# CIawevy/FreeFine

Measured on NVIDIA B200. Metric: edits/s @512^2 50-step SD1.5 (FreeFine 2-D geometric edit), higher is better.
Workload: dtype bf16

## Files before the change

### freefine_b200/_lib.py

```python
from __future__ import annotations

import ctypes as C
import os

_HERE = os.path.dirname(os.path.abspath(__file__))
LIB_PATH = os.environ.get("FREEFINE_B200_LIB", os.path.join(_HERE, "lib", "libfreefine_b200.so"))

FF_MAX_PASS = 4
FF_DT_F32, FF_DT_BF16, FF_DT_F16 = 0, 1, 2
FF_PASS_KEY_INVERT, FF_PASS_ROW_XOR, FF_PASS_ROW_WEIGHT, FF_PASS_KEY2_INVERT = 1, 2, 4, 8
FF_PASS_KEY_PREFIX, FF_PASS_KEY2_PREFIX = 16, 32


class FFAttnPass(C.Structure):
    _fields_ = [("kv_stream", C.c_int32), ("key_mask", C.c_int32), ("row_mask", C.c_int32), ("flags", C.c_uint32),
                ("weight", C.c_float), ("kv_stream2", C.c_int32), ("key_mask2", C.c_int32), ("reserved", C.c_int32)]


class FFAttnHeadPlan(C.Structure):
    _fields_ = [("n_pass", C.c_int32), ("reserved", C.c_int32 * 3), ("passes", FFAttnPass * FF_MAX_PASS)]


class FFAttnArgs(C.Structure):
    _fields_ = [("q", C.c_void_p), ("k", C.c_void_p), ("v", C.c_void_p), ("out", C.c_void_p), ("plan", C.c_void_p),
                ("bitmasks", C.c_void_p), ("mask_popcount", C.c_void_p),
                ("n_streams", C.c_int32), ("n_kv_streams", C.c_int32), ("heads", C.c_int32), ("head_dim", C.c_int32),
                ("s_q", C.c_int32), ("s_kv", C.c_int32), ("n_masks", C.c_int32), ("mask_words", C.c_int32),
                ("out_dtype", C.c_int32), ("scale", C.c_float), ("v_dtype", C.c_int32), ("v_head_stride", C.c_int32)]


PLAN_BYTES = C.sizeof(FFAttnHeadPlan)
PASS_BYTES = C.sizeof(FFAttnPass)

SIGNATURES = {
    "ff_version": (C.c_int, []),
    "ff_last_error": (C.c_char_p, []),
    "ff_attn_masked_kv": (C.c_int, [C.POINTER(FFAttnArgs), C.c_void_p]),
    "ff_attn_v_head_stride": (C.c_int, [C.c_int32]),
    "ff_attn_plain_smallkv": (C.c_int, [C.c_void_p] * 4 + [C.c_int32] * 5 + [C.c_float, C.c_int32, C.c_void_p]),
    "ff_debug_set_timeline": (C.c_int, [C.c_void_p]),
    "ff_kv_gather_cast": (C.c_int, [C.c_void_p, C.c_void_p, C.c_void_p, C.c_void_p, C.c_void_p, C.c_int32, C.c_int64,
                                    C.c_int32, C.c_int32, C.c_void_p]),
    "ff_mask_downsample_pack": (C.c_int, [C.c_void_p, C.c_int32, C.c_int32, C.c_int32, C.c_int32, C.c_int32,
                                          C.c_void_p, C.c_int32, C.c_void_p, C.c_void_p]),
    "ff_upsample2x_nhwc": (C.c_int, [C.c_void_p, C.c_void_p, C.c_int32, C.c_int32, C.c_int32, C.c_int32, C.c_void_p]),
    "ff_concat_nhwc": (C.c_int, [C.c_void_p, C.c_void_p, C.c_void_p, C.c_int64, C.c_int32, C.c_int32, C.c_void_p]),
    "ff_linear_bias_residual": (C.c_int, [C.c_void_p] * 5 + [C.c_int64, C.c_int32, C.c_int32, C.c_void_p, C.c_int64, C.c_void_p]),
    "ff_mask_prep": (C.c_int, [C.c_void_p] * 4 + [C.c_int32] * 7 + [C.c_void_p] * 6),
    "ff_dilate_mask": (C.c_int, [C.c_void_p, C.c_void_p, C.c_int32, C.c_int32, C.c_int32, C.c_int32, C.c_void_p]),
    "ff_warp_affine_blend": (C.c_int, [C.c_void_p, C.c_void_p, C.c_void_p, C.c_void_p, C.c_void_p, C.c_void_p,
                                       C.c_int32, C.c_int32, C.c_int32, C.c_int32, C.c_int32, C.c_int32, C.c_int32,
                                       C.c_int32, C.c_void_p]),
    "ff_ddim_cfg_step": (C.c_int, [C.c_void_p, C.c_void_p, C.c_void_p, C.c_void_p, C.c_void_p, C.c_float, C.c_float,
                                   C.c_float, C.c_float, C.c_float, C.c_float, C.c_float, C.c_void_p, C.c_void_p,
                                   C.c_int32, C.c_int32, C.c_int32, C.c_int32, C.c_void_p]),
    "ff_debug_set_trace": (C.c_int, [C.c_void_p]),
    "ff_ddim_step": (C.c_int, [C.c_void_p, C.c_void_p, C.c_void_p, C.c_void_p, C.c_float, C.c_float, C.c_float,
                               C.c_float, C.c_float, C.c_float, C.c_void_p, C.c_void_p, C.c_int32, C.c_int32,
                               C.c_int32, C.c_int32, C.c_void_p]),
    "ff_ddim_cfg_step_compose": (C.c_int, [C.c_void_p, C.c_int32, C.c_void_p, C.c_void_p, C.c_void_p, C.c_void_p,
                                           C.c_float, C.c_float, C.c_float, C.c_float, C.c_float, C.c_float, C.c_float,
                                           C.c_void_p, C.c_void_p, C.c_int32, C.c_int32, C.c_int32, C.c_int32, C.c_void_p]),
    "ff_ddim_inv_step": (C.c_int, [C.c_void_p, C.c_void_p, C.c_float, C.c_float, C.c_float, C.c_float, C.c_void_p,
                                   C.c_void_p, C.c_int64, C.c_void_p]),
    "ff_cross_region_blend": (C.c_int, [C.c_void_p, C.c_void_p, C.c_int32, C.c_void_p, C.c_int32, C.c_int32,
                                        C.c_int32, C.c_int32, C.c_void_p]),
    "ff_group_norm_ws_bytes": (C.c_int64, [C.c_int32, C.c_int32]),
    "ff_group_norm_nhwc": (C.c_int, [C.c_void_p, C.c_void_p, C.c_int64, C.c_void_p, C.c_void_p, C.c_void_p, C.c_void_p,
                                     C.c_int32, C.c_int32, C.c_int32, C.c_int32, C.c_float, C.c_int32, C.c_void_p]),
    "ff_bias_residual_nhwc": (C.c_int, [C.c_void_p, C.c_void_p, C.c_void_p, C.c_void_p, C.c_int64, C.c_int32,
                                        C.c_void_p]),
    "ff_geglu": (C.c_int, [C.c_void_p, C.c_void_p, C.c_int64, C.c_int32, C.c_void_p]),
    "ff_layer_norm": (C.c_int, [C.c_void_p, C.c_void_p, C.c_void_p, C.c_void_p, C.c_int64, C.c_int32, C.c_float,
                                C.c_void_p]),
}

_lib = None


def load() -> C.CDLL:
    global _lib
    if _lib is None:
        if not os.path.exists(LIB_PATH):
            raise RuntimeError(f"{LIB_PATH} is missing: build it with `python -m freefine_b200.csrc.build` "
                               "(freefine_b200 has no fallback path)")
        lib = C.CDLL(LIB_PATH)
        for name, (res, args) in SIGNATURES.items():
            fn = getattr(lib, name)
            fn.restype, fn.argtypes = res, args
        _lib = lib
    return _lib


def check(rc: int, what: str) -> None:
    if rc != 0:
        msg = load().ff_last_error()
        raise RuntimeError(f"{what} failed (code {rc}): {msg.decode() if msg else ''}")
```

### freefine_b200/attention.py

```python
from __future__ import annotations

import abc
import math

import os

import torch

from . import ops, plans


class AttentionControl(abc.ABC):
    def step_callback(self, x_t):
        return x_t

    def between_steps(self):
        return

    @property
    def num_uncond_att_layers(self):
        return self.num_att_layers if self.LOW_RESOURCE else 0

    @abc.abstractmethod
    def forward(self, attn, is_cross: bool, place_in_unet: str):
        raise NotImplementedError

    def _advance(self):
        self.cur_att_layer += 1
        if self.cur_att_layer == self.num_att_layers + self.num_uncond_att_layers:
            self.cur_att_layer = 0
            self.cur_step += 1
            self.between_steps()

    def __call__(self, attn, is_cross: bool, place_in_unet: str):
        self._advance()
        return attn

    def reset(self):
        self.cur_step = 0
        self.cur_att_layer = 0

    def __init__(self):
        self.cur_step = 0
        self.num_att_layers = -1
        self.cur_att_layer = 0
        self.LOW_RESOURCE = False


def _as_u8_stack(mask: torch.Tensor) -> torch.Tensor:
    m = mask if mask.dim() == 3 else mask[None]
    if m.dtype != torch.uint8:
        m = m.clamp(0, 255).to(torch.uint8)
    return m.contiguous()


class Attention_Modulator(AttentionControl):

    def __init__(self, start_layer=None):
        super().__init__()
        self.step_num = 0
        self.model_type = 'Inverse'
        self.use_cfg = False
        self.use_style_align = False
        self.use_tca = False
        self.local_edit = False
        self.fg_retain_mask = None
        self.fg_retain_mask_st2 = None
        self.fg_ref_mask = None
        self.obj_mask = None
        self.local_edit_region = None
        self.layer_idx = list(range(start_layer, 16)) if start_layer is not None else list(range(16))
        self.down_sampling_shape = dict()
        self.method = None
        self.context_guidance = None
        self.tca_scope = ['up']
        self.style_align_scope = ['down', 'mid', 'up']
        self.src_masks = None
        self.tgt_masks = None
        self.prompt_length = 1
        self.heads = None
        self.scale = None
        self.upcast_attention = False
        self.upcast_softmax = False
        self.log_mask = False
        self.sort_keys = True
        self.p_operand = "f16"
        self.small_kv_kernel = os.environ.get("FF_ATTN_SMALLKV", "1") != "0"
        self._tables = {}
        self._plans = {}

    def forward(self, attn, is_cross: bool, place_in_unet: str):
        return attn

    def reset(self):
        super().reset()
        self.step_num = 0
        self.model_type = 'Inverse'
        self.use_cfg = False
        self.use_tca = False
        self.use_style_align = False
        self.local_edit = False
        self.down_sampling_shape = dict()
        self.style_align = False
        self.method = None
        self.context_guidance = None
        self.tca_scope = ['up']
        self.style_align_scope = ['down', 'mid', 'up']
        self._tables.clear()
        self._plans.clear()

    def get_down_h_w(self, d_ratio, h, w, seq):
        if d_ratio in self.down_sampling_shape:
            nh, nw = self.down_sampling_shape[d_ratio]
            assert nh * nw == seq, f'{nh} * {nw} != {seq}'
            return nh, nw
        r = d_ratio // 8
        nh, nw = h // 8, w // 8
        while r != 1:
            r //= 2
            nh, nw = (nh + 1) // 2, (nw + 1) // 2
        assert nw * nh == seq
        self.down_sampling_shape[d_ratio] = [nh, nw]
        return nh, nw

    def _grid(self, H, W, seq):
        d_ratio = 2 ** int(math.log2((H * W // seq) ** 0.5) + 0.5)
        return self.get_down_h_w(d_ratio, H, W, seq)

    def _table(self, kind: str, seq: int, masks, min_tokens: int = 0):
        sig = tuple((m.data_ptr(), m._version, tuple(m.shape)) for m in masks)
        hit = self._tables.get((kind, seq))
        if hit is not None and hit[0] == sig:
            return hit[1], hit[2]
        stacks = [_as_u8_stack(m) for m in masks]
        E, H, W = stacks[0].shape
        for s in stacks:
            if s.shape != (E, H, W):
                raise ValueError(f"mask shapes differ: {[tuple(x.shape) for x in stacks]}")
            if not s.is_cuda:
                raise RuntimeError("controller masks must live on the CUDA device (no CPU path)")
        h, w = self._grid(H, W, seq)
        stacked = torch.stack(stacks, dim=1).reshape(E * len(stacks), H, W)
        words = ops.mask_words(max(seq, min_tokens))
        bits = torch.zeros((stacked.shape[0], words), dtype=torch.int32, device=stacked.device)
        bits, pop = ops.mask_downsample_pack(stacked, h, w, bits=bits)
        self._tables[(kind, seq)] = (sig, bits, pop, tuple(masks))
        return bits, pop

    def _plan(self, key, builder):
        p = self._plans.get(key)
        if p is None:
            if len(self._plans) > 256:
                self._plans.clear()
            host = builder()
            p = ops.to_device_bytes(host, self._device)
            self._plans[key] = p
            ops.PLAN_REGISTRY[p.data_ptr()] = host
        return p

    def _kv_index(self, kind: str, seq: int, bits, stream_masks):
        ck = (kind, "kvidx", seq)
        hit = self._tables.get(ck)
        if hit is not None and hit[0] is bits:
            return hit[1]
        shifts = torch.arange(32, device=bits.device, dtype=torch.int32)
        key_bits = ((bits[:, :, None] >> shifts) & 1).reshape(bits.shape[0], -1)[:, :seq]
        idx = plans.kv_sort_index(key_bits, stream_masks)
        self._tables[ck] = (bits, idx)
        return idx

    def _attend(self, query, key, value, plan, bits=None, pop=None, kv_index=None):
        self._device = query.device
        dt = query.dtype
        if dt not in (torch.float32, torch.bfloat16):
            query, key, value, dt = query.float(), key.float(), value.float(), torch.float32
        q = query.to(torch.bfloat16).contiguous()
        k = key.to(torch.bfloat16).contiguous()
        v = value.to(torch.bfloat16).contiguous()
        k, v = ops.kv_gather_cast(k, v, self.heads, kv_index, p_operand=self.p_operand)
        return ops.attn_masked_kv(q, k, v, plan, self.heads, self.scale, bits, pop, out_dtype=dt)

    def plain_attention(self, query, key, value):
        self._device = query.device
        B = query.shape[0]
        if key.shape[0] != B:
            raise ValueError("plain attention needs one K/V stream per query stream")
        d = query.shape[-1] // self.heads
        if (key.shape[1] <= (128 if d == 8 else ops.SMALLKV_MAX_KEYS) and d in ops.SMALLKV_HEAD_DIMS and self.p_operand == "f16"
                and self.small_kv_kernel):
            dt = query.dtype
            if dt not in (torch.float32, torch.bfloat16):
                query, key, value, dt = query.float(), key.float(), value.float(), torch.float32
            return ops.attn_plain_smallkv(query.to(torch.bfloat16).contiguous(), key.to(torch.bfloat16).contiguous(),
                                          value.to(torch.bfloat16).contiguous(), self.heads, self.scale, out_dtype=dt)
        plan = self._plan(("plain", B, self.heads), lambda: plans.plain_plan(B, self.heads))
        return self._attend(query, key, value, plan)

    def _tca_common(self, query, key, value, kind):
        B, S, _ = query.shape
        if self.cur_att_layer // 2 not in self.layer_idx:
            out = self.plain_attention(query, key, value)
            self._advance()
            return out
        if B % 4:
            raise ValueError(f"TCA expects 4 streams [u_e,u_r,c_e,c_r] per edit, got batch {B}")
        if self.method not in ('tca', 'mmsa'):
            raise ValueError(f"controller.method must be 'tca' or 'mmsa' here, got {self.method!r}")
        E = B // 4
        self._device = query.device
        if kind == "edit":
            bits, pop = self._table("edit", S, [self.fg_ref_mask, self.fg_retain_mask])
            src_id, tgt_id = (lambda e: 2 * e), (lambda e: 2 * e + 1)
        else:
            bits, pop = self._table("bg", S, [self.fg_retain_mask])
            src_id, tgt_id = (lambda e: e), (lambda e: e)
        if bits.shape[0] not in (2 * E if kind == "edit" else E,):
            raise ValueError(f"{E} edits in the stream batch but masks for {bits.shape[0]} rows")
        cg = None if self.method == 'mmsa' else float(self.context_guidance)
        pf = self.sort_keys
        plan = self._plan((kind, E, self.heads, self.method, cg, pf),
                          lambda: plans.tca_plan(E, self.heads, self.method, cg, src_id, tgt_id, kind=kind, prefix=pf))
        kv_index = None
        if pf:
            kv_index = self._kv_index(kind, S, bits, [src_id(s // 4) if s % 2 else -1 for s in range(B)])
        out = self._attend(query, key, value, plan, bits, pop, kv_index)
        self._advance()
        return out

    def Temporal_contextal_attention(self, query, key, value, is_cross, place_in_unet):
        return self._tca_common(query, key, value, "edit")

    def Temporal_contextal_attention_bg(self, query, key, value, is_cross, place_in_unet):
        return self._tca_common(query, key, value, "bg")

    def Temporal_contextal_attention_compose(self, query, key, value, is_cross, place_in_unet):
        B, S, _ = query.shape
        if self.cur_att_layer // 2 not in self.layer_idx:
            out = self.plain_attention(query, key, value)
            self._advance()
            return out
        N = B - 2
        self._device = query.device
        src = self.src_masks[:N] if torch.is_tensor(self.src_masks) else torch.stack(list(self.src_masks)[:N])
        tgt = self.tgt_masks[:N] if torch.is_tensor(self.tgt_masks) else torch.stack(list(self.tgt_masks)[:N])
        bits, pop = self._table("compose", S, [m for m in src] + [m for m in tgt])
        cg = None if self.method == 'mmsa' else float(self.context_guidance)
        pf = self.sort_keys
        plan = self._plan(("compose", N, self.heads, self.method, cg, pf),
                          lambda: plans.compose_plan(N, self.heads, self.method, cg, list(range(N)),
                                                     list(range(N, 2 * N)), prefix=pf))
        kv_index = self._kv_index("compose", S, bits, [-1] + list(range(N)) + [-1]) if pf else None
        out = self._attend(query, key, value, plan, bits, pop, kv_index)
        self._advance()
        return out

    def _style_align(self, query, key, value, mask, bg=False):
        B, S, _ = query.shape
        if B % 4:
            raise ValueError("style-align expects 4 streams per edit")
        E = B // 4
        self._device = query.device
        bits = pop = None
        src_id = None
        if self.method == 'sdsa':
            bits, pop = self._table("sdsa", S, [mask])
            src_id = lambda e: e
        pf = self.sort_keys and src_id is not None
        plan = self._plan(("style", E, self.heads, self.method, pf, bg),
                          lambda: plans.style_align_plan(E, self.heads, src_id, prefix=pf, bg=bg))
        kv_index = self._kv_index("sdsa", S, bits, [s // 4 if s % 2 else -1 for s in range(B)]) if pf else None
        out = self._attend(query, key, value, plan, bits, pop, kv_index)
        self._advance()
        return out

    def style_align_share_attention(self, query, key, value, is_cross, place_in_unet):
        return self._style_align(query, key, value, self.fg_ref_mask)

    def style_align_share_attention_bg(self, query, key, value, is_cross, place_in_unet):
        return self._style_align(query, key, value, self.fg_retain_mask, bg=True)

    def modulate_local_cross_attn(self, query, key, value, is_cross, place_in_unet):
        B, S, _ = query.shape
        if B % 4:
            raise ValueError("local cross-attention modulation expects 4 streams per edit")
        hs = self.plain_attention(query, key, value)
        bits, _ = self._table("region", S, [self.local_edit_region])
        ids = self._plans.get(("region_ids", B // 4))
        if ids is None:
            ids = torch.arange(B // 4, dtype=torch.int32, device=query.device)
            self._plans[("region_ids", B // 4)] = ids
        ops.cross_region_blend(hs, bits, ids)
        self._advance()
        return hs

    modulate_local_cross_attn_bg = modulate_local_cross_attn

    def modulate_local_cross_attn_compose(self, query, key, value, is_cross, place_in_unet):
        Bq, S, _ = query.shape
        self._device = query.device
        L = len(self.tgt_masks)
        nu = Bq - 1
        if key.shape[0] != nu + L:
            raise ValueError(f"expected {nu + L} prompt streams, got {key.shape[0]}")
        tg = self.tgt_masks if torch.is_tensor(self.tgt_masks) else torch.stack(list(self.tgt_masks))
        bits, pop = self._table("cross_compose", S, [m for m in tg], min_tokens=key.shape[1])

        def build():
            p = plans._empty(Bq, self.heads)
            for s in range(nu):
                for h in range(self.heads):
                    plans._add(p, s, h, s, 1.0)
            for h in range(self.heads):
                for i in range(L):
                    plans._add(p, nu, h, nu + i, 1.0, row_mask=i, flags=plans.FF_PASS_ROW_WEIGHT)
            return p

        plan = self._plan(("cross_compose", Bq, L, self.heads), build)
        out = self._attend(query, key, value, plan, bits, pop)
        self._advance()
        return out


def override_forward(unet):
    inner = unet.forward

    def forward(sample, timestep, encoder_hidden_states, *args, **kwargs):
        out = inner(sample, timestep, encoder_hidden_states, *args, **kwargs)
        if torch.is_tensor(out):
            return out
        return out.sample if hasattr(out, "sample") else out[0]

    return forward


class _DummyController:
    num_att_layers = 0
    use_tca = use_style_align = local_edit = False

    def __call__(self, *args):
        return args[0]


def _register(model, controller, flavour: str):
    if controller is None:
        controller = _DummyController()
    plain = Attention_Modulator()

    def ca_forward(self, place_in_unet):
        to_out = self.to_out[0] if isinstance(self.to_out, torch.nn.ModuleList) else self.to_out

        def forward(hidden_states, encoder_hidden_states=None, attention_mask=None, temb=None):
            is_cross = encoder_hidden_states is not None
            residual = hidden_states
            if self.spatial_norm is not None:
                hidden_states = self.spatial_norm(hidden_states, temb)
            input_ndim = hidden_states.ndim
            if input_ndim == 4:
                batch_size, channel, height, width = hidden_states.shape
                hidden_states = hidden_states.view(batch_size, channel, height * width).transpose(1, 2)
            if attention_mask is not None:
                raise NotImplementedError("explicit attention_mask is not part of the FreeFine hot path")
            if self.group_norm is not None:
                hidden_states = self.group_norm(hidden_states.transpose(1, 2)).transpose(1, 2)
            query = self.to_q(hidden_states)
            if encoder_hidden_states is None:
                encoder_hidden_states = hidden_states
            elif self.norm_cross:
                encoder_hidden_states = self.norm_encoder_hidden_states(encoder_hidden_states)
            key = self.to_k(encoder_hidden_states)
            value = self.to_v(encoder_hidden_states)

            c = controller if isinstance(controller, Attention_Modulator) else plain
            c.heads, c.scale = self.heads, self.scale
            c.upcast_attention, c.upcast_softmax = self.upcast_attention, self.upcast_softmax
            if flavour == "edit":
                if not is_cross and controller.use_style_align and place_in_unet in controller.style_align_scope:
                    hidden_states = controller.style_align_share_attention(query, key, value, is_cross, place_in_unet)
                elif not is_cross and controller.use_tca and place_in_unet in controller.tca_scope:
                    hidden_states = controller.Temporal_contextal_attention(query, key, value, is_cross, place_in_unet)
                elif controller.local_edit and is_cross:
                    hidden_states = controller.modulate_local_cross_attn(query, key, value, is_cross, place_in_unet)
                else:
                    hidden_states = c.plain_attention(query, key, value)
                    controller(None, is_cross, place_in_unet)
            elif flavour == "bggen":
                if place_in_unet in ['up'] and not is_cross and controller.use_tca:
                    hidden_states = controller.Temporal_contextal_attention_bg(query, key, value, is_cross, place_in_unet)
                elif controller.local_edit and is_cross:
                    hidden_states = controller.modulate_local_cross_attn_bg(query, key, value, is_cross, place_in_unet)
                else:
                    hidden_states = c.plain_attention(query, key, value)
                    controller(None, is_cross, place_in_unet)
            else:
                if not is_cross and controller.use_tca and place_in_unet in controller.tca_scope:
                    hidden_states = controller.Temporal_contextal_attention_compose(query, key, value, is_cross, place_in_unet)
                elif controller.local_edit and is_cross:
                    hidden_states = controller.modulate_local_cross_attn_compose(query, key, value, is_cross, place_in_unet)
                else:
                    hidden_states = c.plain_attention(query, key, value)
                    controller(None, is_cross, place_in_unet)

            block_res = getattr(self, "ff_block_residual", None)
            if (block_res is not None and input_ndim == 3 and hidden_states.is_cuda and hidden_states.dtype == torch.bfloat16
                    and isinstance(to_out, torch.nn.Linear) and not self.residual_connection
                    and self.rescale_output_factor == 1.0):
                self.ff_residual_fused = True
                return ops.linear_bias_residual(hidden_states.contiguous(), to_out.weight, to_out.bias, block_res)
            hidden_states = to_out(hidden_states)
            if input_ndim == 4:
                hidden_states = hidden_states.transpose(-1, -2).reshape(batch_size, channel, height, width)
            if self.residual_connection:
                hidden_states = hidden_states + residual
            if self.rescale_output_factor != 1.0:
                hidden_states = hidden_states / self.rescale_output_factor
            return hidden_states

        return forward

    def register_recr(net_, count, place_in_unet):
        if net_.__class__.__name__ == 'Attention':
            net_.forward = ca_forward(net_, place_in_unet)
            return count + 1
        if hasattr(net_, 'children'):
            for child in net_.children():
                count = register_recr(child, count, place_in_unet)
        return count

    n = 0
    for name, net in model.unet.named_children():
        if "down" in name:
            n += register_recr(net, 0, "down")
        elif "up" in name:
            n += register_recr(net, 0, "up")
        elif "mid" in name:
            n += register_recr(net, 0, "mid")
    controller.num_att_layers = n


def register_attention_control(model, controller):
    _register(model, controller, "edit")


def register_attention_control_4bggen(model, controller):
    _register(model, controller, "bggen")


def register_attention_control_compose(model, controller):
    _register(model, controller, "compose")
```

### freefine_b200/csrc/attn_ring.cuh

```cuda
#pragma once
#include <type_traits>

template <int DPAD_, int NWG_, int NBUF_> struct RCfg {
  static constexpr int DPAD = DPAD_, NWG = NWG_, NBUF = NBUF_;
  static_assert(NBUF > NWG || NWG == 1, "a warpgroup must find its next S ready: more S/P buffers than warpgroups");
  static constexpr int DPV = Cfg<DPAD, false>::DPV;
  static constexpr int NKT = (DPAD + BOX_COLS - 1) / BOX_COLS;
  static constexpr int TMEM_S = 0, TMEM_O = NBUF * BN;
  static constexpr int TMEM_USED = TMEM_O + NWG * DPV;
  static_assert(TMEM_USED <= 512, "TMEM budget");
  static constexpr int TMEM_COLS = TMEM_USED <= 256 ? 256 : 512;
  static constexpr int MIN_CTAS = TMEM_COLS == 256 ? 2 : 1;
  static constexpr int NUM_WARPS = 4 * NWG + 4;
  static constexpr int NUM_THREADS = 32 * NUM_WARPS;
  static constexpr bool REBALANCE = false;
  static constexpr int REG_AUX = 32, REG_SOFTMAX = 112;
  static constexpr int SMEM_Q = NKT * TILE_BYTES;
  static constexpr int SMEM_K = NKT * KV_BYTES;
  static constexpr int ACC_LD = DPAD + 4;
  static constexpr int SMEM_ACC = BM * ACC_LD * 4;
  static constexpr int SMEM_MX = NWG > 1 ? NWG * BM * 4 : 0;
  static constexpr int SMEM_FIXED = 2 * SMEM_Q + SMEM_ACC + SMEM_MX + 1024  + 512 ;
  static constexpr int SMEM_BUDGET = MIN_CTAS == 2 ? 113 * 1024 : 227 * 1024;
  static constexpr int NST_FIT = (SMEM_BUDGET - SMEM_FIXED) / (2 * SMEM_K);
  static constexpr int NST = (NST_FIT >= 2 * NBUF && 2 * NBUF <= 8) ? 2 * NBUF : NBUF;
  static_assert(NST <= NST_FIT, "shared memory budget: the K and V rings must hold NBUF tiles each");
  static constexpr int SMEM_BYTES = SMEM_FIXED + 2 * NST * SMEM_K;
};

#ifdef FF_TIMELINE
#define RT_TL(role_, tile_, site_)                                                                                       \
  do {                                                                                                                   \
    if (tl && (tile_) < FF_TL_TILES) tl[(((size_t)tl_cta * 4 + (role_)) * FF_TL_TILES + (tile_)) * 8 + (site_)] = clock64(); \
  } while (0)
#define RT_TLW(wg_, tile_, site_) do { if ((wg_) < 2) RT_TL(wg_, tile_, site_); } while (0)
#else
#define RT_TL(role_, tile_, site_) do { } while (0)
#define RT_TLW(wg_, tile_, site_) do { } while (0)
#endif

struct TileIter {
  const FFAttnHeadPlan* plan;
  int n_pass, q0, n_kv_tiles;
  int ip, seg, jn, j, j1;
  bool seg_live, valid;
  PassCtx cx;
  SegCtx sg;
  __device__ __forceinline__ void init(const FFAttnHeadPlan* pl, int np, int q0_, int nkt, const KParams& p) {
    plan = pl; n_pass = np; q0 = q0_; n_kv_tiles = nkt;
    ip = -1; seg = 1; jn = 0; j = 0; j1 = 0; seg_live = false; valid = true;
    seek(p);
  }
  __device__ __forceinline__ void seek(const KParams& p) {
#pragma unroll 1
    while (true) {
      if (seg_live && jn < n_kv_tiles) {
        const int cls = tile_class(sg, jn, p), e = run_end(sg, jn, cls, p), jb = jn;
        jn = e;
        if (tile_skip(cx, sg, cls, p.s_kv)) continue;
        j = jb; j1 = e;
        return;
      }
      if (ip >= 0 && seg == 0) {
        seg = 1; sg = cx.s1; seg_live = cx.active && sg.kv >= 0; jn = 0;
        continue;
      }
      if (++ip >= n_pass) { valid = false; return; }
      const FFAttnPass ps = plan->pass[ip];
      cx = make_ctx(ps, p, q0);
      seg = 0; sg = cx.s0; seg_live = cx.active && sg.kv >= 0; jn = 0;
    }
  }
  __device__ __forceinline__ void next(const KParams& p) { if (++j >= j1) seek(p); }
};

__device__ __forceinline__ int count_tiles(const FFAttnHeadPlan* plan, int n_pass, int q0, int n_kv_tiles, const KParams& p,
                                           int& pe0, int& pe1, int& pe2) {
  int n_total = 0;
  pe0 = pe1 = pe2 = 0;
#pragma unroll
  for (int ip = 0; ip < FF_MAX_PASS; ++ip) {
    if (ip < n_pass) {
      const FFAttnPass ps = plan->pass[ip];
      const PassCtx cx = make_ctx(ps, p, q0);
      if (cx.active) {
#pragma unroll 1
        for (int seg = 0; seg < 2; ++seg) {
          const SegCtx sg = seg ? cx.s1 : cx.s0;
          if (sg.kv < 0) continue;
#pragma unroll 1
          for (int j0 = 0; j0 < n_kv_tiles;) {
            const int cls = tile_class(sg, j0, p), j1 = run_end(sg, j0, cls, p), jb = j0;
            j0 = j1;
            if (!tile_skip(cx, sg, cls, p.s_kv)) n_total += j1 - jb;
          }
        }
      }
    }
    if (ip == 0) pe0 = n_total;
    if (ip == 1) pe1 = n_total;
    if (ip == 2) pe2 = n_total;
  }
  return n_total;
}

#ifndef FF_RING_POLY
#define FF_RING_POLY FF_POLY_PATTERN
#endif

template <bool MASKED, int PATTERN>
__device__ __forceinline__ void ring_chunk_f16(const float* s, uint32_t* pk, float sc, float nb, uint32_t bits) {
  const float2 sc2 = make_float2(sc, sc), nb2 = make_float2(nb, nb);
#pragma unroll
  for (int i = 0; i < 8; ++i) {
    float2 x = __ffma2_rn(make_float2(s[2 * i], s[2 * i + 1]), sc2, nb2);
    float2 e;
    if (MASKED) {
      x.x = (bits >> (2 * i)) & 1u ? x.x : -INFINITY;
      x.y = (bits >> (2 * i + 1)) & 1u ? x.y : -INFINITY;
      e = make_float2(fast_exp2(x.x), fast_exp2(x.y));
    } else if ((PATTERN >> i) & 1) {
      e = poly_exp2_x2(x);
    } else {
      e = make_float2(fast_exp2(x.x), fast_exp2(x.y));
    }
    pk[i] = pack_f16x2(e.x, e.y);
  }
}

__device__ __forceinline__ void mbar_wait_lean(uint32_t bar, uint32_t parity) {
  uint32_t done;
  asm volatile(
      "{\n\t.reg .pred p;\n\t"
      "mbarrier.try_wait.parity.shared::cta.b64 p, [%1], %2;\n\t"
      "selp.u32 %0, 1, 0, p;\n\t}"
      : "=r"(done)
      : "r"(bar), "r"(parity)
      : "memory");
  if (!done) mbar_wait_slow(bar, parity);
}

template <int DPAD>
__device__ __forceinline__ void issue_qk(uint32_t sbuf, uint64_t qdesc, uint64_t kdesc, uint32_t idesc, uint32_t bar_s_,
                                         uint32_t bar_ke_) {
  static_assert(DPAD == 48 || DPAD == 80, "issue_qk: 3 or 5 K-steps");
  if constexpr (DPAD == 48) {
    asm volatile(
        "{\n\t.reg .pred e, pf, pt;\n\t.reg .b64 q1, q2, k1, k2;\n\t"
        "elect.sync _|e, 0xffffffff;\n\t"
        "setp.ne.b32 pf, 0, 0;\n\tsetp.eq.b32 pt, 0, 0;\n\t"
        "add.u64 q1, %1, 2;\n\tadd.u64 q2, %1, 4;\n\tadd.u64 k1, %2, 2;\n\tadd.u64 k2, %2, 4;\n\t"
        "@e tcgen05.mma.cta_group::1.kind::f16 [%0], %1, %2, %3, pf;\n\t"
        "@e tcgen05.mma.cta_group::1.kind::f16 [%0], q1, k1, %3, pt;\n\t"
        "@e tcgen05.mma.cta_group::1.kind::f16 [%0], q2, k2, %3, pt;\n\t"
        "@e tcgen05.commit.cta_group::1.mbarrier::arrive::one.shared::cluster.b64 [%4];\n\t"
        "@e tcgen05.commit.cta_group::1.mbarrier::arrive::one.shared::cluster.b64 [%5];\n\t}"
        ::"r"(sbuf), "l"(qdesc), "l"(kdesc), "r"(idesc), "r"(bar_s_), "r"(bar_ke_)
        : "memory");
  } else {
    asm volatile(
        "{\n\t.reg .pred e, pf, pt;\n\t.reg .b64 q1, q2, q3, q4, k1, k2, k3, k4;\n\t"
        "elect.sync _|e, 0xffffffff;\n\t"
        "setp.ne.b32 pf, 0, 0;\n\tsetp.eq.b32 pt, 0, 0;\n\t"
        "add.u64 q1, %1, 2;\n\tadd.u64 q2, %1, 4;\n\tadd.u64 q3, %1, 6;\n\tadd.u64 q4, %1, %6;\n\t"
        "add.u64 k1, %2, 2;\n\tadd.u64 k2, %2, 4;\n\tadd.u64 k3, %2, 6;\n\tadd.u64 k4, %2, %7;\n\t"
        "@e tcgen05.mma.cta_group::1.kind::f16 [%0], %1, %2, %3, pf;\n\t"
        "@e tcgen05.mma.cta_group::1.kind::f16 [%0], q1, k1, %3, pt;\n\t"
        "@e tcgen05.mma.cta_group::1.kind::f16 [%0], q2, k2, %3, pt;\n\t"
        "@e tcgen05.mma.cta_group::1.kind::f16 [%0], q3, k3, %3, pt;\n\t"
        "@e tcgen05.mma.cta_group::1.kind::f16 [%0], q4, k4, %3, pt;\n\t"
        "@e tcgen05.commit.cta_group::1.mbarrier::arrive::one.shared::cluster.b64 [%4];\n\t"
        "@e tcgen05.commit.cta_group::1.mbarrier::arrive::one.shared::cluster.b64 [%5];\n\t}"
        ::"r"(sbuf), "l"(qdesc), "l"(kdesc), "r"(idesc), "r"(bar_s_), "r"(bar_ke_), "n"(TILE_BYTES >> 4), "n"(KV_BYTES >> 4)
        : "memory");
  }
}

__device__ __forceinline__ void issue_pv(uint32_t obuf, uint32_t pbase, uint64_t vdesc, uint32_t idesc, uint32_t acc0,
                                         uint32_t bar_ve_, uint32_t bar_d_) {
  asm volatile(
      "{\n\t.reg .pred e, p0, pt;\n\t.reg .b64 v1, v2, v3;\n\t.reg .b32 a1, a2, a3;\n\t"
      "elect.sync _|e, 0xffffffff;\n\t"
      "setp.ne.b32 p0, %4, 0;\n\tsetp.eq.b32 pt, 0, 0;\n\t"
      "add.u64 v1, %2, 128;\n\tadd.u64 v2, %2, 256;\n\tadd.u64 v3, %2, 384;\n\t"
      "add.u32 a1, %1, 8;\n\tadd.u32 a2, %1, 32;\n\tadd.u32 a3, %1, 40;\n\t"
      "@e tcgen05.mma.cta_group::1.kind::f16 [%0], [%1], %2, %3, p0;\n\t"
      "@e tcgen05.mma.cta_group::1.kind::f16 [%0], [a1], v1, %3, pt;\n\t"
      "@e tcgen05.mma.cta_group::1.kind::f16 [%0], [a2], v2, %3, pt;\n\t"
      "@e tcgen05.mma.cta_group::1.kind::f16 [%0], [a3], v3, %3, pt;\n\t"
      "@e tcgen05.commit.cta_group::1.mbarrier::arrive::one.shared::cluster.b64 [%5];\n\t"
      "@e tcgen05.commit.cta_group::1.mbarrier::arrive::one.shared::cluster.b64 [%6];\n\t}"
      ::"r"(obuf), "r"(pbase), "l"(vdesc), "r"(idesc), "r"(acc0), "r"(bar_ve_), "r"(bar_d_)
      : "memory");
}

__device__ __forceinline__ void token_wait(int g) {
  switch (g) {
    case 0: asm volatile("bar.sync 3, 256;" ::: "memory"); break;
    case 1: asm volatile("bar.sync 4, 256;" ::: "memory"); break;
    default: asm volatile("bar.sync 5, 256;" ::: "memory"); break;
  }
}
__device__ __forceinline__ void token_pass(int g) {
  switch (g) {
    case 0: asm volatile("bar.arrive 3, 256;" ::: "memory"); break;
    case 1: asm volatile("bar.arrive 4, 256;" ::: "memory"); break;
    default: asm volatile("bar.arrive 5, 256;" ::: "memory"); break;
  }
}

template <int DPAD, int NWG, int NBUF, bool TOKEN>
__global__ void __launch_bounds__(RCfg<DPAD, NWG, NBUF>::NUM_THREADS, RCfg<DPAD, NWG, NBUF>::MIN_CTAS)
attn_ring_kernel(const __grid_constant__ CUtensorMap tm_q, const __grid_constant__ CUtensorMap tm_k,
                 const __grid_constant__ CUtensorMap tm_v, const KParams p) {
  using C = RCfg<DPAD, NWG, NBUF>;
  constexpr int NST = C::NST, SW = 4 * NWG;
  extern __shared__ uint8_t smem_raw[];
  const uint32_t smem_base = (smem_u32(smem_raw) + 1023u) & ~1023u;
  const uint32_t sQ = smem_base;
  const uint32_t sK = sQ + 2 * C::SMEM_Q;
  const uint32_t sV = sK + NST * C::SMEM_K;
  const uint32_t sACC = sV + NST * C::SMEM_K;
  const uint32_t sMX = sACC + C::SMEM_ACC;
  const uint32_t bar_base = sMX + C::SMEM_MX;
  const uint32_t bar_qf = bar_base;
  const uint32_t bar_qe = bar_base + 16;
  const uint32_t bar_s = bar_base + 32;
  const uint32_t bar_p = bar_s + 8 * NBUF;
  const uint32_t bar_d = bar_p + 8 * NBUF;
  const uint32_t bar_kf = bar_d + 8 * NBUF, bar_ke = bar_kf + 8 * NST;
  const uint32_t bar_vf = bar_ke + 8 * NST, bar_ve = bar_vf + 8 * NST;
  const uint32_t tmem_slot = bar_ve + 8 * NST;
  static_assert(32 + 24 * NBUF + 32 * NST + 8 <= 512, "barrier block");
  uint8_t* gen_base = smem_raw + (smem_base - smem_u32(smem_raw));
  float* const acc_smem = reinterpret_cast<float*>(gen_base + (sACC - smem_base));
  float* const mx_smem = reinterpret_cast<float*>(gen_base + (sMX - smem_base));
  volatile uint32_t* tmem_slot_ptr = reinterpret_cast<volatile uint32_t*>(gen_base + (tmem_slot - smem_base));

  const int warp = threadIdx.x >> 5, lane = threadIdx.x & 31;
  const int n_kv_tiles = (p.s_kv + BN - 1) / BN;
  const int n_items = p.n_qtiles * p.heads * p.n_streams;

  if (threadIdx.x == 0) {
    for (int i = 0; i < 2; ++i) {
      mbar_init(bar_qf + 8 * i, 1);
      mbar_init(bar_qe + 8 * i, 1);
    }
    for (int i = 0; i < NBUF; ++i) {
      mbar_init(bar_s + 8 * i, 1);
      mbar_init(bar_p + 8 * i, 4);
      mbar_init(bar_d + 8 * i, 1);
    }
    for (int i = 0; i < NST; ++i) {
      mbar_init(bar_kf + 8 * i, 1);
      mbar_init(bar_ke + 8 * i, 1);
      mbar_init(bar_vf + 8 * i, 1);
      mbar_init(bar_ve + 8 * i, 1);
    }
    asm volatile("fence.mbarrier_init.release.cluster;" ::: "memory");
  }
  if (warp == SW) {
    asm volatile("tcgen05.alloc.cta_group::1.sync.aligned.shared::cta.b32 [%0], %1;" ::"r"(tmem_slot),
                 "r"((uint32_t)C::TMEM_COLS)
                 : "memory");
    asm volatile("tcgen05.relinquish_alloc_permit.cta_group::1.sync.aligned;" ::: "memory");
  }
  tc_fence_before();
  __syncthreads();
  tc_fence_after();
  const uint32_t tmem = __shfl_sync(0xffffffffu, *tmem_slot_ptr, 0);
#ifdef FF_TIMELINE
  const int tl_cta = blockIdx.x == 5 ? 0 : 1;
  const int tl_role = warp == 0 ? 0 : (warp == 4 && NWG > 1 ? 1 : (warp == SW + 1 ? 2 : (warp == SW + 2 ? 3 : -1)));
  unsigned long long* const tl = ((blockIdx.x == 5 || blockIdx.x == 77) && lane == 0 && tl_role >= 0) ? g_timeline : nullptr;
#endif
  auto item_coords = [&](int w, int& q0, int& head, int& stream) {
    const int qt = w % p.n_qtiles, hs = w / p.n_qtiles;
    q0 = qt * BM;
    head = hs % p.heads;
    stream = hs / p.heads;
  };
  auto item_plan = [&](int head, int stream, int& n_pass) {
    const FFAttnHeadPlan* plan = p.plan + (size_t)stream * p.heads + head;
    n_pass = __ldg(&plan->n_pass);
    n_pass = n_pass < 0 ? 0 : (n_pass > FF_MAX_PASS ? FF_MAX_PASS : n_pass);
    return plan;
  };

  if constexpr (C::REBALANCE) {
    if (warp >= SW) asm volatile("setmaxnreg.dec.sync.aligned.u32 %0;" ::"n"(C::REG_AUX));
    else asm volatile("setmaxnreg.inc.sync.aligned.u32 %0;" ::"n"(C::REG_SOFTMAX));
  }
  if (warp == SW || warp == SW + 3) {
    if (lane == 0) {
      const bool is_k = warp == SW;
      const CUtensorMap* tm = is_k ? &tm_k : &tm_v;
      const uint32_t ring = is_k ? sK : sV, bfull = is_k ? bar_kf : bar_vf, bempty = is_k ? bar_ke : bar_ve;
      int stage = 0, use = 0, li = 0;
#pragma unroll 1
      for (int w = blockIdx.x; w < n_items; w += gridDim.x, ++li) {
        int q0, head, stream, n_pass;
        item_coords(w, q0, head, stream);
        const FFAttnHeadPlan* plan = item_plan(head, stream, n_pass);
        if (is_k) {
          const int qb = li & 1;
          if (li >= 2) mbar_wait(bar_qe + 8 * qb, ((li >> 1) - 1) & 1);
          mbar_expect_tx(bar_qf + 8 * qb, C::NKT * TILE_BYTES);
          for (int kt = 0; kt < C::NKT; ++kt)
            tma_load_4d(sQ + qb * C::SMEM_Q + kt * TILE_BYTES, &tm_q, kt * BOX_COLS, head, q0, stream, bar_qf + 8 * qb);
        }
        TileIter ti;
        ti.init(plan, n_pass, q0, n_kv_tiles, p);
#pragma unroll 1
        while (ti.valid) {
          if (use > 0) mbar_wait(bempty + 8 * stage, (use - 1) & 1);
          const uint32_t full = bfull + 8 * stage, dst = ring + stage * C::SMEM_K;
          mbar_expect_tx(full, C::NKT * KV_BYTES);
          for (int kt = 0; kt < C::NKT; ++kt)
            tma_load_4d(dst + kt * KV_BYTES, tm, kt * BOX_COLS, head, ti.j * BN, ti.sg.kv, full);
          if (++stage == NST) { stage = 0; ++use; }
          ti.next(p);
        }
      }
    }
  } else if (warp == SW + 1) {
    constexpr uint32_t idesc_qk = make_idesc(BN, 0);
    const uint64_t qdesc00 = smem_desc_sw128(sQ, 16);
    const uint64_t kdesc0 = smem_desc_sw128(sK, 16);
    uint32_t kph = 0, bph0 = 0;
    int u = 0, tg = 0, li = 0;
#pragma unroll 1
    for (int w = blockIdx.x; w < n_items; w += gridDim.x, ++li) {
      int q0, head, stream, n_pass, pe0, pe1, pe2;
      item_coords(w, q0, head, stream);
      const FFAttnHeadPlan* plan = item_plan(head, stream, n_pass);
      int left = __shfl_sync(0xffffffffu, count_tiles(plan, n_pass, q0, n_kv_tiles, p, pe0, pe1, pe2), 0);
      const int qb = li & 1;
      const uint64_t qdesc0 = qdesc00 + (uint64_t)((qb * C::SMEM_Q) >> 4);
      mbar_wait(bar_qf + 8 * qb, (li >> 1) & 1);
#pragma unroll 1
      while (left > 0) {
#pragma unroll
        for (int uu = 0; uu < NST; ++uu) {
          if (uu < u) continue;
          if (left == 0) break;
          const int b = uu % NBUF;
          const uint32_t bph = bph0 ^ (uint32_t)((uu / NBUF) & 1);
          RT_TL(2, tg, 0);
          mbar_wait_lean(bar_kf + 8 * uu, kph);
          RT_TL(2, tg, 1);
          if (tg >= NBUF) mbar_wait_lean(bar_d + 8 * b, bph ^ 1u);
          RT_TL(2, tg, 2);
          tc_fence_after();
          issue_qk<DPAD>(tmem + C::TMEM_S + BN * b, qdesc0, kdesc0 + (uint64_t)((uu * C::SMEM_K) >> 4), idesc_qk,
                         bar_s + 8 * b, bar_ke + 8 * uu);
          __syncwarp();
          RT_TL(2, tg, 3);
          --left;
          ++tg;
          u = uu + 1;
        }
        if (u == NST) {
          u = 0;
          kph ^= 1u;
          bph0 ^= (uint32_t)((NST / NBUF) & 1);
        }
      }
      if (elect_one()) tc_commit(bar_qe + 8 * qb);
      __syncwarp();
    }
  } else if (warp == SW + 2) {
    constexpr uint32_t idesc_pv = make_idesc(C::DPV, 1, true);
    const uint64_t vdesc0 = smem_desc_sw128(sV, KV_BYTES);
    uint32_t vph = 0, bph0 = 0, g = 0;
    int u = 0, tg = 0;
#pragma unroll 1
    for (int w = blockIdx.x; w < n_items; w += gridDim.x) {
      int q0, head, stream, n_pass, pe0, pe1, pe2;
      item_coords(w, q0, head, stream);
      const FFAttnHeadPlan* plan = item_plan(head, stream, n_pass);
      const int n_total = __shfl_sync(0xffffffffu, count_tiles(plan, n_pass, q0, n_kv_tiles, p, pe0, pe1, pe2), 0);
      pe0 = __shfl_sync(0xffffffffu, pe0, 0);
      pe1 = __shfl_sync(0xffffffffu, pe1, 0);
      pe2 = __shfl_sync(0xffffffffu, pe2, 0);
      int t = 0, pi = 0, pend = pe0, pstart = 0;
      g = 0;
#pragma unroll 1
      while (t < n_total) {
#pragma unroll
        for (int uu = 0; uu < NST; ++uu) {
          if (uu < u) continue;
          if (t >= n_total) break;
          const int b = uu % NBUF;
          const uint32_t bph = bph0 ^ (uint32_t)((uu / NBUF) & 1);
          while (t >= pend && pi < 3) {
            pstart = pend;
            ++pi;
            pend = pi == 1 ? pe1 : (pi == 2 ? pe2 : n_total);
          }
          const uint32_t acc0 = (t - pstart < NWG) ? 0u : 1u;
          RT_TL(3, tg, 0);
          mbar_wait_lean(bar_vf + 8 * uu, vph);
          RT_TL(3, tg, 1);
          mbar_wait_lean(bar_p + 8 * b, bph);
          RT_TL(3, tg, 2);
          tc_fence_after();
          issue_pv(tmem + C::TMEM_O + C::DPV * g, tmem + C::TMEM_S + BN * b, vdesc0 + (uint64_t)((uu * C::SMEM_K) >> 4),
                   idesc_pv, acc0, bar_ve + 8 * uu, bar_d + 8 * b);
          __syncwarp();
          RT_TL(3, tg, 3);
          if (++g == (uint32_t)NWG) g = 0;
          ++t;
          ++tg;
          u = uu + 1;
        }
        if (u == NST) {
          u = 0;
          vph ^= 1u;
          bph0 ^= (uint32_t)((NST / NBUF) & 1);
        }
      }
    }
  } else if (warp < SW) {
    const int wq = warp & 3;
    const int wg = warp >> 2;
    const int rloc = 32 * wq + lane;
    const uint32_t tlane = tmem + ((uint32_t)(wq * 32) << 16);
    const uint32_t tO = tlane + C::TMEM_O + C::DPV * wg;
    float* const acc_row = acc_smem + (size_t)rloc * C::ACC_LD;
    int base = 0;
    int my_b = 0, prev_b = -1;
    uint32_t my_ph = 0, prev_ph = 0;
    bool s_ready = false;
    if (TOKEN && NWG > 1 && wg == NWG - 1) token_pass(0);
#pragma unroll 1
    for (int w = blockIdx.x; w < n_items; w += gridDim.x) {
      int q0, head, stream, n_pass;
      item_coords(w, q0, head, stream);
      const FFAttnHeadPlan* plan = item_plan(head, stream, n_pass);
      const int row = q0 + rloc;
      bool acc_started = false;
      int it = 0;
      int my_next = wg;
      my_b = (base + wg) % NBUF;
      my_ph = (uint32_t)(((base + wg) / NBUF) & 1);
      s_ready = false;
#pragma unroll 1
      for (int ip = 0; ip < n_pass; ++ip) {
        const FFAttnPass ps = plan->pass[ip];
        const PassCtx cx = make_ctx(ps, p, q0);
        if (!cx.active) continue;
        uint32_t rb = 0;
        if (ps.row_mask >= 0 && row < p.s_q)
          rb = (__ldg(p.bitmasks + (size_t)ps.row_mask * p.mask_words + (row >> 5)) >> (row & 31)) & 1u;
        const bool rowflip = cx.rowxor && rb;
        float m_used = -INFINITY;
        int n_mine = 0;
        const int it_pass0 = it;
#pragma unroll 1
        for (int seg = 0; seg < 2; ++seg) {
          const SegCtx sg = seg ? cx.s1 : cx.s0;
          if (sg.kv < 0) continue;
          const bool flip = sg.kinv != rowflip;
          const bool uniform = uniform_for(cx, sg, flip, p.s_kv);
          const float sc = uniform ? 0.f : p.scale_log2;
#pragma unroll 1
          for (int j0 = 0; j0 < n_kv_tiles;) {
            const int cls = tile_class(sg, j0, p), j1 = run_end(sg, j0, cls, p), jb = j0;
            j0 = j1;
            if (tile_skip(cx, sg, cls, p.s_kv)) continue;
            const bool row_ok_cls = row_allowed(cls, flip, uniform);
            const int it_run = it;
            it += j1 - jb;
            auto tile = [&](auto mixed_tag, int j) {
              constexpr bool MIXED = decltype(mixed_tag)::value;
              const uint32_t tS = tlane + C::TMEM_S + BN * my_b;
              RT_TLW(wg, my_next, 0);
              if (!s_ready) mbar_wait_lean(bar_s + 8 * my_b, my_ph);
              RT_TLW(wg, my_next, 1);
              tc_fence_after();
              float s0[32], s1[32];
              tmem_ld32(tS, s0);
              tmem_ld32(tS + 32, s1);
              uint32_t kb_lo = 0xffffffffu, kb_hi = 0xffffffffu;
              if constexpr (MIXED) {
#pragma unroll
                for (int h = 0; h < 2; ++h) {
                  const int kbase = j * BN + 32 * h;
                  const int rem = p.s_kv - kbase;
                  const uint32_t valid = rem >= 32 ? 0xffffffffu : (rem <= 0 ? 0u : ((1u << rem) - 1u));
                  uint32_t kb = 0xffffffffu;
                  if (sg.kmask >= 0 && !uniform && rem > 0) {
                    if (sg.prefix) {
                      const int tt = sg.T - kbase;
                      kb = tt >= 32 ? 0xffffffffu : (tt <= 0 ? 0u : ((1u << tt) - 1u));
                    } else {
                      kb = __ldg(p.bitmasks + (size_t)sg.kmask * p.mask_words + (kbase >> 5));
                    }
                    if (flip) kb = ~kb;
                  }
                  if (h == 0) kb_lo = kb & valid; else kb_hi = kb & valid;
                }
              }
              tmem_wait_ld32(s0);
              tmem_wait_ld32(s1);
              RT_TLW(wg, my_next, 2);
              float mt;
              {
                float m0, m1, m2, m3;
                if constexpr (!MIXED) {
                  m0 = fmaxf(s0[0], s0[1]);
                  m1 = fmaxf(s0[2], s0[3]);
                  m2 = fmaxf(s1[0], s1[1]);
                  m3 = fmaxf(s1[2], s1[3]);
#pragma unroll
                  for (int i = 4; i < 32; i += 4) {
                    m0 = fmaxf(m0, fmaxf(s0[i], s0[i + 1]));
                    m1 = fmaxf(m1, fmaxf(s0[i + 2], s0[i + 3]));
                    m2 = fmaxf(m2, fmaxf(s1[i], s1[i + 1]));
                    m3 = fmaxf(m3, fmaxf(s1[i + 2], s1[i + 3]));
                  }
                } else {
                  m0 = m1 = m2 = m3 = -INFINITY;
#pragma unroll
                  for (int i = 0; i < 32; i += 2) {
                    m0 = fmaxf(m0, (kb_lo >> i) & 1u ? s0[i] : -INFINITY);
                    m1 = fmaxf(m1, (kb_lo >> (i + 1)) & 1u ? s0[i + 1] : -INFINITY);
                    m2 = fmaxf(m2, (kb_hi >> i) & 1u ? s1[i] : -INFINITY);
                    m3 = fmaxf(m3, (kb_hi >> (i + 1)) & 1u ? s1[i + 1] : -INFINITY);
                  }
                }
                mt = fmaxf(fmaxf(m0, m1), fmaxf(m2, m3));
              }
              const float mts = (!MIXED && !row_ok_cls) ? -INFINITY : (uniform ? 0.f : mt * p.scale_log2);
              float alpha = 1.f;
              bool grow = false;
              if (n_mine == 0) {
                m_used = mts;
              } else if (mts > m_used + rescale_threshold<false>()) {
                alpha = fast_exp2(m_used - mts);
                m_used = mts;
                grow = true;
              }
              RT_TLW(wg, my_next, 3);
              int nb_ = my_b + NWG;
              uint32_t nph = my_ph;
              if (nb_ >= NBUF) { nb_ -= NBUF; nph ^= 1u; }
              s_ready = mbar_test(bar_s + 8 * nb_, nph);
              const float nb = (MIXED || row_ok_cls) ? -m_used : -60000.f;
              if (TOKEN && NWG > 1) token_wait(wg);
#pragma unroll
              for (int hb = 0; hb < 2; ++hb) {
                const float* sv = hb ? s1 : s0;
                uint32_t pk[16];
                if constexpr (!MIXED) {
#pragma unroll
                  for (int jj = 0; jj < 2; ++jj) ring_chunk_f16<false, FF_RING_POLY>(sv + 16 * jj, pk + 8 * jj, sc, nb, 0u);
                } else {
                  const uint32_t kbits = hb ? kb_hi : kb_lo;
#pragma unroll
                  for (int jj = 0; jj < 2; ++jj)
                    ring_chunk_f16<true, 0>(sv + 16 * jj, pk + 8 * jj, sc, nb, (kbits >> (16 * jj)) & 0xffffu);
                }
                tmem_st16(tS + 32 * hb, pk);
              }
              if (TOKEN && NWG > 1) token_pass((wg + 1) % NWG);
              RT_TLW(wg, my_next, 4);
              if (__any_sync(0xffffffffu, grow)) {
                if (prev_b >= 0) mbar_wait(bar_d + 8 * prev_b, prev_ph);
                tc_fence_after();
#pragma unroll
                for (int c = 0; c < C::DPV / 16; ++c) {
                  float o[16];
                  uint32_t ob[16];
                  tmem_ld16(tO + 16 * c, o);
                  tmem_wait_ld16(o);
#pragma unroll
                  for (int i = 0; i < 16; ++i) ob[i] = __float_as_uint(o[i] * alpha);
                  tmem_st16(tO + 16 * c, ob);
                }
              }
              tmem_wait_st();
              tc_fence_before();
              __syncwarp();
              if (lane == 0) mbar_arrive(bar_p + 8 * my_b);
              RT_TLW(wg, my_next, 5);
              ++n_mine;
              prev_b = my_b;
              prev_ph = my_ph;
              my_next += NWG;
              my_b = nb_;
              my_ph = nph;
            };
            if (cls == TILE_MIX) {
#pragma unroll 1
              while (my_next < it) tile(std::true_type{}, jb + (my_next - it_run));
            } else {
#pragma unroll 1
              while (my_next < it) tile(std::false_type{}, 0);
            }
          }
        }
        if (it == it_pass0) continue;
        if (n_mine > 0) mbar_wait(bar_d + 8 * prev_b, prev_ph);
        tc_fence_after();
        float cg_[NWG];
        bool wrote[NWG];
        if constexpr (NWG > 1) {
          mx_smem[wg * BM + rloc] = n_mine > 0 ? m_used : -INFINITY;
          tc_fence_before();
          named_bar_sync(1, 32 * SW);
          tc_fence_after();
          float mg[NWG], m_all = -INFINITY;
#pragma unroll
          for (int g = 0; g < NWG; ++g) {
            const int first = it_pass0 + ((g - it_pass0) % NWG + NWG) % NWG;
            wrote[g] = first < it;
            mg[g] = mx_smem[g * BM + rloc];
            m_all = fmaxf(m_all, mg[g]);
          }
          float l = 0.f;
#pragma unroll
          for (int g = 0; g < NWG; ++g) {
            const float a = (wrote[g] && mg[g] > -INFINITY) ? fast_exp2(mg[g] - m_all) : 0.f;
            cg_[g] = a;
            if (wrote[g]) l = fmaf(a, tmem_ld1_wait(tlane + C::TMEM_O + C::DPV * g + p.head_dim), l);
          }
          float coef = ps.weight;
          if (ps.flags & FF_PASS_ROW_WEIGHT) coef = rb ? coef : 0.f;
          coef = l > 0.f ? coef / l : 0.f;
#pragma unroll
          for (int g = 0; g < NWG; ++g) cg_[g] *= coef;
        } else {
          wrote[0] = n_mine > 0;
          const float l = (wrote[0] && m_used > -INFINITY) ? tmem_ld1_wait(tO + p.head_dim) : 0.f;
          float coef = ps.weight;
          if (ps.flags & FF_PASS_ROW_WEIGHT) coef = rb ? coef : 0.f;
          cg_[0] = l > 0.f ? coef / l : 0.f;
        }
#pragma unroll
        for (int c = 0; c < DPAD / 16; ++c) {
          if (c % NWG != wg) continue;
          float r[16];
#pragma unroll
          for (int i = 0; i < 16; ++i) r[i] = acc_started ? acc_row[16 * c + i] : 0.f;
#pragma unroll
          for (int g = 0; g < NWG; ++g) {
            if (!wrote[g]) continue;
            float o[16];
            tmem_ld16(tlane + C::TMEM_O + C::DPV * g + 16 * c, o);
            tmem_wait_ld16(o);
#pragma unroll
            for (int i = 0; i < 16; ++i) r[i] = fmaf(cg_[g], o[i], r[i]);
          }
#pragma unroll
          for (int i = 0; i < 16; i += 4)
            *reinterpret_cast<float4*>(acc_row + 16 * c + i) = make_float4(r[i], r[i + 1], r[i + 2], r[i + 3]);
        }
        acc_started = true;
        tc_fence_before();
        if constexpr (NWG > 1) named_bar_sync(2, 32 * SW);
        else __syncwarp();
        tc_fence_after();
      }
      base += it;
      {
        const bool row_ok = row < p.s_q;
        const size_t o_off = ((size_t)stream * p.s_q + (row_ok ? row : 0)) * ((size_t)p.heads * p.head_dim) +
                             (size_t)head * p.head_dim;
#pragma unroll
        for (int c = 0; c < DPAD / 16; ++c) {
          if (c % NWG != wg) continue;
          float o[16];
#pragma unroll
          for (int i = 0; i < 16; ++i) o[i] = acc_started ? acc_row[16 * c + i] : 0.f;
#pragma unroll
          for (int g = 0; g < 2; ++g) {
            if (row_ok && 16 * c + 8 * g < p.head_dim) {
              if (p.out_dtype == FF_DT_BF16) {
                uint4 v;
                v.x = pack_bf16x2(o[8 * g + 0], o[8 * g + 1]);
                v.y = pack_bf16x2(o[8 * g + 2], o[8 * g + 3]);
                v.z = pack_bf16x2(o[8 * g + 4], o[8 * g + 5]);
                v.w = pack_bf16x2(o[8 * g + 6], o[8 * g + 7]);
                *reinterpret_cast<uint4*>(static_cast<__nv_bfloat16*>(p.out) + o_off + 16 * c + 8 * g) = v;
              } else {
                float4* dst = reinterpret_cast<float4*>(static_cast<float*>(p.out) + o_off + 16 * c + 8 * g);
                dst[0] = make_float4(o[8 * g + 0], o[8 * g + 1], o[8 * g + 2], o[8 * g + 3]);
                dst[1] = make_float4(o[8 * g + 4], o[8 * g + 5], o[8 * g + 6], o[8 * g + 7]);
              }
            }
          }
        }
      }
    }
  }
  tc_fence_before();
  __syncthreads();
  if (warp == SW) {
    tc_fence_after();
    asm volatile("tcgen05.dealloc.cta_group::1.sync.aligned.b32 %0, %1;" ::"r"(tmem), "r"((uint32_t)C::TMEM_COLS)
                 : "memory");
  }
}
```

### freefine_b200/csrc/attn_t32.cuh

```cuda
#pragma once

constexpr int TBN = 32;

struct T32 {
  static constexpr int DPAD = 48, DPV = 48, NST = 8;
  static constexpr int KVB = TBN * 128;
  static constexpr int TMEM_S = 0, TMEM_P = 4 * TBN, TMEM_O = 4 * TBN + 2 * (TBN / 2), TMEM_COLS = 256;
  static_assert(TMEM_O + 2 * DPV == 256, "TMEM budget: 4 S buffers, 2 P regions, 2 accumulators");
  static constexpr int SMEM_Q = TILE_BYTES, SMEM_STAGE = 2 * KVB;
  static constexpr int ACC_LD = DPAD + 4, SMEM_ACC = BM * ACC_LD * 4, SMEM_MX = 2 * BM * 4;
  static constexpr int SMEM_BYTES = SMEM_Q + NST * SMEM_STAGE + SMEM_ACC + SMEM_MX + 1024 + 512;
  static_assert(SMEM_BYTES <= 113 * 1024, "two CTAs per SM");
};

__device__ __forceinline__ int t32_class(const SegCtx& g, int j, const KParams& p) {
  const int lo = j * TBN;
  if (lo + TBN > p.s_kv) return TILE_MIX;
  if (g.kmask < 0) return TILE_ALL;
  if (g.prefix) return lo + TBN <= g.T ? TILE_IN : (lo >= g.T ? TILE_OUT : TILE_MIX);
  const uint32_t bits = __ldg(p.bitmasks + (size_t)g.kmask * p.mask_words + (lo >> 5));
  return bits == 0xffffffffu ? TILE_IN : (bits == 0 ? TILE_OUT : TILE_MIX);
}
__device__ __forceinline__ int t32_run_end(const SegCtx& g, int j, int cls, const KParams& p) {
  if (cls == TILE_MIX || (g.kmask >= 0 && !g.prefix)) return j + 1;
  const int n_full = p.s_kv / TBN;
  if (cls == TILE_IN) { const int t = g.T / TBN; return t < n_full ? t : n_full; }
  return n_full;
}

__device__ __forceinline__ void t32_pv(uint32_t obuf, uint32_t pbase, uint64_t vdesc, uint32_t idesc_pv, uint32_t acc0,
                                       uint32_t bar_kve, uint32_t bar_o_) {
  asm volatile(
      "{\n\t.reg .pred e, p0, pt;\n\t.reg .b64 v1;\n\t.reg .b32 a1;\n\t"
      "elect.sync _|e, 0xffffffff;\n\t"
      "setp.ne.b32 p0, %4, 0;\n\tsetp.eq.b32 pt, 0, 0;\n\t"
      "add.u64 v1, %2, 128;\n\tadd.u32 a1, %1, 8;\n\t"
      "@e tcgen05.mma.cta_group::1.kind::f16 [%0], [%1], %2, %3, p0;\n\t"
      "@e tcgen05.mma.cta_group::1.kind::f16 [%0], [a1], v1, %3, pt;\n\t"
      "@e tcgen05.commit.cta_group::1.mbarrier::arrive::one.shared::cluster.b64 [%5];\n\t"
      "@e tcgen05.commit.cta_group::1.mbarrier::arrive::one.shared::cluster.b64 [%6];\n\t}"
      ::"r"(obuf), "r"(pbase), "l"(vdesc), "r"(idesc_pv), "r"(acc0), "r"(bar_kve), "r"(bar_o_)
      : "memory");
}

__global__ void __launch_bounds__(NUM_THREADS, 2)
attn_t32_kernel(const __grid_constant__ CUtensorMap tm_q, const __grid_constant__ CUtensorMap tm_k,
                const __grid_constant__ CUtensorMap tm_v, const KParams p) {
  using C = T32;
  extern __shared__ uint8_t smem_raw[];
  const uint32_t smem_base = (smem_u32(smem_raw) + 1023u) & ~1023u;
  const uint32_t sQ = smem_base;
  const uint32_t sKV = smem_base + C::SMEM_Q;
  const uint32_t sACC = sKV + C::NST * C::SMEM_STAGE;
  const uint32_t sMX = sACC + C::SMEM_ACC;
  const uint32_t bar_base = sMX + C::SMEM_MX;
  const uint32_t bar_q = bar_base;
  const uint32_t bar_s = bar_base + 16;
  const uint32_t bar_p = bar_base + 48;
  const uint32_t bar_o = bar_base + 64;
  const uint32_t bar_kv_full = bar_base + 80, bar_kv_empty = bar_base + 80 + 8 * C::NST;
  const uint32_t tmem_slot = bar_base + 80 + 16 * C::NST;
  static_assert(80 + 16 * C::NST + 8 <= 512, "barrier block");
  uint8_t* gen_base = smem_raw + (smem_base - smem_u32(smem_raw));
  float* const acc_smem = reinterpret_cast<float*>(gen_base + (sACC - smem_base));
  float* const mx_smem = reinterpret_cast<float*>(gen_base + (sMX - smem_base));
  volatile uint32_t* tmem_slot_ptr = reinterpret_cast<volatile uint32_t*>(gen_base + (tmem_slot - smem_base));

  const int warp = threadIdx.x >> 5, lane = threadIdx.x & 31;
  const int q0 = blockIdx.x * BM, head = blockIdx.y, stream = blockIdx.z;
  const FFAttnHeadPlan* plan = p.plan + (size_t)stream * p.heads + head;
  int n_pass = __ldg(&plan->n_pass);
  n_pass = n_pass < 0 ? 0 : (n_pass > FF_MAX_PASS ? FF_MAX_PASS : n_pass);
  const int n_kv_tiles = (p.s_kv + TBN - 1) / TBN;

  if (threadIdx.x == 0) {
    mbar_init(bar_q, 1);
    for (int i = 0; i < 4; ++i) mbar_init(bar_s + 8 * i, 1);
    for (int i = 0; i < 2; ++i) {
      mbar_init(bar_p + 8 * i, NUM_SOFTMAX_WARPS / 2);
      mbar_init(bar_o + 8 * i, 1);
    }
    for (int i = 0; i < C::NST; ++i) {
      mbar_init(bar_kv_full + 8 * i, 1);
      mbar_init(bar_kv_empty + 8 * i, 1);
    }
    asm volatile("fence.mbarrier_init.release.cluster;" ::: "memory");
  }
  if (warp == NUM_SOFTMAX_WARPS) {
    asm volatile("tcgen05.alloc.cta_group::1.sync.aligned.shared::cta.b32 [%0], %1;" ::"r"(tmem_slot),
                 "r"((uint32_t)C::TMEM_COLS)
                 : "memory");
    asm volatile("tcgen05.relinquish_alloc_permit.cta_group::1.sync.aligned;" ::: "memory");
  }
  tc_fence_before();
  __syncthreads();
  tc_fence_after();
  const uint32_t tmem = *tmem_slot_ptr;

  if (warp == NUM_SOFTMAX_WARPS) {
    if (lane == 0) {
      mbar_expect_tx(bar_q, TILE_BYTES);
      tma_load_4d(sQ, &tm_q, 0, head, q0, stream, bar_q);
      int it = 0;
#pragma unroll 1
      for (int ip = 0; ip < n_pass; ++ip) {
        const FFAttnPass ps = plan->pass[ip];
        const PassCtx cx = make_ctx(ps, p, q0);
        if (!cx.active) continue;
#pragma unroll 1
        for (int seg = 0; seg < 2; ++seg) {
          const SegCtx sg = seg ? cx.s1 : cx.s0;
          if (sg.kv < 0) continue;
#pragma unroll 1
          for (int j0 = 0; j0 < n_kv_tiles;) {
            const int cls = t32_class(sg, j0, p), j1 = t32_run_end(sg, j0, cls, p), jb = j0;
            j0 = j1;
            if (tile_skip(cx, sg, cls, p.s_kv)) continue;
#pragma unroll 1
            for (int j = jb; j < j1; ++j, ++it) {
              const int stage = it % C::NST, use = it / C::NST;
              if (use > 0) mbar_wait(bar_kv_empty + 8 * stage, (use - 1) & 1);
              const uint32_t full = bar_kv_full + 8 * stage;
              const uint32_t sK = sKV + stage * C::SMEM_STAGE, sV = sK + C::KVB;
              mbar_expect_tx(full, 2 * C::KVB);
              tma_load_4d(sK, &tm_k, 0, head, j * TBN, sg.kv, full);
              tma_load_4d(sV, &tm_v, 0, head, j * TBN, sg.kv, full);
            }
          }
        }
      }
    }
  } else if (warp == NUM_SOFTMAX_WARPS + 1) {
    constexpr uint32_t idesc_qk = make_idesc(TBN, 0);
    constexpr uint32_t idesc_pv = make_idesc(C::DPV, 1, true);
    const uint64_t qdesc0 = smem_desc_sw128(sQ, 16);
    const uint64_t kdesc0 = smem_desc_sw128(sKV, 16);
    const uint64_t vdesc0 = smem_desc_sw128(sKV + C::KVB, C::KVB);
    int pe0 = 0, pe1 = 0, pe2 = 0, n_total = 0;
#pragma unroll
    for (int ip = 0; ip < FF_MAX_PASS; ++ip) {
      if (ip < n_pass) {
        const FFAttnPass ps = plan->pass[ip];
        const PassCtx cx = make_ctx(ps, p, q0);
        if (cx.active) {
#pragma unroll 1
          for (int seg = 0; seg < 2; ++seg) {
            const SegCtx sg = seg ? cx.s1 : cx.s0;
            if (sg.kv < 0) continue;
#pragma unroll 1
            for (int j0 = 0; j0 < n_kv_tiles;) {
              const int cls = t32_class(sg, j0, p), j1 = t32_run_end(sg, j0, cls, p), jb = j0;
              j0 = j1;
              if (!tile_skip(cx, sg, cls, p.s_kv)) n_total += j1 - jb;
            }
          }
        }
      }
      if (ip == 0) pe0 = n_total;
      if (ip == 1) pe1 = n_total;
      if (ip == 2) pe2 = n_total;
    }
    mbar_wait(bar_q, 0);
    tc_fence_after();
#pragma unroll
    for (int t0 = 0; t0 < 4; ++t0) {
      if (t0 < n_total) {
        lean_wait(bar_kv_full + 8 * t0, 0);
        tc_fence_after();
        lean_qk48(tmem + C::TMEM_S + TBN * (2 * (t0 & 1) + ((t0 >> 1) & 1)), qdesc0, kdesc0 + (uint64_t)((t0 * C::SMEM_STAGE) >> 4),
                  idesc_qk, bar_s + 8 * (2 * (t0 & 1) + ((t0 >> 1) & 1)));
      }
    }
    uint32_t gph = 0;
    int t = 0;
#pragma unroll 1
    while (t < n_total) {
#pragma unroll
      for (int u = 0; u < 8; ++u) {
        if (t < n_total) {
          const int pstart = t >= pe2 ? pe2 : (t >= pe1 ? pe1 : (t >= pe0 ? pe0 : 0));
          const uint32_t acc0 = (t - pstart < 2) ? 0u : 1u;
          const int wgi = u & 1, kb = (u >> 1) & 1;
          lean_wait(bar_p + 8 * wgi, (uint32_t)kb);
          tc_fence_after();
          t32_pv(tmem + C::TMEM_O + C::DPV * wgi, tmem + C::TMEM_P + (TBN / 2) * wgi, vdesc0 + (uint64_t)((u * C::SMEM_STAGE) >> 4),
                 idesc_pv, acc0, bar_kv_empty + 8 * u, bar_o + 8 * wgi);
          if (t + 4 < n_total) {
            lean_wait(bar_kv_full + 8 * ((u + 4) & 7), u < 4 ? gph : gph ^ 1u);
            tc_fence_after();
            lean_qk48(tmem + C::TMEM_S + TBN * (2 * wgi + kb), qdesc0, kdesc0 + (uint64_t)((((u + 4) & 7) * C::SMEM_STAGE) >> 4),
                      idesc_qk, bar_s + 8 * (2 * wgi + kb));
          }
          ++t;
        }
      }
      gph ^= 1u;
    }
    __syncwarp();
  } else {
    const int wq = warp & 3, wg = warp >> 2;
    const int rloc = 32 * wq + lane;
    const int row = q0 + rloc;
    const uint32_t tlane = tmem + ((uint32_t)(wq * 32) << 16);
    const uint32_t tP = tlane + C::TMEM_P + (TBN / 2) * wg;
    const uint32_t tO = tlane + C::TMEM_O + C::DPV * wg;
    const uint32_t tOx = tlane + C::TMEM_O + C::DPV * (wg ^ 1);
    float* const acc_row = acc_smem + (size_t)rloc * C::ACC_LD;
    bool acc_started = false;
    int it = 0;
#pragma unroll 1
    for (int ip = 0; ip < n_pass; ++ip) {
      const FFAttnPass ps = plan->pass[ip];
      const PassCtx cx = make_ctx(ps, p, q0);
      if (!cx.active) continue;
      uint32_t rb = 0;
      if (ps.row_mask >= 0 && row < p.s_q)
        rb = (__ldg(p.bitmasks + (size_t)ps.row_mask * p.mask_words + (row >> 5)) >> (row & 31)) & 1u;
      const bool rowflip = cx.rowxor && rb;
      float m_used = -INFINITY;
      int n_mine = 0, last_mine = 0;
      const int it_pass0 = it;
#pragma unroll 1
      for (int seg = 0; seg < 2; ++seg) {
        const SegCtx sg = seg ? cx.s1 : cx.s0;
        if (sg.kv < 0) continue;
        const bool flip = sg.kinv != rowflip;
        const bool uniform = uniform_for(cx, sg, flip, p.s_kv);
        const float sc = uniform ? 0.f : p.scale_log2;
#pragma unroll 1
        for (int j0 = 0; j0 < n_kv_tiles;) {
          const int cls = t32_class(sg, j0, p), j1 = t32_run_end(sg, j0, cls, p), jb = j0;
          j0 = j1;
          if (tile_skip(cx, sg, cls, p.s_kv)) continue;
          const bool row_ok_cls = row_allowed(cls, flip, uniform);
          int j = jb + (((it ^ wg) & 1) ? 1 : 0);
          int itj = it + (j - jb);
          it += j1 - jb;
#pragma unroll 1
          for (; j < j1; j += 2, itj += 2) {
            const int kbuf = (itj >> 1) & 1;
            const uint32_t tS = tlane + C::TMEM_S + TBN * (2 * wg + kbuf);
            mbar_wait(bar_s + 8 * (2 * wg + kbuf), (uint32_t)((itj >> 2) & 1));
            tc_fence_after();
            float s[32];
            tmem_ld32(tS, s);
            uint32_t kbits = 0xffffffffu;
            if (cls == TILE_MIX) {
              const int kbase = j * TBN;
              const int rem = p.s_kv - kbase;
              const uint32_t valid = rem >= 32 ? 0xffffffffu : (rem <= 0 ? 0u : ((1u << rem) - 1u));
              uint32_t kb = 0xffffffffu;
              if (sg.kmask >= 0 && !uniform && rem > 0) {
                if (sg.prefix) {
                  const int tt = sg.T - kbase;
                  kb = tt >= 32 ? 0xffffffffu : (tt <= 0 ? 0u : ((1u << tt) - 1u));
                } else {
                  kb = __ldg(p.bitmasks + (size_t)sg.kmask * p.mask_words + (kbase >> 5));
                }
                if (flip) kb = ~kb;
              }
              kbits = kb & valid;
            }
            tmem_wait_ld32(s);
            float mt;
            {
              float m0, m1;
              if (cls != TILE_MIX) {
                m0 = fmaxf(s[0], s[1]);
                m1 = fmaxf(s[2], s[3]);
#pragma unroll
                for (int i = 4; i < 32; i += 4) {
                  m0 = fmaxf(m0, fmaxf(s[i], s[i + 1]));
                  m1 = fmaxf(m1, fmaxf(s[i + 2], s[i + 3]));
                }
              } else {
                m0 = m1 = -INFINITY;
#pragma unroll
                for (int i = 0; i < 32; i += 2) {
                  m0 = fmaxf(m0, (kbits >> i) & 1u ? s[i] : -INFINITY);
                  m1 = fmaxf(m1, (kbits >> (i + 1)) & 1u ? s[i + 1] : -INFINITY);
                }
              }
              mt = fmaxf(m0, m1);
              if (cls != TILE_MIX && !row_ok_cls) mt = -INFINITY;
            }
            const float mts = uniform ? 0.f : mt * p.scale_log2;
            float alpha = 1.f;
            bool grow = false;
            if (n_mine == 0) {
              m_used = mts;
            } else if (mts > m_used + rescale_threshold<false>()) {
              alpha = fast_exp2(m_used - mts);
              m_used = mts;
              grow = true;
            }
            const bool any_grow = __any_sync(0xffffffffu, grow);
            const float nb = (cls == TILE_MIX || row_ok_cls) ? -m_used : -INFINITY;
            uint32_t pk[16];
            if (cls != TILE_MIX) {
#pragma unroll
              for (int jj = 0; jj < 2; ++jj) softmax_chunk_f16<false>(s + 16 * jj, pk + 8 * jj, sc, nb, 0u);
            } else {
#pragma unroll
              for (int jj = 0; jj < 2; ++jj) softmax_chunk_f16<true>(s + 16 * jj, pk + 8 * jj, sc, nb, (kbits >> (16 * jj)) & 0xffffu);
            }
            if (itj >= 2) {
              const uint32_t po = (uint32_t)(((itj - 2) >> 1) & 1);
              if (!mbar_test(bar_o + 8 * wg, po)) mbar_wait(bar_o + 8 * wg, po);
            }
            tc_fence_after();
            if (any_grow) {
#pragma unroll
              for (int c = 0; c < C::DPV / 16; ++c) {
                float o[16];
                uint32_t ob[16];
                tmem_ld16(tO + 16 * c, o);
                tmem_wait_ld16(o);
#pragma unroll
                for (int i = 0; i < 16; ++i) ob[i] = __float_as_uint(o[i] * alpha);
                tmem_st16(tO + 16 * c, ob);
              }
            }
            tmem_st16(tP, pk);
            tmem_wait_st();
            tc_fence_before();
            __syncwarp();
            if (lane == 0) mbar_arrive(bar_p + 8 * wg);
            ++n_mine;
            last_mine = itj;
          }
        }
      }
      if (it == it_pass0) continue;
      if (n_mine > 0) mbar_wait(bar_o + 8 * wg, (uint32_t)((last_mine >> 1) & 1));
      tc_fence_after();
      mx_smem[wg * BM + rloc] = n_mine > 0 ? m_used : -INFINITY;
      tc_fence_before();
      named_bar_sync(1, 32 * NUM_SOFTMAX_WARPS);
      tc_fence_after();
      const float m_other = mx_smem[(wg ^ 1) * BM + rloc];
      const float m_all = fmaxf(m_used, m_other);
      const bool wrote_mine = n_mine > 0, wrote_other = (it - it_pass0) - n_mine > 0;
      const float a_mine = (wrote_mine && m_used > -INFINITY) ? fast_exp2(m_used - m_all) : 0.f;
      const float a_other = (wrote_other && m_other > -INFINITY) ? fast_exp2(m_other - m_all) : 0.f;
      float l = 0.f;
      if (wrote_mine) l = a_mine * tmem_ld1_wait(tO + p.head_dim);
      if (wrote_other) l = fmaf(a_other, tmem_ld1_wait(tOx + p.head_dim), l);
      float coef = ps.weight;
      if (ps.flags & FF_PASS_ROW_WEIGHT) coef = rb ? coef : 0.f;
      coef = l > 0.f ? coef / l : 0.f;
      const float c_mine = coef * a_mine, c_other = coef * a_other;
#pragma unroll
      for (int c = 0; c < C::DPAD / 16; ++c) {
        if ((c & 1) != wg) continue;
        float r[16];
#pragma unroll
        for (int i = 0; i < 16; ++i) r[i] = acc_started ? acc_row[16 * c + i] : 0.f;
        if (wrote_mine) {
          float o[16];
          tmem_ld16(tO + 16 * c, o);
          tmem_wait_ld16(o);
#pragma unroll
          for (int i = 0; i < 16; ++i) r[i] = fmaf(c_mine, o[i], r[i]);
        }
        if (wrote_other) {
          float o[16];
          tmem_ld16(tOx + 16 * c, o);
          tmem_wait_ld16(o);
#pragma unroll
          for (int i = 0; i < 16; ++i) r[i] = fmaf(c_other, o[i], r[i]);
        }
#pragma unroll
        for (int i = 0; i < 16; i += 4)
          *reinterpret_cast<float4*>(acc_row + 16 * c + i) = make_float4(r[i], r[i + 1], r[i + 2], r[i + 3]);
      }
      acc_started = true;
      tc_fence_before();
      named_bar_sync(2, 32 * NUM_SOFTMAX_WARPS);
      tc_fence_after();
    }
    {
      const bool row_ok = row < p.s_q;
      const size_t o_off = ((size_t)stream * p.s_q + (row_ok ? row : 0)) * ((size_t)p.heads * p.head_dim) +
                           (size_t)head * p.head_dim;
#pragma unroll
      for (int c = 0; c < C::DPAD / 16; ++c) {
        if ((c & 1) != wg) continue;
        float o[16];
#pragma unroll
        for (int i = 0; i < 16; ++i) o[i] = acc_started ? acc_row[16 * c + i] : 0.f;
#pragma unroll
        for (int g = 0; g < 2; ++g) {
          if (row_ok && 16 * c + 8 * g < p.head_dim) {
            if (p.out_dtype == FF_DT_BF16) {
              uint4 v;
              v.x = pack_bf16x2(o[8 * g + 0], o[8 * g + 1]);
              v.y = pack_bf16x2(o[8 * g + 2], o[8 * g + 3]);
              v.z = pack_bf16x2(o[8 * g + 4], o[8 * g + 5]);
              v.w = pack_bf16x2(o[8 * g + 6], o[8 * g + 7]);
              *reinterpret_cast<uint4*>(static_cast<__nv_bfloat16*>(p.out) + o_off + 16 * c + 8 * g) = v;
            } else {
              float4* dst = reinterpret_cast<float4*>(static_cast<float*>(p.out) + o_off + 16 * c + 8 * g);
              dst[0] = make_float4(o[8 * g + 0], o[8 * g + 1], o[8 * g + 2], o[8 * g + 3]);
              dst[1] = make_float4(o[8 * g + 4], o[8 * g + 5], o[8 * g + 6], o[8 * g + 7]);
            }
          }
        }
      }
    }
  }
  tc_fence_before();
  __syncthreads();
  if (warp == NUM_SOFTMAX_WARPS) {
    tc_fence_after();
    asm volatile("tcgen05.dealloc.cta_group::1.sync.aligned.b32 %0, %1;" ::"r"(tmem), "r"((uint32_t)C::TMEM_COLS)
                 : "memory");
  }
}
```

### freefine_b200/csrc/attn_tcgen05.cu

```cuda
#include <cuda.h>
#include <cuda_bf16.h>

#include <atomic>
#include <cstdlib>
#include <type_traits>

#include "ff_common.cuh"

namespace {

constexpr int BM = 128;
constexpr int BN = 64;
constexpr int BOX_COLS = 64;
constexpr int TILE_BYTES = BM * 128;
constexpr int KV_BYTES = BN * 128;
constexpr int NUM_SOFTMAX_WARPS = 8;
constexpr int NUM_THREADS = 32 * (NUM_SOFTMAX_WARPS + 2);
template <bool HILO> constexpr float rescale_threshold() { return HILO ? 24.f : 8.f; }
#ifndef FF_RING_DEFAULT
#define FF_RING_DEFAULT 6
#endif
#ifndef FF_POLY_PATTERN
#define FF_POLY_PATTERN 0x92
#endif
#ifndef FF_T32_DEFAULT
#define FF_T32_DEFAULT 0
#endif
#ifndef FF_SEP_P
#define FF_SEP_P 0
#endif
#ifndef FF_SELF_ISSUE
#define FF_SELF_ISSUE 0
#endif

template <int DPAD, bool HILO> struct Cfg {
  static constexpr int DPV = DPAD == 16 ? 16 : (DPAD == 48 ? 48 : DPAD + 16);
  static constexpr int NKT = (DPAD + BOX_COLS - 1) / BOX_COLS;
  static_assert((DPV + BOX_COLS - 1) / BOX_COLS == NKT, "V tile must span as many boxes as the K tile");
  static constexpr int NSTAGE = DPAD <= 48 ? 4 : (DPAD <= 80 ? 3 : 2);
  static_assert(NSTAGE >= 2, "QK(t+1) is issued before PV(t): tile t+1 must fit beside tile t");
  static constexpr bool SEP = FF_SEP_P && DPAD == 48 && !HILO && NSTAGE == 4;
  static constexpr int TMEM_S = 0, TMEM_P = 2 * BN, TMEM_O = 2 * BN + (SEP ? BN / 2 : 0);
  static constexpr int TMEM_USED = TMEM_O + 2 * DPV;
  static constexpr int TMEM_COLS = TMEM_USED <= 256 ? 256 : 512;
  static constexpr int SMEM_Q = NKT * TILE_BYTES;
  static constexpr int SMEM_STAGE = 2 * NKT * KV_BYTES;
  static constexpr int ACC_LD = DPAD <= 80 ? DPAD + 4 : DPAD;
  static constexpr int SMEM_ACC = BM * ACC_LD * 4;
  static constexpr int SMEM_MX = 2 * BM * 4;
  static constexpr int SMEM_BYTES = SMEM_Q + NSTAGE * SMEM_STAGE + SMEM_ACC + SMEM_MX + 1024  + 256 ;
  static_assert(SMEM_BYTES <= 227 * 1024, "shared memory budget");
  static constexpr int MIN_CTAS = (SMEM_BYTES <= 113 * 1024 && TMEM_COLS == 256) ? 2 : 1;
  static constexpr bool SELF = FF_SELF_ISSUE && !SEP && DPAD == 48 && !HILO && NSTAGE == 4;
  static constexpr int THREADS = SELF ? 32 * (NUM_SOFTMAX_WARPS + 1) : NUM_THREADS;
};

__device__ __forceinline__ uint32_t smem_u32(const void* p) { return (uint32_t)__cvta_generic_to_shared(p); }

__device__ __forceinline__ void mbar_init(uint32_t bar, uint32_t count) {
  asm volatile("mbarrier.init.shared::cta.b64 [%0], %1;" ::"r"(bar), "r"(count));
}
__device__ __forceinline__ void mbar_expect_tx(uint32_t bar, uint32_t bytes) {
  asm volatile("mbarrier.arrive.expect_tx.shared::cta.b64 _, [%0], %1;" ::"r"(bar), "r"(bytes) : "memory");
}
__device__ __forceinline__ void mbar_arrive(uint32_t bar) {
  asm volatile("mbarrier.arrive.shared::cta.b64 _, [%0];" ::"r"(bar) : "memory");
}
__device__ __forceinline__ uint32_t mbar_try(uint32_t bar, uint32_t parity) {
  uint32_t done;
#ifdef FF_TRYWAIT_NOHINT
  asm volatile(
      "{\n\t.reg .pred p;\n\t"
      "mbarrier.try_wait.parity.shared::cta.b64 p, [%1], %2;\n\t"
      "selp.u32 %0, 1, 0, p;\n\t}"
      : "=r"(done)
      : "r"(bar), "r"(parity)
      : "memory");
#else
  asm volatile(
      "{\n\t.reg .pred p;\n\t"
      "mbarrier.try_wait.parity.shared::cta.b64 p, [%1], %2, %3;\n\t"
      "selp.u32 %0, 1, 0, p;\n\t}"
      : "=r"(done)
      : "r"(bar), "r"(parity), "r"(0x989680u)
      : "memory");
#endif
  return done;
}
__device__ __forceinline__ bool mbar_test(uint32_t bar, uint32_t parity) {
  uint32_t done;
  asm volatile(
      "{\n\t.reg .pred p;\n\t"
      "mbarrier.test_wait.parity.shared::cta.b64 p, [%1], %2;\n\t"
      "selp.u32 %0, 1, 0, p;\n\t}"
      : "=r"(done)
      : "r"(bar), "r"(parity)
      : "memory");
  return done != 0;
}
#ifndef FF_WAIT_FORM
#define FF_WAIT_FORM 1
#endif
__device__ __noinline__ void mbar_wait_slow(uint32_t bar, uint32_t parity) {
#if FF_WAIT_FORM == 0
  const long long t0 = clock64();
  while (!mbar_try(bar, parity)) {
    if (clock64() - t0 > 4000000000LL) {
      printf("ff_attn: mbarrier wait timed out (block %d,%d,%d thread %d bar %u parity %u)\n", blockIdx.x,
             blockIdx.y, blockIdx.z, threadIdx.x, bar, parity);
      __trap();
    }
  }
#else
  const long long t0 = clock64();
#pragma unroll 1
  for (uint32_t n = 1;; ++n) {
    if ((n & 15u) == 0 && clock64() - t0 > 4000000000LL) break;
#if FF_WAIT_FORM == 1
    if (mbar_try(bar, parity)) return;
#else
    uint32_t done;
    asm volatile(
        "{\n\t.reg .pred p;\n\t"
        "mbarrier.try_wait.parity.shared::cta.b64 p, [%1], %2;\n\t"
        "selp.u32 %0, 1, 0, p;\n\t}"
        : "=r"(done)
        : "r"(bar), "r"(parity)
        : "memory");
    if (done) return;
#endif
  }
  printf("ff_attn: mbarrier wait timed out (block %d,%d,%d thread %d bar %u parity %u)\n", blockIdx.x, blockIdx.y,
         blockIdx.z, threadIdx.x, bar, parity);
  __trap();
#endif
}
__device__ __forceinline__ void mbar_wait(uint32_t bar, uint32_t parity) {
  if (!mbar_try(bar, parity)) mbar_wait_slow(bar, parity);
}
#ifndef FF_SPIN_MASK
#define FF_SPIN_MASK 0
#endif
template <int ROLE_BIT>
__device__ __forceinline__ void mbar_wait_hot(uint32_t bar, uint32_t parity) {
  if constexpr ((FF_SPIN_MASK >> ROLE_BIT) & 1) {
    for (uint32_t n = 0; !mbar_test(bar, parity); ++n) {
#ifdef FF_SPIN_SLEEP
      __nanosleep(FF_SPIN_SLEEP);
#endif
      if (n > (1u << 24)) { mbar_wait_slow(bar, parity); return; }
    }
  } else {
    mbar_wait(bar, parity);
  }
}
__device__ __forceinline__ void tma_load_4d(uint32_t dst, const CUtensorMap* map, int c0, int c1, int c2, int c3,
                                            uint32_t bar) {
  asm volatile(
      "cp.async.bulk.tensor.4d.shared::cluster.global.tile.mbarrier::complete_tx::bytes [%0], [%1, {%2, %3, %4, %5}], [%6];"
      ::"r"(dst), "l"(map), "r"(c0), "r"(c1), "r"(c2), "r"(c3), "r"(bar)
      : "memory");
}
__device__ __forceinline__ void named_bar_sync(int id, int count) {
  switch (id) {
    case 1: asm volatile("bar.sync 1, %0;" ::"r"(count) : "memory"); break;
    case 2: asm volatile("bar.sync 2, %0;" ::"r"(count) : "memory"); break;
    case 3: asm volatile("bar.sync 3, %0;" ::"r"(count) : "memory"); break;
    default: asm volatile("bar.sync 4, %0;" ::"r"(count) : "memory"); break;
  }
}
__device__ __forceinline__ bool elect_one() {
  uint32_t pred;
  asm volatile("{\n\t.reg .pred p;\n\telect.sync _|p, 0xffffffff;\n\tselp.u32 %0, 1, 0, p;\n\t}" : "=r"(pred));
  return pred != 0;
}
__device__ __forceinline__ void tc_fence_before() { asm volatile("tcgen05.fence::before_thread_sync;" ::: "memory"); }
__device__ __forceinline__ void tc_fence_after() { asm volatile("tcgen05.fence::after_thread_sync;" ::: "memory"); }
__device__ __forceinline__ void tc_commit(uint32_t bar) {
  asm volatile("tcgen05.commit.cta_group::1.mbarrier::arrive::one.shared::cluster.b64 [%0];" ::"r"(bar) : "memory");
}
__device__ __forceinline__ void mma_ss(uint32_t d_tmem, uint64_t a_desc, uint64_t b_desc, uint32_t idesc,
                                       uint32_t accumulate) {
  asm volatile(
      "{\n\t.reg .pred p;\n\tsetp.ne.b32 p, %4, 0;\n\t"
      "tcgen05.mma.cta_group::1.kind::f16 [%0], %1, %2, %3, p;\n\t}"
      ::"r"(d_tmem), "l"(a_desc), "l"(b_desc), "r"(idesc), "r"(accumulate)
      : "memory");
}
__device__ __forceinline__ void mma_ts(uint32_t d_tmem, uint32_t a_tmem, uint64_t b_desc, uint32_t idesc,
                                       uint32_t accumulate) {
  asm volatile(
      "{\n\t.reg .pred p;\n\tsetp.ne.b32 p, %4, 0;\n\t"
      "tcgen05.mma.cta_group::1.kind::f16 [%0], [%1], %2, %3, p;\n\t}"
      ::"r"(d_tmem), "r"(a_tmem), "l"(b_desc), "r"(idesc), "r"(accumulate)
      : "memory");
}
__device__ __forceinline__ void tmem_ld32(uint32_t taddr, float (&v)[32]) {
  uint32_t* r = reinterpret_cast<uint32_t*>(v);
  asm volatile(
      "tcgen05.ld.sync.aligned.32x32b.x32.b32 "
      "{%0, %1, %2, %3, %4, %5, %6, %7, %8, %9, %10, %11, %12, %13, %14, %15, "
      "%16, %17, %18, %19, %20, %21, %22, %23, %24, %25, %26, %27, %28, %29, %30, %31}, [%32];"
      : "=r"(r[0]), "=r"(r[1]), "=r"(r[2]), "=r"(r[3]), "=r"(r[4]), "=r"(r[5]), "=r"(r[6]), "=r"(r[7]),
        "=r"(r[8]), "=r"(r[9]), "=r"(r[10]), "=r"(r[11]), "=r"(r[12]), "=r"(r[13]), "=r"(r[14]), "=r"(r[15]),
        "=r"(r[16]), "=r"(r[17]), "=r"(r[18]), "=r"(r[19]), "=r"(r[20]), "=r"(r[21]), "=r"(r[22]), "=r"(r[23]),
        "=r"(r[24]), "=r"(r[25]), "=r"(r[26]), "=r"(r[27]), "=r"(r[28]), "=r"(r[29]), "=r"(r[30]), "=r"(r[31])
      : "r"(taddr)
      : "memory");
}
__device__ __forceinline__ void tmem_ld16(uint32_t taddr, float (&v)[16]) {
  uint32_t* r = reinterpret_cast<uint32_t*>(v);
  asm volatile(
      "tcgen05.ld.sync.aligned.32x32b.x16.b32 "
      "{%0, %1, %2, %3, %4, %5, %6, %7, %8, %9, %10, %11, %12, %13, %14, %15}, [%16];"
      : "=r"(r[0]), "=r"(r[1]), "=r"(r[2]), "=r"(r[3]), "=r"(r[4]), "=r"(r[5]), "=r"(r[6]), "=r"(r[7]),
        "=r"(r[8]), "=r"(r[9]), "=r"(r[10]), "=r"(r[11]), "=r"(r[12]), "=r"(r[13]), "=r"(r[14]), "=r"(r[15])
      : "r"(taddr)
      : "memory");
}
__device__ __forceinline__ float tmem_ld1_wait(uint32_t taddr) {
  uint32_t r;
  asm volatile("tcgen05.ld.sync.aligned.32x32b.x1.b32 {%0}, [%1];\n\ttcgen05.wait::ld.sync.aligned;"
               : "=r"(r) : "r"(taddr) : "memory");
  return __uint_as_float(r);
}
__device__ __forceinline__ void tmem_st16(uint32_t taddr, const uint32_t (&r)[16]) {
  asm volatile(
      "tcgen05.st.sync.aligned.32x32b.x16.b32 [%0], "
      "{%1, %2, %3, %4, %5, %6, %7, %8, %9, %10, %11, %12, %13, %14, %15, %16};"
      ::"r"(taddr), "r"(r[0]), "r"(r[1]), "r"(r[2]), "r"(r[3]), "r"(r[4]), "r"(r[5]), "r"(r[6]), "r"(r[7]),
        "r"(r[8]), "r"(r[9]), "r"(r[10]), "r"(r[11]), "r"(r[12]), "r"(r[13]), "r"(r[14]), "r"(r[15])
      : "memory");
}
__device__ __forceinline__ void tmem_wait_ld() { asm volatile("tcgen05.wait::ld.sync.aligned;" ::: "memory"); }
__device__ __forceinline__ void tmem_wait_ld16(float (&v)[16]) {
#ifdef FF_PLAIN_WAIT
  tmem_wait_ld();
  return;
#endif
  uint32_t* r = reinterpret_cast<uint32_t*>(v);
  asm volatile("tcgen05.wait::ld.sync.aligned;"
               : "+r"(r[0]), "+r"(r[1]), "+r"(r[2]), "+r"(r[3]), "+r"(r[4]), "+r"(r[5]), "+r"(r[6]), "+r"(r[7]),
                 "+r"(r[8]), "+r"(r[9]), "+r"(r[10]), "+r"(r[11]), "+r"(r[12]), "+r"(r[13]), "+r"(r[14]), "+r"(r[15])
               :
               : "memory");
}
__device__ __forceinline__ void tmem_wait_ld32(float (&v)[32]) {
#ifdef FF_PLAIN_WAIT
  tmem_wait_ld();
  return;
#endif
  uint32_t* r = reinterpret_cast<uint32_t*>(v);
  asm volatile("tcgen05.wait::ld.sync.aligned;"
               : "+r"(r[0]), "+r"(r[1]), "+r"(r[2]), "+r"(r[3]), "+r"(r[4]), "+r"(r[5]), "+r"(r[6]), "+r"(r[7]),
                 "+r"(r[8]), "+r"(r[9]), "+r"(r[10]), "+r"(r[11]), "+r"(r[12]), "+r"(r[13]), "+r"(r[14]), "+r"(r[15]),
                 "+r"(r[16]), "+r"(r[17]), "+r"(r[18]), "+r"(r[19]), "+r"(r[20]), "+r"(r[21]), "+r"(r[22]), "+r"(r[23]),
                 "+r"(r[24]), "+r"(r[25]), "+r"(r[26]), "+r"(r[27]), "+r"(r[28]), "+r"(r[29]), "+r"(r[30]), "+r"(r[31])
               :
               : "memory");
}
__device__ __forceinline__ void tmem_wait_st() { asm volatile("tcgen05.wait::st.sync.aligned;" ::: "memory"); }
__device__ __forceinline__ float fast_exp2(float x) {
#ifdef FF_KO_MUFU
  return x;
#else
  float y;
  asm("ex2.approx.ftz.f32 %0, %1;" : "=f"(y) : "f"(x));
  return y;
#endif
}

__device__ __forceinline__ uint64_t smem_desc_sw128(uint32_t saddr, uint32_t lbo_bytes) {
  return (uint64_t)((saddr & 0x3FFFFu) >> 4) | ((uint64_t)(lbo_bytes >> 4) << 16) | ((uint64_t)(1024u >> 4) << 32) |
         (1ull << 46) | (2ull << 61);
}
__host__ __device__ constexpr uint32_t make_idesc(int n, int b_mn, bool f16 = false) {
  return (1u << 4) | (f16 ? 0u : ((1u << 7) | (1u << 10))) | ((uint32_t)b_mn << 16) | ((uint32_t)(n >> 3) << 17) |
         ((uint32_t)(BM >> 4) << 24);
}

__device__ uint32_t* g_trace = nullptr;
__device__ __forceinline__ void trace(uint32_t* tr, int role, uint32_t it, uint32_t site) {
  if (tr) {
    const uint32_t cta = blockIdx.x + gridDim.x * (blockIdx.y + gridDim.y * blockIdx.z);
    volatile uint32_t* t = tr + (size_t)cta * 8 + role * 2;
    t[0] = it;
    t[1] = site;
    __threadfence_system();
  }
}

#ifdef FF_TIMELINE
__device__ unsigned long long* g_timeline = nullptr;
#define FF_TL_TILES 64
#define FF_TL(role_, tile_, site_)                                                                      \
  do {                                                                                                  \
    if (tl && (tile_) < FF_TL_TILES) tl[(((size_t)tl_cta * 2 + (role_)) * FF_TL_TILES + (tile_)) * 8 + (site_)] = clock64(); \
  } while (0)
#else
#define FF_TL(role_, tile_, site_) do { } while (0)
#endif

struct KParams {
  const FFAttnHeadPlan* plan;
  const uint32_t* bitmasks;
  const int32_t* popc;
  void* out;
  int heads, head_dim, s_q, s_kv, mask_words, out_dtype, n_kv_streams;
  int n_streams, n_qtiles;
  float scale_log2;
};

enum { TILE_ALL = 0, TILE_IN = 1, TILE_OUT = 2, TILE_MIX = 3 };

struct SegCtx {
  int kv;
  int kmask;
  int T;
  bool kinv, prefix;
};
struct PassCtx {
  SegCtx s0, s1;
  bool rowxor, active, two_seg;
  bool has_rf0, has_rf1;
};

__device__ __forceinline__ PassCtx make_ctx(const FFAttnPass& ps, const KParams& p, int q0) {
  PassCtx c;
  c.s0.kv = ps.kv_stream;
  c.s1.kv = ps.kv_stream2;
  c.two_seg = ps.kv_stream2 >= 0;
  c.s0.kmask = ps.key_mask;
  c.s1.kmask = ps.key_mask2;
  c.s0.kinv = (ps.flags & FF_PASS_KEY_INVERT) != 0;
  c.s1.kinv = (ps.flags & FF_PASS_KEY2_INVERT) != 0;
  c.s0.prefix = (ps.flags & FF_PASS_KEY_PREFIX) != 0;
  c.s1.prefix = (ps.flags & FF_PASS_KEY2_PREFIX) != 0;
  c.s0.T = ps.key_mask >= 0 ? __ldg(p.popc + ps.key_mask) : 0;
  c.s1.T = ps.key_mask2 >= 0 ? __ldg(p.popc + ps.key_mask2) : 0;
  c.rowxor = (ps.flags & FF_PASS_ROW_XOR) != 0 && ps.row_mask >= 0;
  c.active = true;
  c.has_rf0 = true;
  c.has_rf1 = false;
  if (ps.row_mask >= 0 && (c.rowxor || (ps.flags & FF_PASS_ROW_WEIGHT))) {
    uint32_t any1 = 0, any0 = 0;
    for (int w = 0; w < BM / 32; ++w) {
      const int base = q0 + 32 * w;
      if (base >= p.s_q) break;
      const uint32_t bits = __ldg(p.bitmasks + (size_t)ps.row_mask * p.mask_words + (base >> 5));
      const int rem = p.s_q - base;
      const uint32_t valid = rem >= 32 ? 0xffffffffu : ((1u << rem) - 1u);
      any1 |= bits & valid;
      any0 |= ~bits & valid;
    }
    if (ps.flags & FF_PASS_ROW_WEIGHT) c.active = any1 != 0;
    if (c.rowxor) {
      c.has_rf0 = any0 != 0;
      c.has_rf1 = any1 != 0;
    }
  }
  return c;
}

__device__ __forceinline__ bool uniform_for(const PassCtx& c, const SegCtx& g, bool f, int s_kv) {
  if (c.two_seg || g.kmask < 0) return false;
  return (f ? s_kv - g.T : g.T) == 0;
}

__device__ __forceinline__ int tile_class(const SegCtx& g, int j, const KParams& p) {
  const int lo = j * BN;
  if (lo + BN > p.s_kv) return TILE_MIX;
  if (g.kmask < 0) return TILE_ALL;
  if (g.prefix) return lo + BN <= g.T ? TILE_IN : (lo >= g.T ? TILE_OUT : TILE_MIX);
  uint32_t a = 0xffffffffu, o = 0;
  for (int w = 0; w < BN / 32; ++w) {
    const uint32_t bits = __ldg(p.bitmasks + (size_t)g.kmask * p.mask_words + (lo >> 5) + w);
    a &= bits;
    o |= bits;
  }
  return a == 0xffffffffu ? TILE_IN : (o == 0 ? TILE_OUT : TILE_MIX);
}

__device__ __forceinline__ int run_end(const SegCtx& g, int j, int cls, const KParams& p) {
  if (cls == TILE_MIX || (g.kmask >= 0 && !g.prefix)) return j + 1;
  const int n_full = p.s_kv / BN;
  if (cls == TILE_IN) { const int t = g.T / BN; return t < n_full ? t : n_full; }
  return n_full;
}

__device__ __forceinline__ bool row_allowed(int cls, bool flip, bool uniform) {
  return uniform || cls == TILE_ALL || ((cls == TILE_IN) != flip);
}

__device__ __forceinline__ bool tile_skip(const PassCtx& c, const SegCtx& g, int cls, int s_kv) {
  if (cls == TILE_MIX || cls == TILE_ALL) return false;
  bool need = false;
  if (c.has_rf0) need = need || row_allowed(cls, g.kinv, uniform_for(c, g, g.kinv, s_kv));
  if (c.has_rf1) need = need || row_allowed(cls, !g.kinv, uniform_for(c, g, !g.kinv, s_kv));
  return !need;
}

__device__ __forceinline__ uint32_t pack_bf16x2(float lo, float hi) {
  const __nv_bfloat162 b = __floats2bfloat162_rn(lo, hi);
  return *reinterpret_cast<const uint32_t*>(&b);
}

template <bool MASKED>
__device__ __forceinline__ void softmax_chunk_hilo(const float* s, uint32_t* hl, float sc, float nb, uint32_t bits) {
  const float2 sc2 = make_float2(sc, sc), nb2 = make_float2(nb, nb);
#pragma unroll
  for (int i = 0; i < 8; ++i) {
    float2 x = __ffma2_rn(make_float2(s[2 * i], s[2 * i + 1]), sc2, nb2);
    if (MASKED) {
      x.x = (bits >> (2 * i)) & 1u ? x.x : -INFINITY;
      x.y = (bits >> (2 * i + 1)) & 1u ? x.y : -INFINITY;
    }
    const float2 e = make_float2(fast_exp2(x.x), fast_exp2(x.y));
    const uint32_t b0 = __float_as_uint(e.x), b1 = __float_as_uint(e.y);
    hl[i] = __byte_perm(b0, b1, 0x7632);
    const float2 r = __fadd2_rn(e, make_float2(-__uint_as_float(b0 & 0xffff0000u), -__uint_as_float(b1 & 0xffff0000u)));
    hl[8 + i] = pack_bf16x2(r.x, r.y);
  }
}

__device__ __forceinline__ float2 poly_exp2_x2(float2 x) {
  const float MAGIC = 12582912.f;
  x.x = fmaxf(x.x, -125.f);
  x.y = fmaxf(x.y, -125.f);
  const float2 t = __fadd2_rn(x, make_float2(MAGIC, MAGIC));
  const float2 n = __fadd2_rn(t, make_float2(-MAGIC, -MAGIC));
  const float2 f = __fadd2_rn(x, make_float2(-n.x, -n.y));
  float2 r = __ffma2_rn(make_float2(0.055205512791872025f, 0.055205512791872025f), f,
                        make_float2(0.24261389672756195f, 0.24261389672756195f));
  r = __ffma2_rn(r, f, make_float2(0.6932547688484192f, 0.6932547688484192f));
  r = __ffma2_rn(r, f, make_float2(0.9999276995658875f, 0.9999276995658875f));
  r.x = __int_as_float(__float_as_int(r.x) + (__float_as_int(t.x) << 23));
  r.y = __int_as_float(__float_as_int(r.y) + (__float_as_int(t.y) << 23));
  return r;
}

__device__ __forceinline__ uint32_t pack_f16x2(float lo, float hi) {
  uint32_t r;
  asm("cvt.rn.f16x2.f32 %0, %1, %2;" : "=r"(r) : "f"(hi), "f"(lo));
  return r;
}

template <bool MASKED>
__device__ __forceinline__ void softmax_chunk_f16(const float* s, uint32_t* pk, float sc, float nb, uint32_t bits) {
  const float2 sc2 = make_float2(sc, sc), nb2 = make_float2(nb, nb);
#pragma unroll
  for (int i = 0; i < 8; ++i) {
    float2 x = __ffma2_rn(make_float2(s[2 * i], s[2 * i + 1]), sc2, nb2);
    float2 e;
    if (MASKED) {
      x.x = (bits >> (2 * i)) & 1u ? x.x : -INFINITY;
      x.y = (bits >> (2 * i + 1)) & 1u ? x.y : -INFINITY;
      e = make_float2(fast_exp2(x.x), fast_exp2(x.y));
#ifdef FF_KO_EXP
    } else if (true) {
      e = x;
#endif
    } else if ((FF_POLY_PATTERN >> i) & 1) {
      e = poly_exp2_x2(x);
    } else {
      e = make_float2(fast_exp2(x.x), fast_exp2(x.y));
    }
    pk[i] = pack_f16x2(e.x, e.y);
  }
}


#ifndef FF_LEAN_ISSUER
#define FF_LEAN_ISSUER 1
#endif
__device__ __forceinline__ void lean_wait(uint32_t bar, uint32_t parity) {
  uint32_t done;
  asm volatile(
      "{\n\t.reg .pred p;\n\t"
      "mbarrier.try_wait.parity.shared::cta.b64 p, [%1], %2;\n\t"
      "selp.u32 %0, 1, 0, p;\n\t}"
      : "=r"(done)
      : "r"(bar), "r"(parity)
      : "memory");
#ifdef FF_LEAN_SPIN
  for (int n = 0; !done && n < FF_LEAN_SPIN; ++n) done = mbar_test(bar, parity);
#endif
  if (!done) mbar_wait_slow(bar, parity);
}
__device__ __forceinline__ void lean_qk48(uint32_t sbuf, uint64_t qdesc, uint64_t kdesc, uint32_t idesc, uint32_t bar_s_) {
  asm volatile(
      "{\n\t.reg .pred e, pf, pt;\n\t.reg .b64 q1, q2, k1, k2;\n\t"
      "elect.sync _|e, 0xffffffff;\n\t"
      "setp.ne.b32 pf, 0, 0;\n\tsetp.eq.b32 pt, 0, 0;\n\t"
      "add.u64 q1, %1, 2;\n\tadd.u64 q2, %1, 4;\n\tadd.u64 k1, %2, 2;\n\tadd.u64 k2, %2, 4;\n\t"
      "@e tcgen05.mma.cta_group::1.kind::f16 [%0], %1, %2, %3, pf;\n\t"
      "@e tcgen05.mma.cta_group::1.kind::f16 [%0], q1, k1, %3, pt;\n\t"
      "@e tcgen05.mma.cta_group::1.kind::f16 [%0], q2, k2, %3, pt;\n\t"
      "@e tcgen05.commit.cta_group::1.mbarrier::arrive::one.shared::cluster.b64 [%4];\n\t}"
      ::"r"(sbuf), "l"(qdesc), "l"(kdesc), "r"(idesc), "r"(bar_s_)
      : "memory");
}
#ifdef FF_KO_PV1
#define FF_KO_PVSTEPS(x)
#else
#define FF_KO_PVSTEPS(x) x
#endif
#ifdef FF_KO_QK1
#define FF_KO_QKSTEPS(x)
#else
#define FF_KO_QKSTEPS(x) x
#endif
template <bool WITH_QK>
__device__ __forceinline__ void lean_pv_qk48(uint32_t obuf, uint32_t sp, uint64_t vdesc, uint32_t idesc_pv, uint32_t acc0,
                                             uint32_t bar_kve, uint64_t qdesc, uint64_t kdesc, uint32_t idesc_qk,
                                             uint32_t bar_s_) {
  if constexpr (WITH_QK) {
    asm volatile(
        "{\n\t.reg .pred e, p0, pf, pt;\n\t.reg .b64 v1, v2, v3, q1, q2, k1, k2;\n\t.reg .b32 a1, a2, a3;\n\t"
        "elect.sync _|e, 0xffffffff;\n\t"
        "setp.ne.b32 p0, %4, 0;\n\tsetp.ne.b32 pf, 0, 0;\n\tsetp.eq.b32 pt, 0, 0;\n\t"
        "add.u64 v1, %2, 128;\n\tadd.u64 v2, %2, 256;\n\tadd.u64 v3, %2, 384;\n\t"
        "add.u32 a1, %1, 8;\n\tadd.u32 a2, %1, 32;\n\tadd.u32 a3, %1, 40;\n\t"
        "add.u64 q1, %6, 2;\n\tadd.u64 q2, %6, 4;\n\tadd.u64 k1, %7, 2;\n\tadd.u64 k2, %7, 4;\n\t"
        "@e tcgen05.mma.cta_group::1.kind::f16 [%0], [%1], %2, %3, p0;\n\t"
        FF_KO_PVSTEPS("@e tcgen05.mma.cta_group::1.kind::f16 [%0], [a1], v1, %3, pt;\n\t")
        FF_KO_PVSTEPS("@e tcgen05.mma.cta_group::1.kind::f16 [%0], [a2], v2, %3, pt;\n\t")
        FF_KO_PVSTEPS("@e tcgen05.mma.cta_group::1.kind::f16 [%0], [a3], v3, %3, pt;\n\t")
        "@e tcgen05.commit.cta_group::1.mbarrier::arrive::one.shared::cluster.b64 [%5];\n\t"
        "@e tcgen05.mma.cta_group::1.kind::f16 [%1], %6, %7, %8, pf;\n\t"
        FF_KO_QKSTEPS("@e tcgen05.mma.cta_group::1.kind::f16 [%1], q1, k1, %8, pt;\n\t")
        FF_KO_QKSTEPS("@e tcgen05.mma.cta_group::1.kind::f16 [%1], q2, k2, %8, pt;\n\t")
        "@e tcgen05.commit.cta_group::1.mbarrier::arrive::one.shared::cluster.b64 [%9];\n\t}"
        ::"r"(obuf), "r"(sp), "l"(vdesc), "r"(idesc_pv), "r"(acc0), "r"(bar_kve), "l"(qdesc), "l"(kdesc), "r"(idesc_qk),
          "r"(bar_s_)
        : "memory");
  } else {
    asm volatile(
        "{\n\t.reg .pred e, p0, pt;\n\t.reg .b64 v1, v2, v3;\n\t.reg .b32 a1, a2, a3;\n\t"
        "elect.sync _|e, 0xffffffff;\n\t"
        "setp.ne.b32 p0, %4, 0;\n\tsetp.eq.b32 pt, 0, 0;\n\t"
        "add.u64 v1, %2, 128;\n\tadd.u64 v2, %2, 256;\n\tadd.u64 v3, %2, 384;\n\t"
        "add.u32 a1, %1, 8;\n\tadd.u32 a2, %1, 32;\n\tadd.u32 a3, %1, 40;\n\t"
        "@e tcgen05.mma.cta_group::1.kind::f16 [%0], [%1], %2, %3, p0;\n\t"
        "@e tcgen05.mma.cta_group::1.kind::f16 [%0], [a1], v1, %3, pt;\n\t"
        "@e tcgen05.mma.cta_group::1.kind::f16 [%0], [a2], v2, %3, pt;\n\t"
        "@e tcgen05.mma.cta_group::1.kind::f16 [%0], [a3], v3, %3, pt;\n\t"
        "@e tcgen05.commit.cta_group::1.mbarrier::arrive::one.shared::cluster.b64 [%5];\n\t"
        "@e tcgen05.commit.cta_group::1.mbarrier::arrive::one.shared::cluster.b64 [%6];\n\t}"
        ::"r"(obuf), "r"(sp), "l"(vdesc), "r"(idesc_pv), "r"(acc0), "r"(bar_kve), "r"(bar_s_)
        : "memory");
  }
}

__device__ __forceinline__ void lean_pv48_sep(uint32_t obuf, uint32_t pbase, uint64_t vdesc, uint32_t idesc_pv, uint32_t acc0,
                                              uint32_t bar_kve, uint32_t bar_o_) {
  asm volatile(
      "{\n\t.reg .pred e, p0, pt;\n\t.reg .b64 v1, v2, v3;\n\t.reg .b32 a1, a2, a3;\n\t"
      "elect.sync _|e, 0xffffffff;\n\t"
      "setp.ne.b32 p0, %4, 0;\n\tsetp.eq.b32 pt, 0, 0;\n\t"
      "add.u64 v1, %2, 128;\n\tadd.u64 v2, %2, 256;\n\tadd.u64 v3, %2, 384;\n\t"
      "add.u32 a1, %1, 8;\n\tadd.u32 a2, %1, 16;\n\tadd.u32 a3, %1, 24;\n\t"
      "@e tcgen05.mma.cta_group::1.kind::f16 [%0], [%1], %2, %3, p0;\n\t"
      "@e tcgen05.mma.cta_group::1.kind::f16 [%0], [a1], v1, %3, pt;\n\t"
      "@e tcgen05.mma.cta_group::1.kind::f16 [%0], [a2], v2, %3, pt;\n\t"
      "@e tcgen05.mma.cta_group::1.kind::f16 [%0], [a3], v3, %3, pt;\n\t"
      "@e tcgen05.commit.cta_group::1.mbarrier::arrive::one.shared::cluster.b64 [%5];\n\t"
      "@e tcgen05.commit.cta_group::1.mbarrier::arrive::one.shared::cluster.b64 [%6];\n\t}"
      ::"r"(obuf), "r"(pbase), "l"(vdesc), "r"(idesc_pv), "r"(acc0), "r"(bar_kve), "r"(bar_o_)
      : "memory");
}

template <int DPAD, bool P_HILO>
__global__ void __launch_bounds__(Cfg<DPAD, P_HILO>::THREADS, Cfg<DPAD, P_HILO>::MIN_CTAS)
attn_masked_kv_kernel(const __grid_constant__ CUtensorMap tm_q, const __grid_constant__ CUtensorMap tm_k,
                      const __grid_constant__ CUtensorMap tm_v, const KParams p) {
  using C = Cfg<DPAD, P_HILO>;
  extern __shared__ uint8_t smem_raw[];
  const uint32_t smem_base = (smem_u32(smem_raw) + 1023u) & ~1023u;
  const uint32_t sQ = smem_base;
  const uint32_t sKV = smem_base + C::SMEM_Q;
  const uint32_t sACC = sKV + C::NSTAGE * C::SMEM_STAGE;
  const uint32_t sMX = sACC + C::SMEM_ACC;
  const uint32_t bar_base = sMX + C::SMEM_MX;
  const uint32_t bar_q = bar_base;
  const uint32_t bar_s = bar_base + 16, bar_p = bar_base + 32;
  const uint32_t bar_kv_full = bar_base + 48, bar_kv_empty = bar_base + 48 + 8 * C::NSTAGE;
  const uint32_t tmem_slot = bar_base + 48 + 16 * C::NSTAGE;
  const uint32_t bar_f = bar_base + 192, bar_o = bar_base + 208;
  static_assert(48 + 16 * C::NSTAGE + 8 <= 192, "barrier block layout");
  uint8_t* gen_base = smem_raw + (smem_base - smem_u32(smem_raw));
  float* const acc_smem = reinterpret_cast<float*>(gen_base + (sACC - smem_base));
  float* const mx_smem = reinterpret_cast<float*>(gen_base + (sMX - smem_base));
  volatile uint32_t* tmem_slot_ptr =
      reinterpret_cast<volatile uint32_t*>(gen_base + (tmem_slot - smem_base));

  const int warp = threadIdx.x >> 5, lane = threadIdx.x & 31;
  const int q0 = blockIdx.x * BM, head = blockIdx.y, stream = blockIdx.z;
  const FFAttnHeadPlan* plan = p.plan + (size_t)stream * p.heads + head;
  int n_pass = __ldg(&plan->n_pass);
  n_pass = n_pass < 0 ? 0 : (n_pass > FF_MAX_PASS ? FF_MAX_PASS : n_pass);
  const int n_kv_tiles = (p.s_kv + BN - 1) / BN;

  if (threadIdx.x == 0) {
    mbar_init(bar_q, 1);
    mbar_init(bar_s, 1);
    mbar_init(bar_s + 8, 1);
    mbar_init(bar_p, NUM_SOFTMAX_WARPS / 2);
    mbar_init(bar_p + 8, NUM_SOFTMAX_WARPS / 2);
    mbar_init(bar_f, NUM_SOFTMAX_WARPS / 2);
    mbar_init(bar_f + 8, NUM_SOFTMAX_WARPS / 2);
    mbar_init(bar_o, 1);
    mbar_init(bar_o + 8, 1);
    for (int i = 0; i < C::NSTAGE; ++i) {
      mbar_init(bar_kv_full + 8 * i, 1);
      mbar_init(bar_kv_empty + 8 * i, 1);
    }
    asm volatile("fence.mbarrier_init.release.cluster;" ::: "memory");
  }
  if (warp == NUM_SOFTMAX_WARPS) {
    asm volatile("tcgen05.alloc.cta_group::1.sync.aligned.shared::cta.b32 [%0], %1;" ::"r"(tmem_slot),
                 "r"((uint32_t)C::TMEM_COLS)
                 : "memory");
    asm volatile("tcgen05.relinquish_alloc_permit.cta_group::1.sync.aligned;" ::: "memory");
  }
  tc_fence_before();
  __syncthreads();
  tc_fence_after();
  const uint32_t tmem = *tmem_slot_ptr;
#ifdef FF_ENABLE_TRACE
  uint32_t* const tr = g_trace;
  const int trole = warp == NUM_SOFTMAX_WARPS ? 0 : (warp == NUM_SOFTMAX_WARPS + 1 ? 1 : (threadIdx.x == 0 ? 2 : (threadIdx.x == 32 * NUM_SOFTMAX_WARPS - 32 ? 3 : -1)));
#define FF_TRACE(it_, site_) do { if (tr && trole >= 0 && (warp < NUM_SOFTMAX_WARPS || lane == 0)) trace(tr, trole, (uint32_t)(it_), (site_)); } while (0)
#else
#define FF_TRACE(it_, site_) do { } while (0)
#endif
  FF_TRACE(0, 1);
#ifdef FF_TIMELINE
  const int tl_lin = blockIdx.x + gridDim.x * (blockIdx.y + gridDim.y * blockIdx.z);
  const int tl_cta = tl_lin == 4000 ? 0 : 1;
  unsigned long long* const tl = ((tl_lin == 4000 || tl_lin == 4101) && lane == 0 &&
                                  (warp == 0 || warp == NUM_SOFTMAX_WARPS + 1)) ? g_timeline : nullptr;
#endif

  if (warp == NUM_SOFTMAX_WARPS) {
    if (lane == 0) {
      mbar_expect_tx(bar_q, C::NKT * TILE_BYTES);
      for (int kt = 0; kt < C::NKT; ++kt)
        tma_load_4d(sQ + kt * TILE_BYTES, &tm_q, kt * BOX_COLS, head, q0, stream, bar_q);
      int it = 0;
#pragma unroll 1
      for (int ip = 0; ip < n_pass; ++ip) {
        const FFAttnPass ps = plan->pass[ip];
        const PassCtx cx = make_ctx(ps, p, q0);
        if (!cx.active) continue;
#pragma unroll 1
        for (int seg = 0; seg < 2; ++seg) {
          const SegCtx sg = seg ? cx.s1 : cx.s0;
          if (sg.kv < 0) continue;
#pragma unroll 1
          for (int j0 = 0; j0 < n_kv_tiles;) {
            const int cls = tile_class(sg, j0, p), j1 = run_end(sg, j0, cls, p), jb = j0;
            j0 = j1;
            if (tile_skip(cx, sg, cls, p.s_kv)) continue;
#pragma unroll 1
            for (int j = jb; j < j1; ++j) {
            const int stage = it % C::NSTAGE, use = it / C::NSTAGE;
            FF_TRACE(it, 10);
            if (use > 0) mbar_wait_hot<2>(bar_kv_empty + 8 * stage, (use - 1) & 1);
            FF_TRACE(it, 11);
            const uint32_t full = bar_kv_full + 8 * stage;
            const uint32_t sK = sKV + stage * C::SMEM_STAGE, sV = sK + C::NKT * KV_BYTES;
#ifdef FF_KO_TMA
            if (it >= C::NSTAGE) { mbar_arrive(full); ++it; continue; }
#endif
            mbar_expect_tx(full, 2 * C::NKT * KV_BYTES);
            for (int kt = 0; kt < C::NKT; ++kt) {
              tma_load_4d(sK + kt * KV_BYTES, &tm_k, kt * BOX_COLS, head, j * BN, sg.kv, full);
              tma_load_4d(sV + kt * KV_BYTES, &tm_v, kt * BOX_COLS, head, j * BN, sg.kv, full);
            }
            ++it;
            }
          }
        }
      }
    }
  } else if (!C::SELF && warp == NUM_SOFTMAX_WARPS + 1) {
    {
      const bool leader = elect_one();
      constexpr uint32_t idesc_qk = make_idesc(BN, 0);
      constexpr uint32_t idesc_pv = make_idesc(C::DPV, 1, !P_HILO);
      const uint64_t qdesc0 = smem_desc_sw128(sQ, 16);
      const uint64_t kdesc0 = smem_desc_sw128(sKV, 16);
      const uint64_t vdesc0 = smem_desc_sw128(sKV + C::NKT * KV_BYTES, KV_BYTES);
      int pe0 = 0, pe1 = 0, pe2 = 0, n_total = 0;
#pragma unroll
      for (int ip = 0; ip < FF_MAX_PASS; ++ip) {
        if (ip < n_pass) {
          const FFAttnPass ps = plan->pass[ip];
          const PassCtx cx = make_ctx(ps, p, q0);
          if (cx.active) {
#pragma unroll 1
            for (int seg = 0; seg < 2; ++seg) {
              const SegCtx sg = seg ? cx.s1 : cx.s0;
              if (sg.kv < 0) continue;
#pragma unroll 1
              for (int j0 = 0; j0 < n_kv_tiles;) {
                const int cls = tile_class(sg, j0, p), j1 = run_end(sg, j0, cls, p), jb = j0;
                j0 = j1;
                if (!tile_skip(cx, sg, cls, p.s_kv)) n_total += j1 - jb;
              }
            }
          }
        }
        if (ip == 0) pe0 = n_total;
        if (ip == 1) pe1 = n_total;
        if (ip == 2) pe2 = n_total;
      }
      FF_TRACE(0, 20);
      mbar_wait(bar_q, 0);
      if constexpr (C::SEP) {
        tc_fence_after();
        if (n_total > 0) { lean_wait(bar_kv_full, 0); tc_fence_after(); lean_qk48(tmem + C::TMEM_S, qdesc0, kdesc0, idesc_qk, bar_s); }
        if (n_total > 1) {
          lean_wait(bar_kv_full + 8, 0);
          tc_fence_after();
          lean_qk48(tmem + C::TMEM_S + BN, qdesc0, kdesc0 + (uint64_t)(C::SMEM_STAGE >> 4), idesc_qk, bar_s + 8);
        }
        uint32_t gph = 0;
        int t = 0;
#pragma unroll 1
        while (t < n_total) {
#pragma unroll
          for (int u = 0; u < 4; ++u) {
            if (t < n_total) {
              const int pstart = t >= pe2 ? pe2 : (t >= pe1 ? pe1 : (t >= pe0 ? pe0 : 0));
              const uint32_t acc0 = (t - pstart < 2) ? 0u : 1u;
              FF_TL(1, t, 0);
              if (t + 2 < n_total) {
                lean_wait(bar_kv_full + 8 * ((u + 2) & 3), u < 2 ? gph : gph ^ 1u);
                lean_wait(bar_f + 8 * (u & 1), (uint32_t)((u >> 1) & 1));
                FF_TL(1, t, 1);
                tc_fence_after();
                lean_qk48(tmem + C::TMEM_S + BN * (u & 1), qdesc0, kdesc0 + (uint64_t)((((u + 2) & 3) * C::SMEM_STAGE) >> 4),
                          idesc_qk, bar_s + 8 * (u & 1));
              }
              FF_TL(1, t, 2);
              lean_wait(bar_p, (uint32_t)(u & 1));
              FF_TL(1, t, 3);
              tc_fence_after();
              lean_pv48_sep(tmem + C::TMEM_O + C::DPV * (u & 1), tmem + C::TMEM_P, vdesc0 + (uint64_t)((u * C::SMEM_STAGE) >> 4),
                            idesc_pv, acc0, bar_kv_empty + 8 * u, bar_o + 8 * (u & 1));
              FF_TL(1, t, 4);
              ++t;
            }
          }
          gph ^= 1u;
        }
        __syncwarp();
      } else if constexpr (FF_LEAN_ISSUER && DPAD == 48 && !P_HILO && C::NSTAGE == 4) {
        tc_fence_after();
        if (n_total > 0) { lean_wait(bar_kv_full, 0); tc_fence_after(); lean_qk48(tmem + C::TMEM_S, qdesc0, kdesc0, idesc_qk, bar_s); }
        if (n_total > 1) {
          lean_wait(bar_kv_full + 8, 0);
          tc_fence_after();
          lean_qk48(tmem + C::TMEM_S + BN, qdesc0, kdesc0 + (uint64_t)(C::SMEM_STAGE >> 4), idesc_qk, bar_s + 8);
        }
        uint32_t gph = 0;
        int t = 0;
#pragma unroll 1
        while (t < n_total) {
#pragma unroll
          for (int u = 0; u < 4; ++u) {
            if (t < n_total) {
              const bool more = t + 2 < n_total;
              const int pstart = t >= pe2 ? pe2 : (t >= pe1 ? pe1 : (t >= pe0 ? pe0 : 0));
              const uint32_t acc0 = (t - pstart < 2) ? 0u : 1u;
              const uint32_t sp = tmem + C::TMEM_S + BN * (u & 1);
              const uint32_t obuf = tmem + C::TMEM_O + C::DPV * (u & 1);
              const uint64_t vd = vdesc0 + (uint64_t)((u * C::SMEM_STAGE) >> 4);
              const uint64_t kd = kdesc0 + (uint64_t)((((u + 2) & 3) * C::SMEM_STAGE) >> 4);
              if (more) lean_wait(bar_kv_full + 8 * ((u + 2) & 3), u < 2 ? gph : gph ^ 1u);
              lean_wait(bar_p + 8 * (u & 1), (uint32_t)((u >> 1) & 1));
              tc_fence_after();
              if (more) lean_pv_qk48<true>(obuf, sp, vd, idesc_pv, acc0, bar_kv_empty + 8 * u, qdesc0, kd, idesc_qk, bar_s + 8 * (u & 1));
              else lean_pv_qk48<false>(obuf, sp, vd, idesc_pv, acc0, bar_kv_empty + 8 * u, 0, 0, 0, bar_s + 8 * (u & 1));
              ++t;
            }
          }
          gph ^= 1u;
        }
        __syncwarp();
      } else {
      int qk_t = 0;
      uint32_t q_stage = 0, q_phase = 0, p_stage = 0;
      auto wait_kv = [&]() { mbar_wait_hot<1>(bar_kv_full + 8 * q_stage, q_phase); };
      auto issue_qk = [&]() {
        const uint64_t kd = kdesc0 + ((q_stage * (uint32_t)C::SMEM_STAGE) >> 4);
        const uint32_t sbuf = tmem + C::TMEM_S + BN * (qk_t & 1);
#pragma unroll
        for (int ks = 0; ks < DPAD / 16; ++ks) {
          const uint32_t qoff = (ks >> 2) * TILE_BYTES + (ks & 3) * 32;
          const uint32_t koff = (ks >> 2) * KV_BYTES + (ks & 3) * 32;
          mma_ss(sbuf, qdesc0 + (qoff >> 4), kd + (koff >> 4), idesc_qk, ks > 0);
        }
        tc_commit(bar_s + 8 * (qk_t & 1));
      };
      auto advance_qk = [&]() {
        ++qk_t;
        if (++q_stage == (uint32_t)C::NSTAGE) { q_stage = 0; q_phase ^= 1u; }
      };
#pragma unroll 1
      for (int k = 0; k < 2 && qk_t < n_total; ++k) {
        wait_kv();
        tc_fence_after();
        if (leader) issue_qk();
        __syncwarp();
        advance_qk();
      }
#pragma unroll 1
      for (int t = 0; t < n_total; ++t) {
        const bool more = qk_t < n_total;
        const int pstart = t >= pe2 ? pe2 : (t >= pe1 ? pe1 : (t >= pe0 ? pe0 : 0));
        const bool first_of_parity = t - pstart < 2;
        const uint64_t vd = vdesc0 + ((p_stage * (uint32_t)C::SMEM_STAGE) >> 4);
        const uint32_t pbase = tmem + C::TMEM_S + BN * (t & 1);
        const uint32_t obuf = tmem + C::TMEM_O + C::DPV * (t & 1);
        bool kv_ready = more && __all_sync(0xffffffffu, mbar_test(bar_kv_full + 8 * q_stage, q_phase));
        FF_TL(1, t, 0);
        mbar_wait_hot<1>(bar_p + 8 * (t & 1), (t >> 1) & 1);
        FF_TL(1, t, 3);
        if (more && !kv_ready) kv_ready = __all_sync(0xffffffffu, mbar_test(bar_kv_full + 8 * q_stage, q_phase));
        tc_fence_after();
        if (leader) {
#pragma unroll
          for (int ks = 0; ks < BN / 16; ++ks) {
            const uint64_t vdesc = vd + ((ks * 2048) >> 4);
            if constexpr (P_HILO) {
              mma_ts(obuf, pbase + 16 * ks, vdesc, idesc_pv, (!first_of_parity || ks > 0) ? 1u : 0u);
              mma_ts(obuf, pbase + 16 * ks + 8, vdesc, idesc_pv, 1u);
            } else {
              mma_ts(obuf, pbase + 32 * (ks >> 1) + 8 * (ks & 1), vdesc, idesc_pv,
                     (!first_of_parity || ks > 0) ? 1u : 0u);
            }
          }
          tc_commit(bar_kv_empty + 8 * p_stage);
          if (kv_ready) issue_qk();
          else if (!more) tc_commit(bar_s + 8 * (t & 1));
        }
        __syncwarp();
        if (more && !kv_ready) {
          wait_kv();
          tc_fence_after();
          if (leader) issue_qk();
          __syncwarp();
        }
        if (more) advance_qk();
        FF_TL(1, t, 4);
        if (++p_stage == (uint32_t)C::NSTAGE) p_stage = 0;
      }
      __syncwarp();
      }
    }
  } else {
    const int wq = warp & 3;
    const int wg = warp >> 2;
    const int rloc = 32 * wq + lane;
    const int row = q0 + rloc;
    const uint32_t tlane = tmem + ((uint32_t)(wq * 32) << 16);
    const uint32_t tS = tlane + C::TMEM_S + BN * wg;
    const uint32_t tO = tlane + C::TMEM_O + C::DPV * wg;
    const uint32_t tOx = tlane + C::TMEM_O + C::DPV * (wg ^ 1);
    float* const acc_row = acc_smem + (size_t)rloc * C::ACC_LD;
    bool acc_started = false;
    int it = 0;
    int n_total = 0;
    [[maybe_unused]] constexpr uint32_t s_idesc_qk = make_idesc(BN, 0);
    [[maybe_unused]] constexpr uint32_t s_idesc_pv = make_idesc(C::DPV, 1, !P_HILO);
    [[maybe_unused]] const uint64_t s_qdesc0 = smem_desc_sw128(sQ, 16);
    [[maybe_unused]] const uint64_t s_kdesc0 = smem_desc_sw128(sKV, 16);
    [[maybe_unused]] const uint64_t s_vdesc0 = smem_desc_sw128(sKV + C::NKT * KV_BYTES, KV_BYTES);
    if constexpr (C::SELF) {
      if (wq == 0) {
#pragma unroll 1
        for (int ip = 0; ip < n_pass; ++ip) {
          const FFAttnPass ps = plan->pass[ip];
          const PassCtx cx = make_ctx(ps, p, q0);
          if (!cx.active) continue;
#pragma unroll 1
          for (int seg = 0; seg < 2; ++seg) {
            const SegCtx sg = seg ? cx.s1 : cx.s0;
            if (sg.kv < 0) continue;
#pragma unroll 1
            for (int j0 = 0; j0 < n_kv_tiles;) {
              const int cls = tile_class(sg, j0, p), j1 = run_end(sg, j0, cls, p), jb = j0;
              j0 = j1;
              if (!tile_skip(cx, sg, cls, p.s_kv)) n_total += j1 - jb;
            }
          }
        }
        n_total = __shfl_sync(0xffffffffu, n_total, 0);
        if (wg < n_total) {
          mbar_wait(bar_q, 0);
          lean_wait(bar_kv_full + 8 * wg, 0);
          tc_fence_after();
          lean_qk48(tmem + C::TMEM_S + BN * wg, s_qdesc0, s_kdesc0 + (uint64_t)((wg * C::SMEM_STAGE) >> 4), s_idesc_qk,
                    bar_s + 8 * wg);
        }
      }
    }
#pragma unroll 1
    for (int ip = 0; ip < n_pass; ++ip) {
      const FFAttnPass ps = plan->pass[ip];
      const PassCtx cx = make_ctx(ps, p, q0);
      if (!cx.active) continue;
      uint32_t rb = 0;
      if (ps.row_mask >= 0 && row < p.s_q)
        rb = (__ldg(p.bitmasks + (size_t)ps.row_mask * p.mask_words + (row >> 5)) >> (row & 31)) & 1u;
      const bool rowflip = cx.rowxor && rb;
      float m_used = -INFINITY;
      int n_mine = 0, last_mine = 0;
      const int it_pass0 = it;
#pragma unroll 1
      for (int seg = 0; seg < 2; ++seg) {
        const SegCtx sg = seg ? cx.s1 : cx.s0;
        if (sg.kv < 0) continue;
        const bool flip = sg.kinv != rowflip;
        const bool uniform = uniform_for(cx, sg, flip, p.s_kv);
        const float sc = uniform ? 0.f : p.scale_log2;
#pragma unroll 1
        for (int j0 = 0; j0 < n_kv_tiles;) {
          const int cls = tile_class(sg, j0, p), j1 = run_end(sg, j0, cls, p), jb = j0;
          j0 = j1;
          if (tile_skip(cx, sg, cls, p.s_kv)) continue;
          const bool row_ok_cls = row_allowed(cls, flip, uniform);
          int j = jb + (((it ^ wg) & 1) ? 1 : 0);
          int itj = it + (j - jb);
          it += j1 - jb;
#pragma unroll 1
          for (; j < j1; j += 2, itj += 2) {
            FF_TRACE(itj, 30);
            FF_TL(0, itj, 0);
            mbar_wait_hot<0>(bar_s + 8 * wg, (itj >> 1) & 1);
            FF_TL(0, itj, 1);
            FF_TRACE(itj, 31);
            tc_fence_after();
            uint32_t kb_lo = 0xffffffffu, kb_hi = 0xffffffffu;
            if (cls == TILE_MIX) {
#pragma unroll
              for (int w = 0; w < 2; ++w) {
                const int kbase = j * BN + 32 * w;
                const int rem = p.s_kv - kbase;
                const uint32_t valid = rem >= 32 ? 0xffffffffu : (rem <= 0 ? 0u : ((1u << rem) - 1u));
                uint32_t kb = 0xffffffffu;
                if (sg.kmask >= 0 && !uniform && rem > 0) {
                  if (sg.prefix) {
                    const int t = sg.T - kbase;
                    kb = t >= 32 ? 0xffffffffu : (t <= 0 ? 0u : ((1u << t) - 1u));
                  } else {
                    kb = __ldg(p.bitmasks + (size_t)sg.kmask * p.mask_words + (kbase >> 5));
                  }
                  if (flip) kb = ~kb;
                }
                if (w == 0) kb_lo = kb & valid; else kb_hi = kb & valid;
              }
            }
            float mt, sb[32];
            {
              float sa[32];
              tmem_ld32(tS, sa);
#ifdef FF_LD_BOTH
              tmem_ld32(tS + 32, sb);
#endif
              tmem_wait_ld32(sa);
              float m0, m1;
              if (cls != TILE_MIX) {
                m0 = fmaxf(sa[0], sa[1]);
                m1 = fmaxf(sa[2], sa[3]);
#pragma unroll
                for (int i = 4; i < 32; i += 4) {
                  m0 = fmaxf(m0, fmaxf(sa[i], sa[i + 1]));
                  m1 = fmaxf(m1, fmaxf(sa[i + 2], sa[i + 3]));
                }
              } else {
                m0 = m1 = -INFINITY;
#pragma unroll
                for (int i = 0; i < 32; i += 2) {
                  m0 = fmaxf(m0, (kb_lo >> i) & 1u ? sa[i] : -INFINITY);
                  m1 = fmaxf(m1, (kb_lo >> (i + 1)) & 1u ? sa[i + 1] : -INFINITY);
                }
              }
              mt = fmaxf(m0, m1);
            }
            {
#ifdef FF_KO_LD2
#pragma unroll
              for (int i = 0; i < 32; ++i) sb[i] = mt + (float)i;
#else
#ifndef FF_LD_BOTH
              tmem_ld32(tS + 32, sb);
#endif
              tmem_wait_ld32(sb);
#endif
              float m0, m1;
              if (cls != TILE_MIX) {
                m0 = fmaxf(sb[0], sb[1]);
                m1 = fmaxf(sb[2], sb[3]);
#pragma unroll
                for (int i = 4; i < 32; i += 4) {
                  m0 = fmaxf(m0, fmaxf(sb[i], sb[i + 1]));
                  m1 = fmaxf(m1, fmaxf(sb[i + 2], sb[i + 3]));
                }
              } else {
                m0 = m1 = -INFINITY;
#pragma unroll
                for (int i = 0; i < 32; i += 2) {
                  m0 = fmaxf(m0, (kb_hi >> i) & 1u ? sb[i] : -INFINITY);
                  m1 = fmaxf(m1, (kb_hi >> (i + 1)) & 1u ? sb[i + 1] : -INFINITY);
                }
              }
              mt = fmaxf(mt, fmaxf(m0, m1));
              if (cls != TILE_MIX && !row_ok_cls) mt = -INFINITY;
#ifdef FF_KO_MAX
              mt = 0.f;
#endif
            }
            FF_TL(0, itj, 2);
            const float mts = uniform ? 0.f : mt * p.scale_log2;
            float alpha = 1.f;
            bool grow = false;
            if (n_mine == 0) {
              m_used = mts;
            } else if (mts > m_used + rescale_threshold<P_HILO>()) {
              alpha = fast_exp2(m_used - mts);
              m_used = mts;
              grow = true;
            }
            const bool any_grow = __any_sync(0xffffffffu, grow);
            auto rescale_o = [&]() {
#pragma unroll
              for (int c = 0; c < C::DPV / 16; ++c) {
                float o[16];
                uint32_t ob[16];
                tmem_ld16(tO + 16 * c, o);
                tmem_wait_ld16(o);
#pragma unroll
                for (int i = 0; i < 16; ++i) ob[i] = __float_as_uint(o[i] * alpha);
                tmem_st16(tO + 16 * c, ob);
              }
            };
            if (!C::SEP && any_grow) rescale_o();
            FF_TL(0, itj, 3);
            const float nb = (cls == TILE_MIX || row_ok_cls) ? -m_used : -INFINITY;
            uint32_t pk[(P_HILO || C::SEP) ? 32 : 16];
#pragma unroll
            for (int hb = 1; hb >= 0; --hb) {
              float sa[32];
#ifdef FF_KO_REREAD
              const float* sv = sb;
#else
              if (hb == 0) {
                tmem_ld32(tS, sa);
                tmem_wait_ld32(sa);
                if constexpr (C::SEP) {
                  tc_fence_before();
                  __syncwarp();
                  if (lane == 0) mbar_arrive(bar_f + 8 * wg);
                }
              }
              const float* sv = hb ? sb : sa;
#endif
              const uint32_t kbits = hb ? kb_hi : kb_lo;
              if (cls != TILE_MIX) {
#pragma unroll
                for (int jj = 0; jj < 2; ++jj) {
                  if constexpr (P_HILO) softmax_chunk_hilo<false>(sv + 16 * jj, pk + 16 * jj, sc, nb, 0u);
                  else softmax_chunk_f16<false>(sv + 16 * jj, pk + (C::SEP ? 16 * hb : 0) + 8 * jj, sc, nb, 0u);
                }
              } else {
#pragma unroll
                for (int jj = 0; jj < 2; ++jj) {
                  const uint32_t bits = (kbits >> (16 * jj)) & 0xffffu;
                  if constexpr (P_HILO) softmax_chunk_hilo<true>(sv + 16 * jj, pk + 16 * jj, sc, nb, bits);
                  else softmax_chunk_f16<true>(sv + 16 * jj, pk + (C::SEP ? 16 * hb : 0) + 8 * jj, sc, nb, bits);
                }
              }
              if constexpr (P_HILO) {
                tmem_st16(tS + 32 * hb, *reinterpret_cast<const uint32_t(*)[16]>(pk));
                tmem_st16(tS + 32 * hb + 16, *reinterpret_cast<const uint32_t(*)[16]>(pk + 16));
              } else if constexpr (!C::SEP) {
                tmem_st16(tS + 32 * hb, *reinterpret_cast<const uint32_t(*)[16]>(pk));
              }
            }
            if constexpr (C::SEP) {
              if (itj >= 1) {
                const uint32_t bo = bar_o + 8 * (wg ^ 1), po = (uint32_t)(((itj - 1) >> 1) & 1);
                if (!mbar_test(bo, po)) mbar_wait(bo, po);
              }
              tc_fence_after();
              if (any_grow) rescale_o();
              tmem_st16(tlane + C::TMEM_P, *reinterpret_cast<const uint32_t(*)[16]>(pk));
              tmem_st16(tlane + C::TMEM_P + 16, *reinterpret_cast<const uint32_t(*)[16]>(pk + 16));
            }
            FF_TL(0, itj, 4);
            tmem_wait_st();
            FF_TL(0, itj, 5);
            tc_fence_before();
            if constexpr (C::SELF) {
              named_bar_sync(3 + wg, 128);
              if (wq == 0) {
                const int stg = itj & 3, nxt = (itj + 2) & 3;
                const bool more = itj + 2 < n_total;
                if (more) lean_wait(bar_kv_full + 8 * nxt, (uint32_t)(((itj + 2) >> 2) & 1));
                tc_fence_after();
                const uint32_t sp = tmem + C::TMEM_S + BN * wg;
                const uint32_t obuf = tmem + C::TMEM_O + C::DPV * wg;
                const uint64_t vd = s_vdesc0 + (uint64_t)((stg * C::SMEM_STAGE) >> 4);
                const uint64_t kd = s_kdesc0 + (uint64_t)((nxt * C::SMEM_STAGE) >> 4);
                const uint32_t acc0 = n_mine == 0 ? 0u : 1u;
                if (more) lean_pv_qk48<true>(obuf, sp, vd, s_idesc_pv, acc0, bar_kv_empty + 8 * stg, s_qdesc0, kd, s_idesc_qk, bar_s + 8 * wg);
                else lean_pv_qk48<false>(obuf, sp, vd, s_idesc_pv, acc0, bar_kv_empty + 8 * stg, 0, 0, 0, bar_s + 8 * wg);
              }
            } else {
              __syncwarp();
              if (lane == 0) mbar_arrive(C::SEP ? bar_p : bar_p + 8 * wg);
            }
            FF_TL(0, itj, 6);
            FF_TRACE(itj, 34);
            ++n_mine;
            last_mine = itj;
          }
        }
      }
      if (it == it_pass0) continue;
      FF_TRACE(it, 35);
      if constexpr (C::SEP) {
        const int L = it - 1;
        mbar_wait(bar_o + 8 * (L & 1), (uint32_t)((L >> 1) & 1));
        tc_fence_after();
      } else if (n_mine > 0) mbar_wait_hot<0>(bar_s + 8 * wg, ((last_mine + 2) >> 1) & 1);
      FF_TRACE(it, 36);
      mx_smem[wg * BM + rloc] = n_mine > 0 ? m_used : -INFINITY;
      tc_fence_before();
      named_bar_sync(1, 32 * NUM_SOFTMAX_WARPS);
      tc_fence_after();
      const float m_other = mx_smem[(wg ^ 1) * BM + rloc];
      const float m_all = fmaxf(m_used, m_other);
      const bool wrote_mine = n_mine > 0, wrote_other = (it - it_pass0) - n_mine > 0;
      const float a_mine = (wrote_mine && m_used > -INFINITY) ? fast_exp2(m_used - m_all) : 0.f;
      const float a_other = (wrote_other && m_other > -INFINITY) ? fast_exp2(m_other - m_all) : 0.f;
      float l = 0.f;
      if (wrote_mine) l = a_mine * tmem_ld1_wait(tO + p.head_dim);
      if (wrote_other) l = fmaf(a_other, tmem_ld1_wait(tOx + p.head_dim), l);
      float coef = ps.weight;
      if (ps.flags & FF_PASS_ROW_WEIGHT) coef = rb ? coef : 0.f;
      coef = l > 0.f ? coef / l : 0.f;
      const float c_mine = coef * a_mine, c_other = coef * a_other;
#pragma unroll
      for (int c = 0; c < DPAD / 16; ++c) {
        if ((c & 1) != wg) continue;
        float r[16];
#pragma unroll
        for (int i = 0; i < 16; ++i) r[i] = acc_started ? acc_row[16 * c + i] : 0.f;
        if (wrote_mine) {
          float o[16];
          tmem_ld16(tO + 16 * c, o);
          tmem_wait_ld16(o);
#pragma unroll
          for (int i = 0; i < 16; ++i) r[i] = fmaf(c_mine, o[i], r[i]);
        }
        if (wrote_other) {
          float o[16];
          tmem_ld16(tOx + 16 * c, o);
          tmem_wait_ld16(o);
#pragma unroll
          for (int i = 0; i < 16; ++i) r[i] = fmaf(c_other, o[i], r[i]);
        }
#pragma unroll
        for (int i = 0; i < 16; i += 4)
          *reinterpret_cast<float4*>(acc_row + 16 * c + i) = make_float4(r[i], r[i + 1], r[i + 2], r[i + 3]);
      }
      acc_started = true;
      tc_fence_before();
      named_bar_sync(2, 32 * NUM_SOFTMAX_WARPS);
      tc_fence_after();
    }
    {
      const bool row_ok = row < p.s_q;
      const size_t o_off = ((size_t)stream * p.s_q + (row_ok ? row : 0)) * ((size_t)p.heads * p.head_dim) +
                           (size_t)head * p.head_dim;
#pragma unroll
      for (int c = 0; c < DPAD / 16; ++c) {
        if ((c & 1) != wg) continue;
        float o[16];
#pragma unroll
        for (int i = 0; i < 16; ++i) o[i] = acc_started ? acc_row[16 * c + i] : 0.f;
#pragma unroll
        for (int g = 0; g < 2; ++g) {
          if (row_ok && 16 * c + 8 * g < p.head_dim) {
            if (p.out_dtype == FF_DT_BF16) {
              uint4 v;
              v.x = pack_bf16x2(o[8 * g + 0], o[8 * g + 1]);
              v.y = pack_bf16x2(o[8 * g + 2], o[8 * g + 3]);
              v.z = pack_bf16x2(o[8 * g + 4], o[8 * g + 5]);
              v.w = pack_bf16x2(o[8 * g + 6], o[8 * g + 7]);
              *reinterpret_cast<uint4*>(static_cast<__nv_bfloat16*>(p.out) + o_off + 16 * c + 8 * g) = v;
            } else {
              float4* dst = reinterpret_cast<float4*>(static_cast<float*>(p.out) + o_off + 16 * c + 8 * g);
              dst[0] = make_float4(o[8 * g + 0], o[8 * g + 1], o[8 * g + 2], o[8 * g + 3]);
              dst[1] = make_float4(o[8 * g + 4], o[8 * g + 5], o[8 * g + 6], o[8 * g + 7]);
            }
          }
        }
      }
    }
  }
  FF_TRACE(0, 90);
  tc_fence_before();
  __syncthreads();
  if (warp == NUM_SOFTMAX_WARPS) {
    tc_fence_after();
    asm volatile("tcgen05.dealloc.cta_group::1.sync.aligned.b32 %0, %1;" ::"r"(tmem), "r"((uint32_t)C::TMEM_COLS)
                 : "memory");
  }
}

#include "attn_ring.cuh"
#include "attn_t32.cuh"

typedef CUresult (*EncodeTiledFn)(CUtensorMap*, CUtensorMapDataType, cuuint32_t, void*, const cuuint64_t*,
                                  const cuuint64_t*, const cuuint32_t*, const cuuint32_t*, CUtensorMapInterleave,
                                  CUtensorMapSwizzle, CUtensorMapL2promotion, CUtensorMapFloatOOBfill);

EncodeTiledFn get_encode_fn() {
  static EncodeTiledFn fn = nullptr;
  if (!fn) {
    void* ptr = nullptr;
    cudaDriverEntryPointQueryResult qres;
    if (cudaGetDriverEntryPoint("cuTensorMapEncodeTiled", &ptr, cudaEnableDefault, &qres) == cudaSuccess &&
        qres == cudaDriverEntryPointSuccess)
      fn = reinterpret_cast<EncodeTiledFn>(ptr);
  }
  return fn;
}

int make_map(CUtensorMap* map, const void* base, int streams, int S, int heads, int d, int box_rows,
             bool f16 = false) {
  EncodeTiledFn enc = get_encode_fn();
  if (!enc) return ff::fail(FF_E_CUDA, "cuTensorMapEncodeTiled entry point not found");
  const cuuint64_t C = (cuuint64_t)heads * d;
  cuuint64_t dims[4] = {(cuuint64_t)d, (cuuint64_t)heads, (cuuint64_t)S, (cuuint64_t)streams};
  cuuint64_t strides[3] = {(cuuint64_t)d * 2, C * 2, (cuuint64_t)S * C * 2};
  cuuint32_t box[4] = {BOX_COLS, 1, (cuuint32_t)box_rows, 1};
  cuuint32_t estr[4] = {1, 1, 1, 1};
  CUresult r = enc(map, f16 ? CU_TENSOR_MAP_DATA_TYPE_FLOAT16 : CU_TENSOR_MAP_DATA_TYPE_BFLOAT16, 4, const_cast<void*>(base), dims, strides, box, estr,
                   CU_TENSOR_MAP_INTERLEAVE_NONE, CU_TENSOR_MAP_SWIZZLE_128B, CU_TENSOR_MAP_L2_PROMOTION_L2_128B,
                   CU_TENSOR_MAP_FLOAT_OOB_FILL_NONE);
  if (r != CUDA_SUCCESS)
    return ff::fail(FF_E_CUDA, "cuTensorMapEncodeTiled failed (CUresult %d) dims=[%d,%d,%d,%d]", (int)r, d, heads, S,
                    streams);
  return FF_OK;
}

template <typename K>
int ensure_smem(K kernel, int bytes, std::atomic<uint64_t>& done) {
  int dev = 0;
  cudaGetDevice(&dev);
  const uint64_t bit = 1ull << (dev & 63);
  if (done.load(std::memory_order_acquire) & bit) return FF_OK;
  cudaError_t e = cudaFuncSetAttribute(kernel, cudaFuncAttributeMaxDynamicSharedMemorySize, bytes);
  if (e != cudaSuccess) return ff::fail(FF_E_CUDA, "cudaFuncSetAttribute(smem=%d): %s", bytes, cudaGetErrorString(e));
  done.fetch_or(bit, std::memory_order_release);
  return FF_OK;
}

template <int DPAD, bool HILO>
int launch(const CUtensorMap& mq, const CUtensorMap& mk, const CUtensorMap& mv, const KParams& kp, int n_streams,
           cudaStream_t st) {
  using C = Cfg<DPAD, HILO>;
  static std::atomic<uint64_t> configured{0};
  int rc = ensure_smem(attn_masked_kv_kernel<DPAD, HILO>, C::SMEM_BYTES, configured);
  if (rc != FF_OK) return rc;
  dim3 grid((kp.s_q + BM - 1) / BM, kp.heads, n_streams);
  attn_masked_kv_kernel<DPAD, HILO><<<grid, C::THREADS, C::SMEM_BYTES, st>>>(mq, mk, mv, kp);
  return ff::check_launch("ff_attn_masked_kv");
}

int sm_count() {
  static std::atomic<int> cached[64];
  int dev = 0;
  cudaGetDevice(&dev);
  int n = cached[dev & 63].load(std::memory_order_relaxed);
  if (n == 0) {
    cudaDeviceGetAttribute(&n, cudaDevAttrMultiProcessorCount, dev);
    if (n <= 0) n = 148;
    cached[dev & 63].store(n, std::memory_order_relaxed);
  }
  return n;
}

template <int DPAD, int NWG, int NBUF, bool TOKEN>
int launch_ring(const CUtensorMap& mq, const CUtensorMap& mk, const CUtensorMap& mv, const KParams& kp, int n_streams,
                cudaStream_t st) {
  using C = RCfg<DPAD, NWG, NBUF>;
  static std::atomic<uint64_t> configured{0};
  int rc = ensure_smem(attn_ring_kernel<DPAD, NWG, NBUF, TOKEN>, C::SMEM_BYTES, configured);
  if (rc != FF_OK) return rc;
  const int n_items = kp.n_qtiles * kp.heads * n_streams;
  int ctas = sm_count() * C::MIN_CTAS;
  if (ctas > n_items) ctas = n_items;
  attn_ring_kernel<DPAD, NWG, NBUF, TOKEN><<<ctas, C::NUM_THREADS, C::SMEM_BYTES, st>>>(mq, mk, mv, kp);
  return ff::check_launch("ff_attn_masked_kv (ring kernel)");
}

int launch_t32(const CUtensorMap& mq, const CUtensorMap& mk, const CUtensorMap& mv, const KParams& kp, int n_streams, cudaStream_t st) {
  static std::atomic<uint64_t> configured{0};
  int rc = ensure_smem(attn_t32_kernel, T32::SMEM_BYTES, configured);
  if (rc != FF_OK) return rc;
  dim3 grid((kp.s_q + BM - 1) / BM, kp.heads, n_streams);
  attn_t32_kernel<<<grid, NUM_THREADS, T32::SMEM_BYTES, st>>>(mq, mk, mv, kp);
  return ff::check_launch("ff_attn_masked_kv (32-key tiles)");
}

int t32_mode() {
  static int mode = -1;
  if (mode < 0) {
    const char* e = getenv("FF_ATTN_T32");
    mode = e ? (atoi(e) != 0) : FF_T32_DEFAULT;
  }
  return mode;
}

int ring_mode() {
  static int mode = -1;
  if (mode < 0) {
    const char* e = getenv("FF_ATTN_RING");
    mode = e ? atoi(e) : FF_RING_DEFAULT;
    if (mode < 0 || mode > 7) mode = FF_RING_DEFAULT;
  }
  return mode;
}

}

extern "C" int ff_debug_set_timeline(void* device_ptr) {
#ifdef FF_TIMELINE
  cudaError_t e = cudaMemcpyToSymbol(g_timeline, &device_ptr, sizeof(void*));
  if (e != cudaSuccess) return ff::fail(FF_E_CUDA, "ff_debug_set_timeline: %s", cudaGetErrorString(e));
  return FF_OK;
#else
  (void)device_ptr;
  return ff::fail(FF_E_UNSUPPORTED, "ff_debug_set_timeline: library built without -DFF_TIMELINE");
#endif
}

extern "C" int ff_debug_set_trace(void* device_visible_ptr) {
#ifndef FF_ENABLE_TRACE
  if (device_visible_ptr) return ff::fail(FF_E_UNSUPPORTED, "ff_debug_set_trace: library built without FF_TRACE=1");
#endif
  cudaError_t e = cudaMemcpyToSymbol(g_trace, &device_visible_ptr, sizeof(void*));
  if (e != cudaSuccess) return ff::fail(FF_E_CUDA, "ff_debug_set_trace: %s", cudaGetErrorString(e));
  return FF_OK;
}

extern "C" int ff_attn_v_head_stride(int32_t head_dim) {
  if (head_dim <= 8) return Cfg<16, false>::DPV;
  if (head_dim <= 40) return Cfg<48, false>::DPV;
  if (head_dim <= 80) return Cfg<80, false>::DPV;
  return Cfg<160, false>::DPV;
}

extern "C" int ff_attn_masked_kv(const FFAttnArgs* a, void* stream) {
  FF_REQUIRE(a != nullptr, "ff_attn_masked_kv: null args");
  FF_REQUIRE(a->q && a->k && a->v && a->out && a->plan, "ff_attn_masked_kv: null pointer");
  FF_REQUIRE(a->n_streams > 0 && a->n_kv_streams > 0 && a->heads > 0 && a->s_q > 0 && a->s_kv > 0,
             "ff_attn_masked_kv: bad shape");
  FF_REQUIRE(a->head_dim >= 8 && a->head_dim % 8 == 0, "ff_attn_masked_kv: head_dim=%d must be a multiple of 8",
             a->head_dim);
  if (a->head_dim > 160) return ff::fail(FF_E_UNSUPPORTED, "ff_attn_masked_kv: head_dim=%d > 160", a->head_dim);
  FF_REQUIRE(a->heads <= 65535 && a->n_streams <= 65535, "ff_attn_masked_kv: heads / streams exceed grid limits");
  FF_REQUIRE(ff::aligned16(a->q) && ff::aligned16(a->k) && ff::aligned16(a->v) && ff::aligned16(a->out),
             "ff_attn_masked_kv: q/k/v/out must be 16-byte aligned");
  FF_REQUIRE(a->out_dtype == FF_DT_BF16 || a->out_dtype == FF_DT_F32, "ff_attn_masked_kv: bad out_dtype");
  FF_REQUIRE(a->v_dtype == FF_DT_BF16 || a->v_dtype == FF_DT_F16, "ff_attn_masked_kv: v_dtype must be bf16 or f16");
  FF_REQUIRE(a->scale > 0.f, "ff_attn_masked_kv: scale must be positive");
  if (a->n_masks > 0) {
    FF_REQUIRE(a->bitmasks && a->mask_popcount, "ff_attn_masked_kv: n_masks>0 but no bitmasks / popcounts");
    const int need = ((a->s_q > a->s_kv ? a->s_q : a->s_kv) + 31) / 32;
    FF_REQUIRE(a->mask_words >= need, "ff_attn_masked_kv: mask_words=%d < %d", a->mask_words, need);
  }
  int dev = 0, major = 0;
  cudaGetDevice(&dev);
  {
    static std::atomic<int> cached_major[64];
    major = cached_major[dev & 63].load(std::memory_order_relaxed);
    if (major == 0) {
      cudaDeviceGetAttribute(&major, cudaDevAttrComputeCapabilityMajor, dev);
      cached_major[dev & 63].store(major, std::memory_order_relaxed);
    }
  }
  if (major != 10) return ff::fail(FF_E_ARCH, "ff_attn_masked_kv: needs an sm_100 device (got sm_%d*)", major);

  alignas(64) CUtensorMap mq, mk, mv;
  int rc;
  if ((rc = make_map(&mq, a->q, a->n_streams, a->s_q, a->heads, a->head_dim, BM)) != FF_OK) return rc;
  const bool v_f16 = a->v_dtype == FF_DT_F16;
  const bool use_t32 = v_f16 && a->head_dim > 8 && a->head_dim <= 40 && t32_mode() != 0;
  const int kv_rows = use_t32 ? TBN : BN;
  if ((rc = make_map(&mk, a->k, a->n_kv_streams, a->s_kv, a->heads, a->head_dim, kv_rows)) != FF_OK) return rc;
  FF_REQUIRE(a->v_head_stride == ff_attn_v_head_stride(a->head_dim),
             "ff_attn_masked_kv: V must be staged by ff_kv_gather_cast (v_head_stride=%d, expected %d)",
             a->v_head_stride, ff_attn_v_head_stride(a->head_dim));
  if ((rc = make_map(&mv, a->v, a->n_kv_streams, a->s_kv, a->heads, a->v_head_stride, kv_rows, v_f16)) != FF_OK) return rc;

  KParams kp;
  kp.plan = a->plan;
  kp.bitmasks = a->bitmasks;
  kp.popc = a->mask_popcount;
  kp.out = a->out;
  kp.heads = a->heads;
  kp.head_dim = a->head_dim;
  kp.s_q = a->s_q;
  kp.s_kv = a->s_kv;
  kp.mask_words = a->mask_words;
  kp.out_dtype = a->out_dtype;
  kp.n_kv_streams = a->n_kv_streams;
  kp.n_streams = a->n_streams;
  kp.n_qtiles = (a->s_q + BM - 1) / BM;
  kp.scale_log2 = a->scale * 1.4426950408889634f;
  cudaStream_t st = static_cast<cudaStream_t>(stream);
  const int d = a->head_dim;
  if (v_f16) {
    if (d <= 8) return launch<16, false>(mq, mk, mv, kp, a->n_streams, st);
    if (use_t32) return launch_t32(mq, mk, mv, kp, a->n_streams, st);
    const int rm = ring_mode();
    if (rm == 1 && d <= 40) return launch_ring<48, 1, 3, false>(mq, mk, mv, kp, a->n_streams, st);
    if (rm == 2 && d <= 40) return launch_ring<48, 2, 4, false>(mq, mk, mv, kp, a->n_streams, st);
    if (rm == 3 && d <= 40) return launch_ring<48, 3, 5, false>(mq, mk, mv, kp, a->n_streams, st);
    if (rm == 7 && d <= 40) return launch_ring<48, 4, 5, false>(mq, mk, mv, kp, a->n_streams, st);
    if (rm == 4 && d <= 40) return launch_ring<48, 3, 5, true>(mq, mk, mv, kp, a->n_streams, st);
    if (rm == 5 && d <= 40) return launch_ring<48, 2, 4, true>(mq, mk, mv, kp, a->n_streams, st);
    if (d > 40 && d <= 80 && (rm == 4 || rm == 5)) return launch_ring<80, 2, 3, true>(mq, mk, mv, kp, a->n_streams, st);
    if (d > 40 && d <= 80 && rm != 0) return launch_ring<80, 2, 3, false>(mq, mk, mv, kp, a->n_streams, st);
    if (d <= 40) return launch<48, false>(mq, mk, mv, kp, a->n_streams, st);
    if (d <= 80) return launch<80, false>(mq, mk, mv, kp, a->n_streams, st);
    return launch<160, false>(mq, mk, mv, kp, a->n_streams, st);
  }
  if (d <= 8) return launch<16, true>(mq, mk, mv, kp, a->n_streams, st);
  if (d <= 40) return launch<48, true>(mq, mk, mv, kp, a->n_streams, st);
  if (d <= 80) return launch<80, true>(mq, mk, mv, kp, a->n_streams, st);
  return launch<160, true>(mq, mk, mv, kp, a->n_streams, st);
}
```

### freefine_b200/plans.py

```python
from __future__ import annotations

import numpy as np

from ._lib import (FF_MAX_PASS, FF_PASS_KEY2_INVERT, FF_PASS_KEY2_PREFIX, FF_PASS_KEY_INVERT, FF_PASS_KEY_PREFIX,
                   FF_PASS_ROW_WEIGHT, FF_PASS_ROW_XOR, PLAN_BYTES)

PASS_DTYPE = np.dtype([("kv_stream", "<i4"), ("key_mask", "<i4"), ("row_mask", "<i4"), ("flags", "<u4"),
                       ("weight", "<f4"), ("kv_stream2", "<i4"), ("key_mask2", "<i4"), ("reserved", "<i4")])
PLAN_DTYPE = np.dtype([("n_pass", "<i4"), ("reserved", "<i4", (3,)), ("passes", PASS_DTYPE, (FF_MAX_PASS,))])
assert PLAN_DTYPE.itemsize == PLAN_BYTES


def q0_masked(heads: int, stream_in_edit: int, head: int) -> bool:
    return ((heads * stream_in_edit + head) % 4) in (0, 2)


def _empty(n_streams: int, heads: int) -> np.ndarray:
    p = np.zeros((n_streams, heads), PLAN_DTYPE)
    p["passes"]["kv_stream"] = -1
    p["passes"]["kv_stream2"] = -1
    p["passes"]["key_mask"] = -1
    p["passes"]["key_mask2"] = -1
    p["passes"]["row_mask"] = -1
    return p


def _add(plan, s, h, kv, weight, key_mask=-1, row_mask=-1, flags=0, kv2=-1, key_mask2=-1):
    e = plan[s, h]
    i = int(e["n_pass"])
    if i >= FF_MAX_PASS:
        raise ValueError(f"more than {FF_MAX_PASS} passes for stream {s} head {h}")
    ps = e["passes"][i]
    ps["kv_stream"], ps["key_mask"], ps["row_mask"], ps["flags"] = kv, key_mask, row_mask, flags
    ps["weight"], ps["kv_stream2"], ps["key_mask2"] = weight, kv2, key_mask2
    plan[s, h]["n_pass"] = i + 1


def plain_plan(n_streams: int, heads: int, kv_of=None) -> np.ndarray:
    p = _empty(n_streams, heads)
    for s in range(n_streams):
        for h in range(heads):
            _add(p, s, h, s if kv_of is None else kv_of(s), 1.0)
    return p


def tca_plan(n_edits: int, heads: int, method: str, cg, src_id, tgt_id, kind: str = "edit",
             prefix: bool = False) -> np.ndarray:
    pf = FF_PASS_KEY_PREFIX if prefix else 0
    if method not in ("tca", "mmsa"):
        raise ValueError(f"method must be 'tca' or 'mmsa', got {method!r}")
    if kind not in ("edit", "bg"):
        raise ValueError(kind)
    p = _empty(4 * n_edits, heads)
    w_ref = 1.0 if method == "mmsa" else float(cg)
    w_self = 0.0 if method == "mmsa" else 1.0 - float(cg)
    for e in range(n_edits):
        for sl in range(4):
            s = 4 * e + sl
            r = 4 * e + (1 if sl < 2 else 3)
            for h in range(heads):
                masked = q0_masked(heads, sl, h)
                if not masked and r == s:
                    _add(p, s, h, s, 1.0 if method == "mmsa" else w_ref + w_self)
                    continue
                if masked and kind == "edit":
                    _add(p, s, h, r, w_ref, key_mask=src_id(e), row_mask=tgt_id(e),
                         flags=FF_PASS_KEY_INVERT | FF_PASS_ROW_XOR | pf)
                elif masked:
                    _add(p, s, h, r, w_ref, key_mask=src_id(e), flags=FF_PASS_KEY_INVERT | pf)
                else:
                    _add(p, s, h, r, w_ref)
                if method == "tca":
                    _add(p, s, h, s, w_self)
    return p


def compose_plan(n_src: int, heads: int, method: str, cg, src_ids, tgt_ids, prefix: bool = False) -> np.ndarray:
    if method not in ("tca", "mmsa"):
        raise ValueError(method)
    B = n_src + 2
    p = _empty(B, heads)
    for s in range(B):
        for h in range(heads):
            if s in (0, B - 1):
                w_new = 1.0 if method == "mmsa" else float(cg)
                for i in range(n_src):
                    _add(p, s, h, 1 + i, w_new, key_mask=src_ids[i], row_mask=tgt_ids[i],
                         flags=FF_PASS_ROW_WEIGHT | (FF_PASS_KEY_PREFIX if prefix else 0))
                if method == "tca":
                    _add(p, s, h, s, 1.0 - float(cg))
            else:
                _add(p, s, h, s, 1.0)
    return p


def style_align_plan(n_edits: int, heads: int, src_id=None, prefix: bool = False, bg: bool = False) -> np.ndarray:
    p = _empty(4 * n_edits, heads)
    for e in range(n_edits):
        for sl in range(4):
            s = 4 * e + sl
            r = 4 * e + (1 if sl < 2 else 3)
            for h in range(heads):
                masked = src_id is not None and q0_masked(heads, sl, h)
                if bg and masked:
                    _add(p, s, h, r, 1.0, key_mask=src_id(e), flags=FF_PASS_KEY_INVERT | (FF_PASS_KEY_PREFIX if prefix else 0))
                    continue
                km2 = src_id(e) if masked else -1
                _add(p, s, h, s, 1.0, kv2=r, key_mask2=km2, flags=FF_PASS_KEY2_PREFIX if (prefix and km2 >= 0) else 0)
    return p


def kv_sort_index(key_bits, stream_masks) -> "torch.Tensor":
    import torch
    n, S = key_bits.shape
    order = torch.sort(key_bits.to(torch.uint8), dim=1, descending=True, stable=True).indices
    ident = torch.arange(S, device=key_bits.device)
    rows = [order[m] if m >= 0 else ident for m in stream_masks]
    base = (torch.arange(len(stream_masks), device=key_bits.device) * S)[:, None]
    return (torch.stack(rows) + base).reshape(-1)


def algorithmic_flops(plan: np.ndarray, s_q: int, s_kv: int, d: int, popcount=None) -> float:
    total = 0.0
    for e in plan.reshape(-1):
        for ps in e["passes"][: int(e["n_pass"])]:
            flags = int(ps["flags"])
            n_r = int(popcount[int(ps["row_mask"])]) if ps["row_mask"] >= 0 else 0
            if ps["key_mask"] >= 0:
                n_k = int(popcount[int(ps["key_mask"])])
                c0 = s_kv - n_k if flags & FF_PASS_KEY_INVERT else n_k
            else:
                c0 = s_kv
            if flags & FF_PASS_ROW_WEIGHT:
                pairs = n_r * c0
            elif flags & FF_PASS_ROW_XOR and ps["key_mask"] >= 0:
                pairs = (s_q - n_r) * c0 + n_r * (s_kv - c0)
            else:
                pairs = s_q * c0
            if ps["kv_stream2"] >= 0:
                if ps["key_mask2"] >= 0:
                    n2 = int(popcount[int(ps["key_mask2"])])
                    pairs += s_q * (s_kv - n2 if flags & FF_PASS_KEY2_INVERT else n2)
                else:
                    pairs += s_q * s_kv
            total += 4.0 * d * pairs
    return total


def describe(plan: np.ndarray) -> str:
    out = []
    for s in range(plan.shape[0]):
        for h in range(plan.shape[1]):
            e = plan[s, h]
            ps = ", ".join(
                f"kv{int(q['kv_stream'])}" + (f"+kv{int(q['kv_stream2'])}" if q["kv_stream2"] >= 0 else "") +
                f"[k{int(q['key_mask'])} r{int(q['row_mask'])} f{int(q['flags'])}]*{float(q['weight']):.3f}"
                for q in e["passes"][: int(e["n_pass"])])
            out.append(f"s{s}h{h}: {ps}")
    return "\n".join(out)


__all__ = ["PASS_DTYPE", "PLAN_DTYPE", "q0_masked", "plain_plan", "tca_plan", "compose_plan", "style_align_plan",
           "kv_sort_index", "algorithmic_flops", "describe", "FF_PASS_KEY_INVERT", "FF_PASS_ROW_XOR", "FF_PASS_ROW_WEIGHT",
           "FF_PASS_KEY2_INVERT", "FF_PASS_KEY_PREFIX", "FF_PASS_KEY2_PREFIX"]
```

### include/freefine_b200.h

```cpp
#ifndef FREEFINE_B200_H_
#define FREEFINE_B200_H_

#include <stdint.h>

#ifdef __cplusplus
extern "C" {
#endif

#define FF_VERSION 100

enum {
  FF_OK = 0,
  FF_E_INVALID = -1,
  FF_E_UNSUPPORTED = -2,
  FF_E_CUDA = -3,
  FF_E_ARCH = -4
};

enum { FF_DT_F32 = 0, FF_DT_BF16 = 1, FF_DT_F16 = 2 };

int ff_version(void);
const char* ff_last_error(void);

#define FF_MAX_PASS 4

enum {
  FF_PASS_KEY_INVERT = 1u,
  FF_PASS_ROW_XOR = 2u,
  FF_PASS_ROW_WEIGHT = 4u,
  FF_PASS_KEY2_INVERT = 8u,
  FF_PASS_KEY_PREFIX = 16u,
  FF_PASS_KEY2_PREFIX = 32u
};

typedef struct FFAttnPass {
  int32_t kv_stream;
  int32_t key_mask;
  int32_t row_mask;
  uint32_t flags;
  float weight;
  int32_t kv_stream2;
  int32_t key_mask2;
  int32_t reserved;
} FFAttnPass;

typedef struct FFAttnHeadPlan {
  int32_t n_pass;
  int32_t reserved[3];
  FFAttnPass pass[FF_MAX_PASS];
} FFAttnHeadPlan;

typedef struct FFAttnArgs {
  const void* q;
  const void* k;
  const void* v;
  void* out;
  const FFAttnHeadPlan* plan;
  const uint32_t* bitmasks;
  const int32_t* mask_popcount;
  int32_t n_streams, n_kv_streams, heads, head_dim;
  int32_t s_q, s_kv;
  int32_t n_masks, mask_words;
  int32_t out_dtype;
  float scale;
  int32_t v_dtype;
  int32_t v_head_stride;
} FFAttnArgs;

int ff_attn_masked_kv(const FFAttnArgs* h_args, void* stream);

int ff_attn_plain_smallkv(const void* q, const void* k, const void* v, void* out, int32_t n_streams, int32_t heads,
                          int32_t head_dim, int32_t s_q, int32_t s_kv, float scale, int32_t out_dtype, void* stream);

int ff_attn_v_head_stride(int32_t head_dim);

int ff_kv_gather_cast(const void* k, const void* v, const int64_t* row_index, void* k_out, void* v_out,
                      int32_t v_out_dtype, int64_t rows, int32_t heads, int32_t head_dim, void* stream);

int ff_mask_downsample_pack(const uint8_t* masks, int32_t n, int32_t H, int32_t W, int32_t h, int32_t w,
                            uint32_t* bits, int32_t words, int32_t* popcount, void* stream);

int ff_mask_prep(const uint8_t* shifted, const uint8_t* ori, const uint8_t* draw, const uint8_t* cons, int32_t E,
                 int32_t H, int32_t W, int32_t h, int32_t w, int32_t use_auto_draw, int32_t reduce_inp_artifacts,
                 uint8_t* fg, uint8_t* shifted_out, uint8_t* ori_out, uint8_t* comp_lat, uint8_t* lvar_lat, void* stream);

int ff_dilate_mask(const uint8_t* mask, uint8_t* out, int32_t N, int32_t H, int32_t W, int32_t k, void* stream);

int ff_upsample2x_nhwc(const void* x, void* y, int32_t N, int32_t H, int32_t W, int32_t C, void* stream);
int ff_concat_nhwc(const void* a, const void* b, void* out, int64_t M, int32_t Ca, int32_t Cb, void* stream);

int ff_linear_bias_residual(const void* x, const void* w, const void* bias, const void* res, void* out, int64_t M, int32_t N,
                            int32_t K, void* workspace, int64_t ws_bytes, void* stream);

int ff_warp_affine_blend(const void* src, const float* theta, const uint8_t* mask_src, const void* bg, void* out,
                         uint8_t* mask_out, int32_t N, int32_t C, int32_t H, int32_t W, int32_t dH, int32_t dW,
                         int32_t mode, int32_t dtype, void* stream);

int ff_ddim_cfg_step(const float* eps4, const float* x, const float* noise, const uint8_t* cfg_mask,
                     const uint8_t* var_mask, float guidance_scale, float sqrt_1m_at, float sqrt_at, float sqrt_ap,
                     float c_ddim, float c_ddpm, float sigma, float* x_prev, float* pred_x0, int32_t n_edits,
                     int32_t C, int32_t h, int32_t w, void* stream);

int ff_ddim_step(const float* eps2, const float* x, const float* noise, const uint8_t* var_mask, float sqrt_1m_at,
                 float sqrt_at, float sqrt_ap, float c_ddim, float c_ddpm, float sigma, float* x_prev,
                 float* pred_x0, int32_t n_edits, int32_t C, int32_t h, int32_t w, void* stream);

int ff_ddim_cfg_step_compose(const float* eps, int32_t streams_per_edit, const float* x, const float* noise,
                             const uint8_t* cfg_mask, const uint8_t* var_mask, float guidance_scale, float sqrt_1m_at,
                             float sqrt_at, float sqrt_ap, float c_ddim, float c_ddpm, float sigma, float* x_prev,
                             float* pred_x0, int32_t n_edits, int32_t C, int32_t h, int32_t w, void* stream);

int ff_ddim_inv_step(const float* eps, const float* x, float sqrt_1m_at, float sqrt_at, float sqrt_an, float c_next,
                     float* x_next, float* pred_x0, int64_t n, void* stream);

int ff_cross_region_blend(void* hs, const uint32_t* bitmasks, int32_t mask_words, const int32_t* region_mask,
                          int32_t n_edits, int32_t S, int32_t C, int32_t dtype, void* stream);


int64_t ff_group_norm_ws_bytes(int32_t N, int32_t G);
int ff_group_norm_nhwc(const void* x, const float* add_nc, int64_t add_ld, const void* gamma, const void* beta, void* y,
                       void* workspace, int32_t N, int32_t HW, int32_t C, int32_t G, float eps, int32_t silu, void* stream);

int ff_bias_residual_nhwc(const void* h, const void* bias, const void* res, void* out, int64_t M, int32_t C,
                          void* stream);

int ff_geglu(const void* h, void* out, int64_t M, int32_t F, void* stream);

int ff_layer_norm(const void* x, const void* gamma, const void* beta, void* y, int64_t M, int32_t C, float eps,
                  void* stream);

int ff_debug_set_trace(void* device_visible_ptr);
int ff_debug_set_timeline(void* device_ptr);

#ifdef __cplusplus
}
#endif
#endif
```

Baseline: 2.738.

## Fuse masked-self and full-self TCA passes into one split-softmax sweep

```diff
diff --git a/freefine_b200/_lib.py b/freefine_b200/_lib.py
--- a/freefine_b200/_lib.py
+++ b/freefine_b200/_lib.py
@@ -9,12 +9,12 @@
 FF_MAX_PASS = 4
 FF_DT_F32, FF_DT_BF16, FF_DT_F16 = 0, 1, 2
 FF_PASS_KEY_INVERT, FF_PASS_ROW_XOR, FF_PASS_ROW_WEIGHT, FF_PASS_KEY2_INVERT = 1, 2, 4, 8
-FF_PASS_KEY_PREFIX, FF_PASS_KEY2_PREFIX = 16, 32
+FF_PASS_KEY_PREFIX, FF_PASS_KEY2_PREFIX, FF_PASS_SPLIT_SELF = 16, 32, 64
 
 
 class FFAttnPass(C.Structure):
     _fields_ = [("kv_stream", C.c_int32), ("key_mask", C.c_int32), ("row_mask", C.c_int32), ("flags", C.c_uint32),
-                ("weight", C.c_float), ("kv_stream2", C.c_int32), ("key_mask2", C.c_int32), ("reserved", C.c_int32)]
+                ("weight", C.c_float), ("kv_stream2", C.c_int32), ("key_mask2", C.c_int32), ("weight2", C.c_float)]
 
 
 class FFAttnHeadPlan(C.Structure):
diff --git a/freefine_b200/attention.py b/freefine_b200/attention.py
--- a/freefine_b200/attention.py
+++ b/freefine_b200/attention.py
@@ -86,6 +86,7 @@
         self.sort_keys = True
         self.p_operand = "f16"
         self.small_kv_kernel = os.environ.get("FF_ATTN_SMALLKV", "1") != "0"
+        self.tca_split_self = os.environ.get("FF_TCA_SPLIT_SELF", "1") != "0"
         self._tables = {}
         self._plans = {}
 
@@ -218,8 +219,10 @@
             raise ValueError(f"{E} edits in the stream batch but masks for {bits.shape[0]} rows")
         cg = None if self.method == 'mmsa' else float(self.context_guidance)
         pf = self.sort_keys
-        plan = self._plan((kind, E, self.heads, self.method, cg, pf),
-                          lambda: plans.tca_plan(E, self.heads, self.method, cg, src_id, tgt_id, kind=kind, prefix=pf))
+        split = self.tca_split_self
+        plan = self._plan((kind, E, self.heads, self.method, cg, pf, split),
+                          lambda: plans.tca_plan(E, self.heads, self.method, cg, src_id, tgt_id, kind=kind, prefix=pf,
+                                                 split_self=split))
         kv_index = None
         if pf:
             kv_index = self._kv_index(kind, S, bits, [src_id(s // 4) if s % 2 else -1 for s in range(B)])
diff --git a/freefine_b200/csrc/attn_ring.cuh b/freefine_b200/csrc/attn_ring.cuh
--- a/freefine_b200/csrc/attn_ring.cuh
+++ b/freefine_b200/csrc/attn_ring.cuh
@@ -20,7 +20,8 @@
   static constexpr int ACC_LD = DPAD + 4;
   static constexpr int SMEM_ACC = BM * ACC_LD * 4;
   static constexpr int SMEM_MX = NWG > 1 ? NWG * BM * 4 : 0;
-  static constexpr int SMEM_FIXED = 2 * SMEM_Q + SMEM_ACC + SMEM_MX + 1024  + 512 ;
+  static constexpr int SMEM_PRE = NWG * BM * 8;
+  static constexpr int SMEM_FIXED = 2 * SMEM_Q + SMEM_ACC + SMEM_MX + SMEM_PRE + 1024  + 512 ;
   static constexpr int SMEM_BUDGET = MIN_CTAS == 2 ? 113 * 1024 : 227 * 1024;
   static constexpr int NST_FIT = (SMEM_BUDGET - SMEM_FIXED) / (2 * SMEM_K);
   static constexpr int NST = (NST_FIT >= 2 * NBUF && 2 * NBUF <= 8) ? 2 * NBUF : NBUF;
@@ -41,13 +42,14 @@
 
 struct TileIter {
   const FFAttnHeadPlan* plan;
-  int n_pass, q0, n_kv_tiles;
+  int n_pass, n_vpass, q0, n_kv_tiles;
+  bool any_split;
   int ip, seg, jn, j, j1;
   bool seg_live, valid;
   PassCtx cx;
   SegCtx sg;
   __device__ __forceinline__ void init(const FFAttnHeadPlan* pl, int np, int q0_, int nkt, const KParams& p) {
-    plan = pl; n_pass = np; q0 = q0_; n_kv_tiles = nkt;
+    plan = pl; n_pass = np; n_vpass = n_virtual_passes(pl, np, any_split); q0 = q0_; n_kv_tiles = nkt;
     ip = -1; seg = 1; jn = 0; j = 0; j1 = 0; seg_live = false; valid = true;
     seek(p);
   }
@@ -65,9 +67,9 @@
         seg = 1; sg = cx.s1; seg_live = cx.active && sg.kv >= 0; jn = 0;
         continue;
       }
-      if (++ip >= n_pass) { valid = false; return; }
-      const FFAttnPass ps = plan->pass[ip];
-      cx = make_ctx(ps, p, q0);
+      if (++ip >= n_vpass) { valid = false; return; }
+      const VPass vp = virtual_pass(plan, n_pass, any_split, ip, p);
+      cx = make_ctx(vp.ps, p, q0, vp.kind);
       seg = 0; sg = cx.s0; seg_live = cx.active && sg.kv >= 0; jn = 0;
     }
   }
@@ -78,11 +80,13 @@
                                            int& pe0, int& pe1, int& pe2) {
   int n_total = 0;
   pe0 = pe1 = pe2 = 0;
+  bool any_split;
+  const int n_vpass = n_virtual_passes(plan, n_pass, any_split);
 #pragma unroll
   for (int ip = 0; ip < FF_MAX_PASS; ++ip) {
-    if (ip < n_pass) {
-      const FFAttnPass ps = plan->pass[ip];
-      const PassCtx cx = make_ctx(ps, p, q0);
+    if (ip < n_vpass) {
+      const VPass vp = virtual_pass(plan, n_pass, any_split, ip, p);
+      const PassCtx cx = make_ctx(vp.ps, p, q0, vp.kind);
       if (cx.active) {
 #pragma unroll 1
         for (int seg = 0; seg < 2; ++seg) {
@@ -222,7 +226,8 @@
   const uint32_t sV = sK + NST * C::SMEM_K;
   const uint32_t sACC = sV + NST * C::SMEM_K;
   const uint32_t sMX = sACC + C::SMEM_ACC;
-  const uint32_t bar_base = sMX + C::SMEM_MX;
+  const uint32_t sPRE = sMX + C::SMEM_MX;
+  const uint32_t bar_base = sPRE + C::SMEM_PRE;
   const uint32_t bar_qf = bar_base;
   const uint32_t bar_qe = bar_base + 16;
   const uint32_t bar_s = bar_base + 32;
@@ -440,15 +445,18 @@
       const FFAttnHeadPlan* plan = item_plan(head, stream, n_pass);
       const int row = q0 + rloc;
       bool acc_started = false;
+      bool any_split;
+      const int n_vpass = n_virtual_passes(plan, n_pass, any_split);
       int it = 0;
       int my_next = wg;
       my_b = (base + wg) % NBUF;
       my_ph = (uint32_t)(((base + wg) / NBUF) & 1);
       s_ready = false;
 #pragma unroll 1
-      for (int ip = 0; ip < n_pass; ++ip) {
-        const FFAttnPass ps = plan->pass[ip];
-        const PassCtx cx = make_ctx(ps, p, q0);
+      for (int ip = 0; ip < n_vpass; ++ip) {
+        const VPass vp = virtual_pass(plan, n_pass, any_split, ip, p);
+        const FFAttnPass& ps = vp.ps;
+        const PassCtx cx = make_ctx(ps, p, q0, vp.kind);
         if (!cx.active) continue;
         uint32_t rb = 0;
         if (ps.row_mask >= 0 && row < p.s_q)
@@ -606,6 +614,7 @@
         tc_fence_after();
         float cg_[NWG];
         bool wrote[NWG];
+        float keep;
         if constexpr (NWG > 1) {
           mx_smem[wg * BM + rloc] = n_mine > 0 ? m_used : -INFINITY;
           tc_fence_before();
@@ -626,24 +635,22 @@
             cg_[g] = a;
             if (wrote[g]) l = fmaf(a, tmem_ld1_wait(tlane + C::TMEM_O + C::DPV * g + p.head_dim), l);
           }
-          float coef = ps.weight;
-          if (ps.flags & FF_PASS_ROW_WEIGHT) coef = rb ? coef : 0.f;
-          coef = l > 0.f ? coef / l : 0.f;
+          const float coef = pass_coef(virtual_pass(plan, n_pass, any_split, ip, p), rb, m_all, l, acc_started,
+                                       mx_smem + C::SMEM_MX / 4 + 2 * threadIdx.x, keep);
 #pragma unroll
           for (int g = 0; g < NWG; ++g) cg_[g] *= coef;
         } else {
           wrote[0] = n_mine > 0;
           const float l = (wrote[0] && m_used > -INFINITY) ? tmem_ld1_wait(tO + p.head_dim) : 0.f;
-          float coef = ps.weight;
-          if (ps.flags & FF_PASS_ROW_WEIGHT) coef = rb ? coef : 0.f;
-          cg_[0] = l > 0.f ? coef / l : 0.f;
+          cg_[0] = pass_coef(virtual_pass(plan, n_pass, any_split, ip, p), rb, m_used, l, acc_started,
+                             mx_smem + C::SMEM_MX / 4 + 2 * threadIdx.x, keep);
         }
 #pragma unroll
         for (int c = 0; c < DPAD / 16; ++c) {
           if (c % NWG != wg) continue;
           float r[16];
 #pragma unroll
-          for (int i = 0; i < 16; ++i) r[i] = acc_started ? acc_row[16 * c + i] : 0.f;
+          for (int i = 0; i < 16; ++i) r[i] = keep != 0.f ? keep * acc_row[16 * c + i] : 0.f;
 #pragma unroll
           for (int g = 0; g < NWG; ++g) {
             if (!wrote[g]) continue;
diff --git a/freefine_b200/csrc/attn_t32.cuh b/freefine_b200/csrc/attn_t32.cuh
--- a/freefine_b200/csrc/attn_t32.cuh
+++ b/freefine_b200/csrc/attn_t32.cuh
@@ -8,8 +8,8 @@
   static constexpr int TMEM_S = 0, TMEM_P = 4 * TBN, TMEM_O = 4 * TBN + 2 * (TBN / 2), TMEM_COLS = 256;
   static_assert(TMEM_O + 2 * DPV == 256, "TMEM budget: 4 S buffers, 2 P regions, 2 accumulators");
   static constexpr int SMEM_Q = TILE_BYTES, SMEM_STAGE = 2 * KVB;
-  static constexpr int ACC_LD = DPAD + 4, SMEM_ACC = BM * ACC_LD * 4, SMEM_MX = 2 * BM * 4;
-  static constexpr int SMEM_BYTES = SMEM_Q + NST * SMEM_STAGE + SMEM_ACC + SMEM_MX + 1024 + 512;
+  static constexpr int ACC_LD = DPAD + 4, SMEM_ACC = BM * ACC_LD * 4, SMEM_MX = 2 * BM * 4, SMEM_PRE = 2 * BM * 8;
+  static constexpr int SMEM_BYTES = SMEM_Q + NST * SMEM_STAGE + SMEM_ACC + SMEM_MX + SMEM_PRE + 1024 + 512;
   static_assert(SMEM_BYTES <= 113 * 1024, "two CTAs per SM");
 };
 
@@ -53,7 +53,8 @@
   const uint32_t sKV = smem_base + C::SMEM_Q;
   const uint32_t sACC = sKV + C::NST * C::SMEM_STAGE;
   const uint32_t sMX = sACC + C::SMEM_ACC;
-  const uint32_t bar_base = sMX + C::SMEM_MX;
+  const uint32_t sPRE = sMX + C::SMEM_MX;
+  const uint32_t bar_base = sPRE + C::SMEM_PRE;
   const uint32_t bar_q = bar_base;
   const uint32_t bar_s = bar_base + 16;
   const uint32_t bar_p = bar_base + 48;
@@ -71,6 +72,8 @@
   const FFAttnHeadPlan* plan = p.plan + (size_t)stream * p.heads + head;
   int n_pass = __ldg(&plan->n_pass);
   n_pass = n_pass < 0 ? 0 : (n_pass > FF_MAX_PASS ? FF_MAX_PASS : n_pass);
+  bool any_split;
+  const int n_vpass = n_virtual_passes(plan, n_pass, any_split);
   const int n_kv_tiles = (p.s_kv + TBN - 1) / TBN;
 
   if (threadIdx.x == 0) {
@@ -103,9 +106,9 @@
       tma_load_4d(sQ, &tm_q, 0, head, q0, stream, bar_q);
       int it = 0;
 #pragma unroll 1
-      for (int ip = 0; ip < n_pass; ++ip) {
-        const FFAttnPass ps = plan->pass[ip];
-        const PassCtx cx = make_ctx(ps, p, q0);
+      for (int ip = 0; ip < n_vpass; ++ip) {
+        const VPass vp = virtual_pass(plan, n_pass, any_split, ip, p);
+        const PassCtx cx = make_ctx(vp.ps, p, q0, vp.kind);
         if (!cx.active) continue;
 #pragma unroll 1
         for (int seg = 0; seg < 2; ++seg) {
@@ -139,9 +142,9 @@
     int pe0 = 0, pe1 = 0, pe2 = 0, n_total = 0;
 #pragma unroll
     for (int ip = 0; ip < FF_MAX_PASS; ++ip) {
-      if (ip < n_pass) {
-        const FFAttnPass ps = plan->pass[ip];
-        const PassCtx cx = make_ctx(ps, p, q0);
+      if (ip < n_vpass) {
+        const VPass vp = virtual_pass(plan, n_pass, any_split, ip, p);
+        const PassCtx cx = make_ctx(vp.ps, p, q0, vp.kind);
         if (cx.active) {
 #pragma unroll 1
           for (int seg = 0; seg < 2; ++seg) {
@@ -209,9 +212,10 @@
     bool acc_started = false;
     int it = 0;
 #pragma unroll 1
-    for (int ip = 0; ip < n_pass; ++ip) {
-      const FFAttnPass ps = plan->pass[ip];
-      const PassCtx cx = make_ctx(ps, p, q0);
+    for (int ip = 0; ip < n_vpass; ++ip) {
+      const VPass vp = virtual_pass(plan, n_pass, any_split, ip, p);
+      const FFAttnPass& ps = vp.ps;
+      const PassCtx cx = make_ctx(ps, p, q0, vp.kind);
       if (!cx.active) continue;
       uint32_t rb = 0;
       if (ps.row_mask >= 0 && row < p.s_q)
@@ -346,16 +350,16 @@
       float l = 0.f;
       if (wrote_mine) l = a_mine * tmem_ld1_wait(tO + p.head_dim);
       if (wrote_other) l = fmaf(a_other, tmem_ld1_wait(tOx + p.head_dim), l);
-      float coef = ps.weight;
-      if (ps.flags & FF_PASS_ROW_WEIGHT) coef = rb ? coef : 0.f;
-      coef = l > 0.f ? coef / l : 0.f;
+      float keep;
+      const float coef = pass_coef(virtual_pass(plan, n_pass, any_split, ip, p), rb, m_all, l, acc_started,
+                                   mx_smem + C::SMEM_MX / 4 + 2 * threadIdx.x, keep);
       const float c_mine = coef * a_mine, c_other = coef * a_other;
 #pragma unroll
       for (int c = 0; c < C::DPAD / 16; ++c) {
         if ((c & 1) != wg) continue;
         float r[16];
 #pragma unroll
-        for (int i = 0; i < 16; ++i) r[i] = acc_started ? acc_row[16 * c + i] : 0.f;
+        for (int i = 0; i < 16; ++i) r[i] = keep != 0.f ? keep * acc_row[16 * c + i] : 0.f;
         if (wrote_mine) {
           float o[16];
           tmem_ld16(tO + 16 * c, o);
diff --git a/freefine_b200/csrc/attn_tcgen05.cu b/freefine_b200/csrc/attn_tcgen05.cu
--- a/freefine_b200/csrc/attn_tcgen05.cu
+++ b/freefine_b200/csrc/attn_tcgen05.cu
@@ -48,7 +48,10 @@
   static constexpr int ACC_LD = DPAD <= 80 ? DPAD + 4 : DPAD;
   static constexpr int SMEM_ACC = BM * ACC_LD * 4;
   static constexpr int SMEM_MX = 2 * BM * 4;
-  static constexpr int SMEM_BYTES = SMEM_Q + NSTAGE * SMEM_STAGE + SMEM_ACC + SMEM_MX + 1024  + 256 ;
+  static constexpr bool SPLIT = DPAD <= 80;
+  static constexpr int SMEM_PRE = SPLIT ? 2 * BM * 8 : 0;
+  static constexpr int SMEM_BYTES = SMEM_Q + NSTAGE * SMEM_STAGE + SMEM_ACC + SMEM_MX + SMEM_PRE + 1024  +
+                                    256 ;
   static_assert(SMEM_BYTES <= 227 * 1024, "shared memory budget");
   static constexpr int MIN_CTAS = (SMEM_BYTES <= 113 * 1024 && TMEM_COLS == 256) ? 2 : 1;
   static constexpr bool SELF = FF_SELF_ISSUE && !SEP && DPAD == 48 && !HILO && NSTAGE == 4;
@@ -325,20 +328,98 @@
   bool has_rf0, has_rf1;
 };
 
-__device__ __forceinline__ PassCtx make_ctx(const FFAttnPass& ps, const KParams& p, int q0) {
+enum { VP_PLAIN = 0, VP_SPLIT_PRE = 1, VP_SPLIT_SUF = 2 };
+struct VPass {
+  FFAttnPass ps;
+  int kind;
+};
+
+__device__ __forceinline__ int n_virtual_passes(const FFAttnHeadPlan* plan, int n_pass, bool& any_split) {
+  int n = 0;
+  any_split = false;
+#pragma unroll
+  for (int ip = 0; ip < FF_MAX_PASS; ++ip) {
+    const uint32_t f = __ldg(&plan->pass[ip].flags);
+    if (ip < n_pass) {
+      n += (f & FF_PASS_SPLIT_SELF) ? 2 : 1;
+      any_split = any_split || (f & FF_PASS_SPLIT_SELF) != 0;
+    }
+  }
+  return n < FF_MAX_PASS ? n : FF_MAX_PASS;
+}
+
+__device__ __forceinline__ VPass virtual_pass(const FFAttnHeadPlan* plan, int n_pass, bool any_split, int vi,
+                                              const KParams& p, bool one_sweep = true) {
+  VPass v;
+  if (!any_split) {
+    v.ps = plan->pass[vi];
+    v.kind = VP_PLAIN;
+    return v;
+  }
+  int ip = 0;
+  bool found = false;
+#pragma unroll
+  for (int i = 0; i < FF_MAX_PASS - 1; ++i) {
+    const int e = (__ldg(&plan->pass[i].flags) & FF_PASS_SPLIT_SELF) ? 2 : 1;
+    if (!found && i < n_pass - 1) {
+      if (vi < e) found = true;
+      else { vi -= e; ip = i + 1; }
+    }
+  }
+  v.ps = plan->pass[ip];
+  v.kind = VP_PLAIN;
+  if (!(v.ps.flags & FF_PASS_SPLIT_SELF)) return v;
+  const int T = v.ps.key_mask >= 0 ? __ldg(p.popc + v.ps.key_mask) : 0;
+  if (one_sweep && ip == 0 && v.ps.key_mask >= 0 && v.ps.kv_stream2 < 0 && !(v.ps.flags & FF_PASS_ROW_WEIGHT) && T > 0 && T < p.s_kv) {
+    v.kind = vi == 0 ? VP_SPLIT_PRE : VP_SPLIT_SUF;
+  } else if (vi == 0) {
+    v.ps.flags &= ~FF_PASS_SPLIT_SELF;
+  } else {
+    v.ps.key_mask = v.ps.row_mask = v.ps.kv_stream2 = v.ps.key_mask2 = -1;
+    v.ps.flags = 0;
+    v.ps.weight = v.ps.weight2;
+  }
+  return v;
+}
+
+__device__ __forceinline__ float pass_coef(const VPass& v, uint32_t rb, float m_all, float l, bool acc_started,
+                                           float* pre, float& keep) {
+  keep = acc_started ? 1.f : 0.f;
+  float coef = v.ps.weight;
+  if (v.kind == VP_SPLIT_PRE) {
+    pre[0] = m_all;
+    pre[1] = l;
+    keep = 0.f;
+    coef = 1.f;
+  } else if (v.kind == VP_SPLIT_SUF) {
+    const bool own_pre = ((v.ps.flags & FF_PASS_KEY_INVERT) != 0) == ((v.ps.flags & FF_PASS_ROW_XOR) != 0 && rb);
+    const float m_pre = pre[0], l_pre = pre[1];
+    const float mm = fmaxf(m_pre, m_all);
+    const float lp = l_pre > 0.f ? l_pre * fast_exp2(m_pre - mm) : 0.f;
+    const float ls = l > 0.f ? l * fast_exp2(m_all - mm) : 0.f;
+    const float inv = lp + ls > 0.f ? 1.f / (lp + ls) : 0.f;
+    keep = (own_pre ? v.ps.weight : 0.f) + v.ps.weight2 * (lp * inv);
+    coef = (own_pre ? 0.f : v.ps.weight) + v.ps.weight2 * (ls * inv);
+  } else if (v.ps.flags & FF_PASS_ROW_WEIGHT) {
+    coef = rb ? coef : 0.f;
+  }
+  return l > 0.f ? coef / l : 0.f;
+}
+
+__device__ __forceinline__ PassCtx make_ctx(const FFAttnPass& ps, const KParams& p, int q0, int kind = VP_PLAIN) {
   PassCtx c;
   c.s0.kv = ps.kv_stream;
   c.s1.kv = ps.kv_stream2;
   c.two_seg = ps.kv_stream2 >= 0;
   c.s0.kmask = ps.key_mask;
   c.s1.kmask = ps.key_mask2;
-  c.s0.kinv = (ps.flags & FF_PASS_KEY_INVERT) != 0;
+  c.s0.kinv = kind == VP_PLAIN ? (ps.flags & FF_PASS_KEY_INVERT) != 0 : kind == VP_SPLIT_SUF;
   c.s1.kinv = (ps.flags & FF_PASS_KEY2_INVERT) != 0;
   c.s0.prefix = (ps.flags & FF_PASS_KEY_PREFIX) != 0;
   c.s1.prefix = (ps.flags & FF_PASS_KEY2_PREFIX) != 0;
   c.s0.T = ps.key_mask >= 0 ? __ldg(p.popc + ps.key_mask) : 0;
   c.s1.T = ps.key_mask2 >= 0 ? __ldg(p.popc + ps.key_mask2) : 0;
-  c.rowxor = (ps.flags & FF_PASS_ROW_XOR) != 0 && ps.row_mask >= 0;
+  c.rowxor = kind == VP_PLAIN && (ps.flags & FF_PASS_ROW_XOR) != 0 && ps.row_mask >= 0;
   c.active = true;
   c.has_rf0 = true;
   c.has_rf1 = false;
@@ -581,7 +662,8 @@
   const uint32_t sKV = smem_base + C::SMEM_Q;
   const uint32_t sACC = sKV + C::NSTAGE * C::SMEM_STAGE;
   const uint32_t sMX = sACC + C::SMEM_ACC;
-  const uint32_t bar_base = sMX + C::SMEM_MX;
+  const uint32_t sPRE = sMX + C::SMEM_MX;
+  const uint32_t bar_base = sPRE + C::SMEM_PRE;
   const uint32_t bar_q = bar_base;
   const uint32_t bar_s = bar_base + 16, bar_p = bar_base + 32;
   const uint32_t bar_kv_full = bar_base + 48, bar_kv_empty = bar_base + 48 + 8 * C::NSTAGE;
@@ -599,6 +681,8 @@
   const FFAttnHeadPlan* plan = p.plan + (size_t)stream * p.heads + head;
   int n_pass = __ldg(&plan->n_pass);
   n_pass = n_pass < 0 ? 0 : (n_pass > FF_MAX_PASS ? FF_MAX_PASS : n_pass);
+  bool any_split;
+  const int n_vpass = n_virtual_passes(plan, n_pass, any_split);
   const int n_kv_tiles = (p.s_kv + BN - 1) / BN;
 
   if (threadIdx.x == 0) {
@@ -649,9 +733,9 @@
         tma_load_4d(sQ + kt * TILE_BYTES, &tm_q, kt * BOX_COLS, head, q0, stream, bar_q);
       int it = 0;
 #pragma unroll 1
-      for (int ip = 0; ip < n_pass; ++ip) {
-        const FFAttnPass ps = plan->pass[ip];
-        const PassCtx cx = make_ctx(ps, p, q0);
+      for (int ip = 0; ip < n_vpass; ++ip) {
+        const VPass vp = virtual_pass(plan, n_pass, any_split, ip, p, C::SPLIT);
+        const PassCtx cx = make_ctx(vp.ps, p, q0, vp.kind);
         if (!cx.active) continue;
 #pragma unroll 1
         for (int seg = 0; seg < 2; ++seg) {
@@ -695,9 +779,9 @@
       int pe0 = 0, pe1 = 0, pe2 = 0, n_total = 0;
 #pragma unroll
       for (int ip = 0; ip < FF_MAX_PASS; ++ip) {
-        if (ip < n_pass) {
-          const FFAttnPass ps = plan->pass[ip];
-          const PassCtx cx = make_ctx(ps, p, q0);
+        if (ip < n_vpass) {
+          const VPass vp = virtual_pass(plan, n_pass, any_split, ip, p, C::SPLIT);
+          const PassCtx cx = make_ctx(vp.ps, p, q0, vp.kind);
           if (cx.active) {
 #pragma unroll 1
             for (int seg = 0; seg < 2; ++seg) {
@@ -882,9 +966,9 @@
     if constexpr (C::SELF) {
       if (wq == 0) {
 #pragma unroll 1
-        for (int ip = 0; ip < n_pass; ++ip) {
-          const FFAttnPass ps = plan->pass[ip];
-          const PassCtx cx = make_ctx(ps, p, q0);
+        for (int ip = 0; ip < n_vpass; ++ip) {
+          const VPass vp = virtual_pass(plan, n_pass, any_split, ip, p, C::SPLIT);
+          const PassCtx cx = make_ctx(vp.ps, p, q0, vp.kind);
           if (!cx.active) continue;
 #pragma unroll 1
           for (int seg = 0; seg < 2; ++seg) {
@@ -909,9 +993,10 @@
       }
     }
 #pragma unroll 1
-    for (int ip = 0; ip < n_pass; ++ip) {
-      const FFAttnPass ps = plan->pass[ip];
-      const PassCtx cx = make_ctx(ps, p, q0);
+    for (int ip = 0; ip < n_vpass; ++ip) {
+      const VPass vp = virtual_pass(plan, n_pass, any_split, ip, p, C::SPLIT);
+      const FFAttnPass& ps = vp.ps;
+      const PassCtx cx = make_ctx(ps, p, q0, vp.kind);
       if (!cx.active) continue;
       uint32_t rb = 0;
       if (ps.row_mask >= 0 && row < p.s_q)
@@ -1151,16 +1236,16 @@
       float l = 0.f;
       if (wrote_mine) l = a_mine * tmem_ld1_wait(tO + p.head_dim);
       if (wrote_other) l = fmaf(a_other, tmem_ld1_wait(tOx + p.head_dim), l);
-      float coef = ps.weight;
-      if (ps.flags & FF_PASS_ROW_WEIGHT) coef = rb ? coef : 0.f;
-      coef = l > 0.f ? coef / l : 0.f;
+      float keep;
+      const float coef = pass_coef(virtual_pass(plan, n_pass, any_split, ip, p, C::SPLIT), rb, m_all, l, acc_started,
+                                   mx_smem + C::SMEM_MX / 4 + 2 * threadIdx.x, keep);
       const float c_mine = coef * a_mine, c_other = coef * a_other;
 #pragma unroll
       for (int c = 0; c < DPAD / 16; ++c) {
         if ((c & 1) != wg) continue;
         float r[16];
 #pragma unroll
-        for (int i = 0; i < 16; ++i) r[i] = acc_started ? acc_row[16 * c + i] : 0.f;
+        for (int i = 0; i < 16; ++i) r[i] = keep != 0.f ? keep * acc_row[16 * c + i] : 0.f;
         if (wrote_mine) {
           float o[16];
           tmem_ld16(tO + 16 * c, o);
diff --git a/freefine_b200/plans.py b/freefine_b200/plans.py
--- a/freefine_b200/plans.py
+++ b/freefine_b200/plans.py
@@ -3,10 +3,10 @@
 import numpy as np
 
 from ._lib import (FF_MAX_PASS, FF_PASS_KEY2_INVERT, FF_PASS_KEY2_PREFIX, FF_PASS_KEY_INVERT, FF_PASS_KEY_PREFIX,
-                   FF_PASS_ROW_WEIGHT, FF_PASS_ROW_XOR, PLAN_BYTES)
+                   FF_PASS_ROW_WEIGHT, FF_PASS_ROW_XOR, FF_PASS_SPLIT_SELF, PLAN_BYTES)
 
 PASS_DTYPE = np.dtype([("kv_stream", "<i4"), ("key_mask", "<i4"), ("row_mask", "<i4"), ("flags", "<u4"),
-                       ("weight", "<f4"), ("kv_stream2", "<i4"), ("key_mask2", "<i4"), ("reserved", "<i4")])
+                       ("weight", "<f4"), ("kv_stream2", "<i4"), ("key_mask2", "<i4"), ("weight2", "<f4")])
 PLAN_DTYPE = np.dtype([("n_pass", "<i4"), ("reserved", "<i4", (3,)), ("passes", PASS_DTYPE, (FF_MAX_PASS,))])
 assert PLAN_DTYPE.itemsize == PLAN_BYTES
 
@@ -25,14 +25,17 @@
     return p
 
 
-def _add(plan, s, h, kv, weight, key_mask=-1, row_mask=-1, flags=0, kv2=-1, key_mask2=-1):
+def _add(plan, s, h, kv, weight, key_mask=-1, row_mask=-1, flags=0, kv2=-1, key_mask2=-1, weight2=0.0):
+    if weight == 0.0 and weight2 == 0.0:
+        return
     e = plan[s, h]
     i = int(e["n_pass"])
-    if i >= FF_MAX_PASS:
+    used = sum(2 if int(q["flags"]) & FF_PASS_SPLIT_SELF else 1 for q in e["passes"][:i])
+    if used + (2 if flags & FF_PASS_SPLIT_SELF else 1) > FF_MAX_PASS:
         raise ValueError(f"more than {FF_MAX_PASS} passes for stream {s} head {h}")
     ps = e["passes"][i]
     ps["kv_stream"], ps["key_mask"], ps["row_mask"], ps["flags"] = kv, key_mask, row_mask, flags
-    ps["weight"], ps["kv_stream2"], ps["key_mask2"] = weight, kv2, key_mask2
+    ps["weight"], ps["kv_stream2"], ps["key_mask2"], ps["weight2"] = weight, kv2, key_mask2, weight2
     plan[s, h]["n_pass"] = i + 1
 
 
@@ -45,7 +48,7 @@
 
 
 def tca_plan(n_edits: int, heads: int, method: str, cg, src_id, tgt_id, kind: str = "edit",
-             prefix: bool = False) -> np.ndarray:
+             prefix: bool = False, split_self: bool = False) -> np.ndarray:
     pf = FF_PASS_KEY_PREFIX if prefix else 0
     if method not in ("tca", "mmsa"):
         raise ValueError(f"method must be 'tca' or 'mmsa', got {method!r}")
@@ -62,6 +65,12 @@
                 masked = q0_masked(heads, sl, h)
                 if not masked and r == s:
                     _add(p, s, h, s, 1.0 if method == "mmsa" else w_ref + w_self)
+                    continue
+                if masked and r == s and split_self and prefix and method == "tca" and w_ref != 0.0 and w_self != 0.0:
+                    edit = kind == "edit"
+                    _add(p, s, h, s, w_ref, key_mask=src_id(e), row_mask=tgt_id(e) if edit else -1,
+                         flags=FF_PASS_KEY_INVERT | (FF_PASS_ROW_XOR if edit else 0) | pf | FF_PASS_SPLIT_SELF,
+                         weight2=w_self)
                     continue
                 if masked and kind == "edit":
                     _add(p, s, h, r, w_ref, key_mask=src_id(e), row_mask=tgt_id(e),
@@ -131,7 +140,9 @@
                 c0 = s_kv - n_k if flags & FF_PASS_KEY_INVERT else n_k
             else:
                 c0 = s_kv
-            if flags & FF_PASS_ROW_WEIGHT:
+            if flags & FF_PASS_SPLIT_SELF:
+                pairs = s_q * s_kv
+            elif flags & FF_PASS_ROW_WEIGHT:
                 pairs = n_r * c0
             elif flags & FF_PASS_ROW_XOR and ps["key_mask"] >= 0:
                 pairs = (s_q - n_r) * c0 + n_r * (s_kv - c0)
@@ -154,7 +165,8 @@
             e = plan[s, h]
             ps = ", ".join(
                 f"kv{int(q['kv_stream'])}" + (f"+kv{int(q['kv_stream2'])}" if q["kv_stream2"] >= 0 else "") +
-                f"[k{int(q['key_mask'])} r{int(q['row_mask'])} f{int(q['flags'])}]*{float(q['weight']):.3f}"
+                f"[k{int(q['key_mask'])} r{int(q['row_mask'])} f{int(q['flags'])}]*{float(q['weight']):.3f}" +
+                (f"+all*{float(q['weight2']):.3f}" if int(q["flags"]) & FF_PASS_SPLIT_SELF else "")
                 for q in e["passes"][: int(e["n_pass"])])
             out.append(f"s{s}h{h}: {ps}")
     return "\n".join(out)
@@ -162,4 +174,4 @@
 
 __all__ = ["PASS_DTYPE", "PLAN_DTYPE", "q0_masked", "plain_plan", "tca_plan", "compose_plan", "style_align_plan",
            "kv_sort_index", "algorithmic_flops", "describe", "FF_PASS_KEY_INVERT", "FF_PASS_ROW_XOR", "FF_PASS_ROW_WEIGHT",
-           "FF_PASS_KEY2_INVERT", "FF_PASS_KEY_PREFIX", "FF_PASS_KEY2_PREFIX"]
+           "FF_PASS_KEY2_INVERT", "FF_PASS_KEY_PREFIX", "FF_PASS_KEY2_PREFIX", "FF_PASS_SPLIT_SELF"]
diff --git a/include/freefine_b200.h b/include/freefine_b200.h
--- a/include/freefine_b200.h
+++ b/include/freefine_b200.h
@@ -30,7 +30,8 @@
   FF_PASS_ROW_WEIGHT = 4u,
   FF_PASS_KEY2_INVERT = 8u,
   FF_PASS_KEY_PREFIX = 16u,
-  FF_PASS_KEY2_PREFIX = 32u
+  FF_PASS_KEY2_PREFIX = 32u,
+  FF_PASS_SPLIT_SELF = 64u
 };
 
 typedef struct FFAttnPass {
@@ -41,7 +42,7 @@
   float weight;
   int32_t kv_stream2;
   int32_t key_mask2;
-  int32_t reserved;
+  float weight2;
 } FFAttnPass;
 
 typedef struct FFAttnHeadPlan {
```

Result: no change. 2.764 (median of 6 runs) (+1.0%).
